# microsoft/Tokenizer

Measured on AMD Instinct MI355X. Metric: input MB/s encoded (cl100k_base), higher is better.
Workload: dtype u8

## Files before the change

### include/tkz.h

```cpp
#ifndef TKZ_H
#define TKZ_H

#include <stddef.h>
#include <stdint.h>

#ifdef __cplusplus
extern "C" {
#endif

typedef enum tkz_status {
    TKZ_OK = 0,
    TKZ_E_FORMAT = -1,
    TKZ_E_DUP_RANK = -2,
    TKZ_E_KEY_NOT_FOUND = -3,
    TKZ_E_CAPACITY = -4,
    TKZ_E_INVALID_UTF8 = -5,
    TKZ_E_ARG = -6,
    TKZ_E_UNSUPPORTED = -7,
    TKZ_E_DEVICE = -8,
    TKZ_E_NO_DEVICE = -9,
    TKZ_E_OUT_OF_MEMORY = -10
} tkz_status;

typedef enum tkz_pattern { TKZ_PATTERN_P1 = 1, TKZ_PATTERN_CL100K = 2, TKZ_PATTERN_O200K = 3, TKZ_PATTERN_O200K_DOTNET = 4 } tkz_pattern;
// ... 44 lines not shown
                                         int32_t n_allowed, int32_t* out_ids, int64_t out_cap, int64_t* out_offsets, int64_t* needed);
void tkz_encoder_special_stats(const tkz_encoder* e, int64_t* batches, int64_t* literals);

typedef struct tkz_pending tkz_pending;
tkz_status tkz_encode_batch_device_begin(tkz_encoder* e, const uint8_t* d_bytes, const int64_t* d_doc_offsets,
                                         int64_t n_docs, int64_t total_bytes, int32_t* d_out_ids,
                                         int64_t out_cap, int64_t* d_out_offsets, void* hip_stream,
                                         tkz_pending** pending);
tkz_status tkz_encode_batch_device_end(tkz_pending* pending, int64_t* total_tokens);
tkz_status tkz_encode_batch_device_begin_counts(tkz_encoder* e, const uint8_t* d_bytes, const int64_t* d_doc_offsets,
                                                int64_t n_docs, int64_t total_bytes, int32_t* d_out_ids,
                                                int64_t out_cap, int64_t* d_out_offsets, void* hip_stream,
                                                int64_t* d_counts3, tkz_pending** pending);
const int64_t* tkz_pending_counts_device(const tkz_pending* pending);

tkz_status tkz_encode_batch_utf16(tkz_encoder* e, const uint16_t* units, const int64_t* unit_offsets,
                                  int64_t n_docs, int32_t* out_ids, int64_t out_cap,
                                  int64_t* out_offsets, int64_t* needed);

tkz_status tkz_encode_utf8(tkz_encoder* e, const uint8_t* text, int64_t len, int32_t* out_ids,
                           int64_t out_cap, int64_t* n_out);
tkz_status tkz_encode_utf16(tkz_encoder* e, const uint16_t* text, int64_t len, int32_t* out_ids,
                            int64_t out_cap, int64_t* n_out);

tkz_status tkz_encode_batch_pieces_utf8(tkz_encoder* e, const uint8_t* bytes, const int64_t* doc_offsets,
                                        int64_t n_docs, int32_t* out_ids, int64_t out_cap,
                                        int64_t* doc_piece_offsets, int64_t* piece_byte_offsets,
                                        int64_t* piece_token_offsets, int64_t piece_cap,
                                        int64_t* n_pieces, int64_t* needed_ids);

tkz_status tkz_encoder_set_special_tokens(tkz_encoder* e, const int32_t* ids, const uint8_t* literals_utf8, const int64_t* literal_offsets, int32_t n);
tkz_status tkz_decode_batch_device(tkz_encoder* e, const int32_t* d_ids, const int64_t* d_id_offsets, int64_t n_docs, int64_t total_ids,
                                   uint8_t* d_out_bytes, int64_t out_cap, int64_t* d_out_offsets, void* hip_stream, int64_t* total_bytes);
tkz_status tkz_decode_batch(tkz_encoder* e, const int32_t* ids, const int64_t* id_offsets, int64_t n_docs, uint8_t* out_bytes, int64_t out_cap,
                            int64_t* out_offsets, int64_t* needed);

tkz_status tkz_shard_write(const char* path, const int32_t* ids, int64_t n_tokens, const int64_t* offsets, int64_t n_docs,
                           int64_t doc_base, int64_t token_base);
tkz_status tkz_shard_write_device(const char* path, int32_t device, const int32_t* d_ids, int64_t n_tokens, const int64_t* d_offsets,
                                  int64_t n_docs, int64_t doc_base, int64_t token_base);
tkz_status tkz_shard_read_header(const char* path, int64_t* n_docs, int64_t* n_tokens, int64_t* doc_base, int64_t* token_base);

typedef struct tkz_comm tkz_comm;
enum { TKZ_COMM_ID_BYTES = 128 };
tkz_status tkz_comm_unique_id(uint8_t* id128);
tkz_status tkz_comm_create(const uint8_t* id128, int32_t rank, int32_t world, int32_t device, tkz_comm** out);
void tkz_comm_destroy(tkz_comm* c);
int32_t tkz_comm_world(const tkz_comm* c);
int32_t tkz_comm_rank(const tkz_comm* c);
const char* tkz_comm_backend(const tkz_comm* c);
tkz_status tkz_comm_allgather_counts_device(tkz_comm* c, const int64_t* d_mine, int64_t* d_table, void* hip_stream);
tkz_status tkz_comm_allgather_counts(tkz_comm* c, int64_t n_docs, int64_t n_bytes, int64_t n_tokens, int64_t* table);
const int64_t* tkz_encoder_counts_device(const tkz_encoder* e);
void tkz_shard_range(int64_t n_docs_total, int32_t rank, int32_t world, int64_t* lo, int64_t* hi);
tkz_status tkz_shard_bases(const int64_t* table, int32_t world, int32_t rank, int64_t* bases3, int64_t* totals3);


tkz_status tkz_pretokenize_utf8(tkz_encoder* e, const uint8_t* bytes, const int64_t* doc_offsets,
                                int64_t n_docs, uint64_t* out_bitmap_words);
tkz_status tkz_encode_pieces(tkz_encoder* e, const uint8_t* bytes, const int64_t* piece_offsets,
                             int64_t n_pieces, int32_t* out_ids, int64_t out_cap,
                             int64_t* out_offsets, int64_t* needed);

enum { TKZ_OPT_PRETOK_SEQUENTIAL = 1,
       TKZ_OPT_PIECE_MEMO = 2,
       TKZ_OPT_PIECE_STATS = 3,
       TKZ_OPT_PROMOTE = 4,
       TKZ_OPT_PROMOTE_MIN_BYTES = 5, TKZ_OPT_PROMOTE_CAP = 6,
       TKZ_OPT_CASE_EQUIVALENCE = 7,
       TKZ_OPT_LATENCY_BYTES = 8,
       TKZ_OPT_ADAPT = 9 };
tkz_status tkz_encoder_set_option(tkz_encoder* e, int32_t option, int64_t value);


enum { TKZ_K_DOCMARK = 0, TKZ_K_PRETOK = 1, TKZ_K_PROBE = 2 , TKZ_K_SCAN = 3, TKZ_K_PLACE = 4,
       TKZ_K_DOCOFFS = 5, TKZ_K_MERGE_LONG = 6 , TKZ_K_MERGE_SHORT = 7 ,
       TKZ_K_COUNT = 8 };
tkz_status tkz_encoder_set_profiling(tkz_encoder* e, int32_t enabled);
tkz_status tkz_encoder_kernel_ms(tkz_encoder* e, double* ms, int64_t* launches, int32_t reset);
void tkz_encoder_pretok_leftovers(const tkz_encoder* e, int64_t* after_ascii_scanner, int64_t* after_multibyte_scanner);
void tkz_encoder_small_path_calls(const tkz_encoder* e, int64_t* calls, int64_t* handed_back);
int32_t tkz_encoder_small_path_phases(const tkz_encoder* e, int64_t* clocks16);
tkz_status tkz_encoder_piece_stats(tkz_encoder* e, int64_t* out8, int32_t reset);
tkz_status tkz_encoder_adapt_stats(tkz_encoder* e, int64_t* out8);
int64_t tkz_encoder_memo_slots(const tkz_encoder* e);
int32_t tkz_encoder_memo_ways(const tkz_encoder* e);
int64_t tkz_encoder_memo_bucket(const tkz_encoder* e, const uint8_t* piece, int32_t len);
tkz_status tkz_encoder_reserve(tkz_encoder* e, int64_t max_bytes, int64_t max_docs);
int64_t tkz_encoder_workspace_bytes(const tkz_encoder* e);
int64_t tkz_encoder_side_by_side_batches(const tkz_encoder* e);
int64_t tkz_encoder_engine_downloads(const tkz_encoder* e);
const char* tkz_kernel_name(int32_t k);

tkz_status tkz_corpus_generate_device(int32_t device, int32_t kind, uint64_t seed, int64_t first_doc,
                                      int64_t n_docs, int32_t min_len, int32_t max_len,
                                      int64_t* d_doc_offsets, uint8_t* d_bytes, int64_t cap_bytes,
                                      void* hip_stream, int64_t* total_bytes);
int64_t tkz_corpus_generate_doc_host(int32_t kind, uint64_t seed, int64_t doc_index, int32_t min_len,
                                     int32_t max_len, uint8_t* buf, int64_t cap);

#ifdef __cplusplus
}
#endif
#endif
```

### tokenizer_amd/_native.py

```python
import ctypes as C
import os

import numpy as np

_HERE = os.path.dirname(os.path.abspath(__file__))
DEFAULT_LIB = os.environ.get("TKZ_LIBTKZ") or os.path.join(_HERE, "lib", "libtkz.so")

OK = 0
E_FORMAT, E_DUP_RANK, E_KEY_NOT_FOUND, E_CAPACITY, E_INVALID_UTF8, E_ARG, E_UNSUPPORTED, E_DEVICE, E_NO_DEVICE, E_OUT_OF_MEMORY = range(-1, -11, -1)
ENGINE_DOTNET, ENGINE_ECMASCRIPT = 0, 1
P1, CL100K, O200K, O200K_DOTNET = 1, 2, 3, 4
OPT_PRETOK_SEQUENTIAL = 1
OPT_PIECE_MEMO = 2
OPT_PIECE_STATS = 3
OPT_PROMOTE_MIN_BYTES, OPT_PROMOTE_CAP = 5, 6
OPT_CASE_EQUIVALENCE = 7
OPT_LATENCY_BYTES = 8
OPT_ADAPT = 9
OPT_PROMOTE = 4
K_NAMES = ["k_docmark", "k_pretok", "k_probe", "k_scan", "k_place", "k_docoffs", "k_merge_long_group", "k_merge_short"]


class TkzError(Exception):

# ... 10 lines not shown
    pass


class KeyNotFoundError(TkzError, KeyError):
    pass


class UnsupportedError(TkzError, NotImplementedError):
    pass


_EXC = {E_FORMAT: FormatError, E_DUP_RANK: DuplicateRankError, E_KEY_NOT_FOUND: KeyNotFoundError, E_UNSUPPORTED: UnsupportedError}


class Library:
    def __init__(self, path=None):
        path = path or DEFAULT_LIB
        if not os.path.exists(path):
            raise RuntimeError("libtkz not built: %s is missing (run `python -c 'import __graft_entry__ as g; g.build()'` "
                               "or `make -C tokenizer_amd/csrc`); there is no CPU fallback" % path)
        self.path = path
        if os.path.basename(path) == "libtkz.so":
            try:
                import torch
                if torch.cuda.is_available():
                    torch.cuda.init()
            except ImportError:
                pass
        L = self.L = C.CDLL(path)
        vp, i64, i32, sz = C.c_void_p, C.c_int64, C.c_int32, C.c_size_t
        pv = C.POINTER(C.c_void_p)
        pi64 = C.POINTER(C.c_int64)
        L.tkz_last_error.restype = C.c_char_p
        L.tkz_vocab_from_tiktoken.argtypes = [vp, sz, pv]
        L.tkz_vocab_destroy.argtypes = [vp]
        L.tkz_vocab_destroy.restype = None
        L.tkz_vocab_size.argtypes = [vp]
        L.tkz_vocab_size.restype = i64
        L.tkz_vocab_max_key_len.argtypes = [vp]
        L.tkz_vocab_pair_table_entries.argtypes = [vp]
        L.tkz_vocab_pair_table_entries.restype = i64
        L.tkz_encoder_memo_slots.argtypes = [vp]
        L.tkz_encoder_memo_slots.restype = i64
        L.tkz_encoder_memo_ways.argtypes = [vp]
        L.tkz_encoder_small_path_calls.argtypes = [vp, pi64, pi64]
        L.tkz_encoder_small_path_calls.restype = None
        L.tkz_encoder_small_path_phases.argtypes = [vp, vp]
        L.tkz_encoder_memo_bucket.argtypes = [vp, vp, i32]
        L.tkz_encoder_memo_bucket.restype = i64
        L.tkz_unicode_classes.argtypes = [C.c_uint32, C.c_int32, vp]
        L.tkz_unicode_classes.restype = None
        L.tkz_encoder_unicode_classes.argtypes = [vp, C.c_uint32, C.c_int32, vp]
        L.tkz_encoder_set_unicode_classes.argtypes = [vp, vp, i64]
        L.tkz_encoder_pretok_leftovers.argtypes = [vp, pi64, pi64]
        L.tkz_encoder_pretok_leftovers.restype = None
        L.tkz_vocab_table_bytes.argtypes = [vp, C.c_int32]
        L.tkz_vocab_table_bytes.restype = i64
        L.tkz_vocab_rank.argtypes = [vp, vp, i32]
        L.tkz_pattern_from_regex.argtypes = [C.c_char_p, C.POINTER(i32)]
        L.tkz_pattern_from_regex_engine.argtypes = [C.c_char_p, i32, C.POINTER(i32)]
        L.tkz_encoder_create.argtypes = [vp, i32, i32, pv]
        L.tkz_encoder_destroy.argtypes = [vp]
        L.tkz_encoder_destroy.restype = None
        L.tkz_encoder_device.argtypes = [vp]
        L.tkz_encode_batch_utf8.argtypes = [vp, vp, vp, i64, vp, i64, vp, pi64]
        L.tkz_host_alloc.argtypes = [C.c_size_t, pv]
        L.tkz_host_free.argtypes = [vp]
        L.tkz_host_free.restype = None
        L.tkz_encode_batch_device.argtypes = [vp, vp, vp, i64, i64, vp, i64, vp, vp, pi64]
        L.tkz_encode_batch_device_begin.argtypes = [vp, vp, vp, i64, i64, vp, i64, vp, vp, C.POINTER(vp)]
        L.tkz_encode_batch_device_end.argtypes = [vp, pi64]
        L.tkz_encode_batch_device_begin_counts.argtypes = [vp, vp, vp, i64, i64, vp, i64, vp, vp, vp, C.POINTER(vp)]
        L.tkz_pending_counts_device.argtypes = [vp]
        L.tkz_pending_counts_device.restype = vp
        L.tkz_encode_batch_utf16.argtypes = [vp, vp, vp, i64, vp, i64, vp, pi64]
        L.tkz_encode_utf8.argtypes = [vp, vp, i64, vp, i64, pi64]
        L.tkz_encode_utf16.argtypes = [vp, vp, i64, vp, i64, pi64]
        L.tkz_pretokenize_utf8.argtypes = [vp, vp, vp, i64, vp]
        L.tkz_encode_pieces.argtypes = [vp, vp, vp, i64, vp, i64, vp, pi64]
        L.tkz_encode_batch_pieces_utf8.argtypes = [vp, vp, vp, i64, vp, i64, vp, vp, vp, i64, pi64, pi64]
        L.tkz_encoder_set_option.argtypes = [vp, i32, i64]
        L.tkz_encoder_piece_stats.argtypes = [vp, vp, i32]
        L.tkz_encoder_adapt_stats.argtypes = [vp, vp]
        L.tkz_encoder_reserve.argtypes = [vp, i64, i64]
        L.tkz_encoder_set_profiling.argtypes = [vp, i32]
        L.tkz_encoder_kernel_ms.argtypes = [vp, vp, vp, i32]
        L.tkz_encoder_workspace_bytes.argtypes = [vp]
        L.tkz_encoder_workspace_bytes.restype = i64
        L.tkz_encoder_side_by_side_batches.argtypes = [vp]
        L.tkz_encoder_side_by_side_batches.restype = i64
        L.tkz_encoder_engine_downloads.argtypes = [vp]
        L.tkz_encoder_engine_downloads.restype = i64
        L.tkz_kernel_name.argtypes = [i32]
        L.tkz_kernel_name.restype = C.c_char_p
        L.tkz_corpus_generate_device.argtypes = [i32, i32, C.c_uint64, i64, i64, i32, i32, vp, vp, i64, vp, pi64]
        L.tkz_corpus_generate_doc_host.argtypes = [i32, C.c_uint64, i64, i32, i32, vp, i64]
        L.tkz_corpus_generate_doc_host.restype = i64
        L.tkz_shard_range.argtypes = [i64, i32, i32, pi64, pi64]
        L.tkz_shard_range.restype = None
        L.tkz_shard_bases.argtypes = [vp, i32, i32, vp, vp]
        L.tkz_encoder_counts_device.argtypes = [vp]
        L.tkz_encoder_counts_device.restype = vp
        L.tkz_encoder_set_special_tokens.argtypes = [vp, vp, vp, vp, i32]
        L.tkz_encode_batch_special_device.argtypes = [vp, vp, vp, i64, i64, vp, i32, vp, i64, vp, vp, pi64]
        L.tkz_encode_batch_special_utf8.argtypes = [vp, vp, vp, i64, vp, i32, vp, i64, vp, pi64]
        L.tkz_encoder_special_stats.argtypes = [vp, pi64, pi64]
        L.tkz_encoder_special_stats.restype = None
        L.tkz_decode_batch_device.argtypes = [vp, vp, vp, i64, i64, vp, i64, vp, vp, pi64]
        L.tkz_decode_batch.argtypes = [vp, vp, vp, i64, vp, i64, vp, pi64]
        L.tkz_shard_write.argtypes = [C.c_char_p, vp, i64, vp, i64, i64, i64]
        L.tkz_shard_write_device.argtypes = [C.c_char_p, i32, vp, i64, vp, i64, i64, i64]
        L.tkz_shard_read_header.argtypes = [C.c_char_p, pi64, pi64, pi64, pi64]
        self.has_comm = hasattr(L, "tkz_comm_create")
        if self.has_comm:
            L.tkz_comm_unique_id.argtypes = [vp]
            L.tkz_comm_create.argtypes = [vp, i32, i32, i32, pv]
            L.tkz_comm_destroy.argtypes = [vp]
            L.tkz_comm_destroy.restype = None
            L.tkz_comm_world.argtypes = [vp]
            L.tkz_comm_rank.argtypes = [vp]
            L.tkz_comm_backend.argtypes = [vp]
            L.tkz_comm_backend.restype = C.c_char_p
            L.tkz_comm_allgather_counts_device.argtypes = [vp, vp, vp, vp]
            L.tkz_comm_allgather_counts.argtypes = [vp, i64, i64, i64, vp]

    def check(self, status):
        if status != OK:
            msg = (self.L.tkz_last_error() or b"").decode("utf-8", "replace")
            raise _EXC.get(status, TkzError)(status, msg)


_default = None


def default_library():
    global _default
    if _default is None:
        _default = Library()
    return _default


def _ptr(a):
    return a.ctypes.data if a is not None else None


class Vocab:

    def __init__(self, tiktoken_bytes: bytes, lib: Library = None):
        self.lib = lib or default_library()
        h = C.c_void_p()
        buf = (C.c_uint8 * max(1, len(tiktoken_bytes))).from_buffer_copy(tiktoken_bytes or b"\0")
        self.lib.check(self.lib.L.tkz_vocab_from_tiktoken(buf, len(tiktoken_bytes), C.byref(h)))
        self._h = h

    def __del__(self):
        if getattr(self, "_h", None):
            self.lib.L.tkz_vocab_destroy(self._h)
            self._h = None

    def __len__(self):
        return self.lib.L.tkz_vocab_size(self._h)

    @property
    def max_key_len(self):
        return self.lib.L.tkz_vocab_max_key_len(self._h)

    @property
    def pair_table_entries(self):
        return self.lib.L.tkz_vocab_pair_table_entries(self._h)

    def table_bytes(self):
        f = self.lib.L.tkz_vocab_table_bytes
        d = {k: int(f(self._h, i)) for i, k in enumerate(("short", "mid", "long", "pair", "direct"))}
        d["total"] = int(f(self._h, -1))
        return d

    def rank(self, key: bytes):
        buf = (C.c_uint8 * max(1, len(key))).from_buffer_copy(key or b"\0")
        return self.lib.L.tkz_vocab_rank(self._h, buf, len(key))


class Encoder:

    def __init__(self, vocab: Vocab, pattern: int, device: int = 0):
        self.lib = vocab.lib
        h = C.c_void_p()
        self.lib.check(self.lib.L.tkz_encoder_create(vocab._h, pattern, device, C.byref(h)))
        self._h = h
        self.pattern = pattern

    def close(self):
        if getattr(self, "_h", None):
            self.lib.L.tkz_encoder_destroy(self._h)
            self._h = None

    def __del__(self):
        self.close()

    def set_option(self, opt, value):
        self.lib.check(self.lib.L.tkz_encoder_set_option(self._h, opt, value))

    def set_unicode_classes(self, classes):
        if classes is None:
            self.lib.check(self.lib.L.tkz_encoder_set_unicode_classes(self._h, None, 0))
            return
        a = np.ascontiguousarray(classes, dtype=np.uint8)
        self.lib.check(self.lib.L.tkz_encoder_set_unicode_classes(self._h, a.ctypes.data, len(a)))

    def unicode_classes(self, first, n):
        out = np.zeros(n, np.uint8)
        self.lib.check(self.lib.L.tkz_encoder_unicode_classes(self._h, first, n, out.ctypes.data))
        return out

    def piece_stats(self, reset=False):
        out = np.zeros(8, np.int64)
        self.lib.check(self.lib.L.tkz_encoder_piece_stats(self._h, out.ctypes.data, 1 if reset else 0))
        pieces, sm, lm, gm, look, hit = (int(out[i]) for i in (1, 2, 3, 4, 5, 6))
        return {"batches": int(out[0]), "pieces": pieces, "short_misses": sm, "long_misses": lm, "giant_pieces": gm,
                "whole_piece_hit_rate": round(1.0 - (sm + lm + gm) / pieces, 5) if pieces else None,
                "memo_lookups": look, "memo_hits": hit, "memo_hit_rate": round(hit / look, 5) if look else None,
                "merged_short": look - hit if look else sm, "promoted_pieces_in_tables": int(out[7])}

    def reserve(self, max_bytes, max_docs):
        self.lib.check(self.lib.L.tkz_encoder_reserve(self._h, int(max_bytes), int(max_docs)))

    def adapt_stats(self):
        out = np.zeros(8, np.int64)
        self.lib.check(self.lib.L.tkz_encoder_adapt_stats(self._h, out.ctypes.data))
        return {"promotions": int(out[0]), "relearns": int(out[1]), "promoted_pieces": int(out[2]), "retired_images": int(out[3]),
                "settled_miss_share": None if out[4] < 0 else out[4] / 1e6, "recent_miss_share": None if out[5] < 0 else out[5] / 1e6,
                "bytes_since_tables_changed": int(out[6]), "learning_window_bytes": int(out[7])}

    def set_profiling(self, on):
        self.lib.check(self.lib.L.tkz_encoder_set_profiling(self._h, 1 if on else 0))

    def kernel_ms(self, reset=False):
        ms = np.zeros(len(K_NAMES), np.float64)
        n = np.zeros(len(K_NAMES), np.int64)
        self.lib.check(self.lib.L.tkz_encoder_kernel_ms(self._h, ms.ctypes.data, n.ctypes.data, 1 if reset else 0))
        return {K_NAMES[i]: (float(ms[i]), int(n[i])) for i in range(len(K_NAMES))}

    @property
    def memo_slots(self):
        return int(self.lib.L.tkz_encoder_memo_slots(self._h))

    @property
    def memo_ways(self):
        return int(self.lib.L.tkz_encoder_memo_ways(self._h))

    def memo_bucket(self, piece: bytes):
        return int(self.lib.L.tkz_encoder_memo_bucket(self._h, piece, len(piece)))

    def small_path_calls(self):
        a, b = C.c_int64(0), C.c_int64(0)
        self.lib.L.tkz_encoder_small_path_calls(self._h, C.byref(a), C.byref(b))
        return a.value, b.value

    def small_path_phases(self):
        a = np.zeros(16, np.int64)
        n = self.lib.L.tkz_encoder_small_path_phases(self._h, a.ctypes.data)
        return a[:n].tolist()

    def pretok_leftovers(self):
        a, b = C.c_int64(0), C.c_int64(0)
        self.lib.L.tkz_encoder_pretok_leftovers(self._h, C.byref(a), C.byref(b))
        return a.value, b.value

    @property
    def workspace_bytes(self):
        return self.lib.L.tkz_encoder_workspace_bytes(self._h)

    @property
    def engine_downloads(self):
        return self.lib.L.tkz_encoder_engine_downloads(self._h)

    @property
    def side_by_side_batches(self):
        return self.lib.L.tkz_encoder_side_by_side_batches(self._h)

    def encode_batch(self, data: np.ndarray, offsets: np.ndarray, out_cap=None, out=None):
        data = np.ascontiguousarray(data, dtype=np.uint8)
        offsets = np.ascontiguousarray(offsets, dtype=np.int64)
        n = len(offsets) - 1
        cap = len(data) if out_cap is None else out_cap
        if out is not None:
            ids, ooff = out
            assert ids.dtype == np.int32 and ooff.dtype == np.int64 and ids.flags.c_contiguous and ooff.flags.c_contiguous
            assert len(ooff) >= n + 1
            cap = len(ids)
        else:
            ids = np.empty(max(1, cap), np.int32)
            ooff = np.empty(n + 1, np.int64)
        needed = C.c_int64(0)
        self.lib.check(self.lib.L.tkz_encode_batch_utf8(self._h, _ptr(data), _ptr(offsets), n, _ptr(ids), cap, _ptr(ooff), C.byref(needed)))
        return ids[:needed.value], ooff[:n + 1]

    def encode_batch_special(self, data: np.ndarray, offsets: np.ndarray, allowed, out_cap=None, out=None):
        data = np.ascontiguousarray(data, dtype=np.uint8)
        offsets = np.ascontiguousarray(offsets, dtype=np.int64)
        allowed = np.ascontiguousarray(allowed, dtype=np.int32)
        n = len(offsets) - 1
        cap = len(data) if out_cap is None else out_cap
        if out is not None:
            ids, ooff = out
            assert ids.dtype == np.int32 and ooff.dtype == np.int64 and ids.flags.c_contiguous and ooff.flags.c_contiguous
# ... 240 lines not shown
```

### tokenizer_amd/csrc/tkz_api.cpp

```cpp
#include <algorithm>
#include <cstdio>
#include <cstdlib>
#include <cstring>
#include <atomic>
#include <chrono>
#include <memory>
#include <mutex>
#include <thread>
#include <string>
#include <unordered_map>
#include <unordered_set>
#include <vector>

#include "../../include/tkz.h"
#include "tkz_adapt.h"
#include "tkz_bpe.h"
#include "tkz_corpus.h"
#include "tkz_kernels.h"
#include "tkz_pretok.h"
#include "tkz_promo_select.h"
#include "tkz_sdma.h"
#include "tkz_vocab.h"

namespace {
// ... 5 lines not shown
struct DeviceScope {
    int prev = -1;
    hipError_t enter(int dev) {
        int cur = -1;
        if (hipGetDevice(&cur) == hipSuccess && cur == dev) return hipSuccess;
        const hipError_t r = hipSetDevice(dev);
        if (r == hipSuccess) prev = cur;
        return r;
    }
    ~DeviceScope() { if (prev >= 0) (void)hipSetDevice(prev); }
};

#define HIP_TRY(expr)                                                                                   \
    do {                                                                                                \
        hipError_t e_ = (expr);                                                                         \
        if (e_ != hipSuccess) return fail(TKZ_E_DEVICE, std::string(#expr) + ": " + hipGetErrorString(e_)); \
    } while (0)
#define TKZ_TRY(expr)                                                                                   \
    do {                                                                                                \
        const tkz_status s_ = (expr);                                                                   \
        if (s_ != TKZ_OK) return s_;                                                                    \
    } while (0)

thread_local int64_t g_alloc_ns = 0;
thread_local int g_alloc_calls = 0;
struct AllocClock {
    std::chrono::steady_clock::time_point t0 = std::chrono::steady_clock::now();
    ~AllocClock() { g_alloc_ns += std::chrono::duration_cast<std::chrono::nanoseconds>(std::chrono::steady_clock::now() - t0).count(); ++g_alloc_calls; }
};
struct DevBuf {
    void* p = nullptr; size_t cap = 0;
    hipError_t ensure(size_t n, int64_t* accounted) {
        if (n <= cap) return hipSuccess;
        AllocClock clock;
        size_t want = std::max(n, cap + cap / 2);
        want = (want + 255) & ~size_t(255);
        void* q = nullptr;
        hipError_t e = hipMalloc(&q, want);
        if (e != hipSuccess && want > n) { want = (n + 255) & ~size_t(255); e = hipMalloc(&q, want); }
        if (e != hipSuccess) return e;
        if (p) (void)hipFree(p);
        if (getenv("TKZ_LOG_ALLOC")) fprintf(stderr, "tkz alloc: %zu -> %zu bytes (asked %zu)\n", cap, want, n);
        *accounted += (int64_t)want - (int64_t)cap;
        p = q; cap = want;
        return hipSuccess;
    }
    void release() { if (p) { AllocClock clock; (void)hipFree(p); } p = nullptr; cap = 0; }
    template <class T> T* as() const { return reinterpret_cast<T*>(p); }
};

struct DevView {
    void* p = nullptr;
    template <class T> T* as() const { return reinterpret_cast<T*>(p); }
};

struct CounterBlock {
    int32_t err; int32_t mneed ; int32_t mhigh ;
    int32_t over64 ;
    int64_t grand;
    unsigned long long pool_head;
    int64_t ndocstarts;
    unsigned long long heavy_count;
    int64_t npieces;
    unsigned long long giant_ticket;
    unsigned long long xcount, xcount2;
    unsigned long long coop_count, coop_ticket;
    unsigned long long long_log_count;
    int64_t lq_total;
    unsigned long long miss_short, miss_long;
    unsigned long long n_literals;
};

}

namespace tkz { tkz_status set_error(tkz_status s, const std::string& msg) { return fail(s, msg); } }

struct tkz_vocab { tkz::Vocab v; };

struct Workspace {
    DevBuf w_gq, w_gcnt, w_xq, w_startbits, w_tmp, w_dense, w_tcount, w_prank, w_pcount, w_pbase, w_tbase, w_bsum, w_doctok, w_dcount, w_dbase, w_pool;
    DevBuf w_zero; size_t zero_bytes = 0;
    DevView w_counters, w_docbits, w_heavyq;
    DevBuf w_mlist, w_mquad, w_mcount, w_pextra, w_coopq, w_lqcnt, w_lqbase, w_lq;
    bool learn_window_start = false;
    DevBuf w_candbits, w_segbits, w_specbits, w_endbits, w_segoffs;
    int64_t n_seg = 0;
    int64_t spec_taken = 0;
    DevBuf w_counts3;
    bool sized = false;
    int32_t mcap = tkz::kMissCapMin;
    bool place128 = false;
    int low_lists = 0, low_place = 0;
    bool learning = false;
    DevBuf s_bytes[2], s_offs[2], s_out[3], s_outoffs[3];
    struct U16Stage {
        DevBuf units, offs, docbits, grp, tsum, tbase, bsum, counters, boffs; struct Host { int32_t err; int32_t pad; int64_t grand; }* h = nullptr;
        hipError_t ensure(int64_t max_units, int64_t max_docs, int64_t* acc) {
            const int64_t nw = max_units / 64 + 1, nt = tkz::u16_tiles(max_units), nblk = (nt + tkz::kScanBlock - 1) / tkz::kScanBlock;
            const std::pair<DevBuf*, size_t> want[] = {{&units, (size_t)(max_units + 64) * 2}, {&offs, (size_t)(max_docs + 1) * 8}, {&docbits, (size_t)(nw + 8) * 8},
                                                       {&grp, (size_t)nt * 64 * 4}, {&tsum, (size_t)nt * 4}, {&tbase, (size_t)nt * 8}, {&bsum, (size_t)(nblk + 1) * 8},
                                                       {&counters, 64}, {&boffs, (size_t)(max_docs + 1) * 8}};
            for (const auto& w : want) { const hipError_t r = w.first->ensure(w.second, acc); if (r != hipSuccess) return r; }
            return h ? hipSuccess : hipHostMalloc((void**)&h, 64, 0);
        }
        void release() {
            for (DevBuf* b : {&units, &offs, &docbits, &grp, &tsum, &tbase, &bsum, &counters, &boffs}) b->release();
            if (h) (void)hipHostFree(h);
            h = nullptr;
        }
    } u16[2];
    DevBuf u_bytes[2];
    DevBuf d_grp, d_tsum, d_tbase, d_bsum, d_counters, d_ids, d_idoffs, d_out, d_outoffs;
    DevBuf p_boffs, p_toffs, p_docp;
    CounterBlock* h_counters = nullptr;
    uint8_t* h_small = nullptr;
    bool fork_token = false;
    int64_t forked_batches = 0;
    int64_t last_coop = 0;
    int64_t last_lq_total = -1;
    hipStream_t st_side = nullptr, st_side2 = nullptr; hipEvent_t ev_fork = nullptr, ev_join = nullptr, ev_join2 = nullptr;
    hipStream_t st_small = nullptr;
    std::atomic<int64_t> small_calls{0}, small_fallbacks{0};
    int64_t small_clocks[16] = {};
    hipStream_t st_compute = nullptr, st_in = nullptr, st_out = nullptr;
    hipEvent_t ev_in[2] = {}, ev_out[3] = {};
    tkz::SdmaSignal sig_out[3], sig_outoffs[3];
    int sdma_state = 0;
    std::atomic<int64_t> engine_downloads{0};
    int64_t bytes_allocated = 0;
    bool busy = false;
    hipEvent_t ev[tkz::K_COUNT][2] = {};
    bool ev_used[tkz::K_COUNT] = {};
    double ms[tkz::K_COUNT] = {};
    int64_t launches[tkz::K_COUNT] = {};
    void release_all() {
        DevBuf* bufs[] = {&w_candbits, &w_segbits, &w_specbits, &w_endbits, &w_segoffs, &w_counts3, &w_mlist, &w_mquad, &w_mcount, &w_pextra, &w_coopq, &w_lqcnt, &w_lqbase, &w_lq, &w_gq, &w_gcnt, &w_xq, &w_zero, &w_startbits, &w_tmp, &w_dense, &w_tcount, &w_prank, &w_pcount, &w_pbase, &w_tbase, &w_bsum,
                          &w_doctok, &w_dcount, &w_dbase, &w_pool, &s_bytes[0], &s_bytes[1], &s_offs[0], &s_offs[1], &s_out[0], &s_out[1], &s_out[2],
                          &s_outoffs[0], &s_outoffs[1], &s_outoffs[2], &u_bytes[0], &u_bytes[1],
                          &d_grp, &d_tsum, &d_tbase, &d_bsum, &d_counters, &d_ids, &d_idoffs, &d_out, &d_outoffs, &p_boffs, &p_toffs, &p_docp};
        for (DevBuf* b : bufs) b->release();
        for (U16Stage& U : u16) U.release();
        if (h_counters) (void)hipHostFree(h_counters);
        if (h_small) (void)hipHostFree(h_small);
        if (st_small) (void)hipStreamDestroy(st_small);
        for (hipStream_t st : {st_side, st_side2}) if (st) (void)hipStreamDestroy(st);
        for (hipEvent_t ev : {ev_fork, ev_join, ev_join2}) if (ev) (void)hipEventDestroy(ev);
        for (int k = 0; k < tkz::K_COUNT; ++k) for (int q = 0; q < 2; ++q) if (ev[k][q]) (void)hipEventDestroy(ev[k][q]);
        for (int q = 0; q < 2; ++q) if (ev_in[q]) (void)hipEventDestroy(ev_in[q]);
        for (int q = 0; q < 3; ++q) if (ev_out[q]) (void)hipEventDestroy(ev_out[q]);
        if (st_compute) (void)hipStreamDestroy(st_compute);
        if (st_in) (void)hipStreamDestroy(st_in);
        if (st_out) (void)hipStreamDestroy(st_out);
        for (int q = 0; q < 3; ++q) { tkz::sdma_signal_destroy(&sig_out[q]); tkz::sdma_signal_destroy(&sig_outoffs[q]); }
    }
};

struct tkz_encoder {
    int device = 0;
    int pattern = 0;
    int max_key_len = 0;
    bool pretok_seq = false;
    bool profiling = false;
    std::mutex mu;
    std::vector<Workspace*> pool;
    DevBuf t_short, t_mid, t_long, t_blob, t_pair, t_byte, t_bpair, t_bmp, t_counts3, t_memo;
    uint32_t memo_slots = 0;
    TkzTables T{};
    DevBuf t_decoff, t_decblob, t_decids;
    TkzDecodeTable D{};
    std::vector<std::pair<int32_t, std::string>> dec_vocab, dec_special;
    DevBuf t_lit;
    tkz::TkzLitTable LIT{};
    int lit_state = 0;
    std::string lit_why;
    std::atomic<int64_t> spec_batches{0}, spec_literals{0};
    int64_t bytes_allocated = 0;
    std::atomic<int64_t> last_xcount{0}, last_xcount2{0};
    bool small_ok = false;
    bool piece_stats = false;
    int64_t latency_bytes = [] { const char* v = getenv("TKZ_LATENCY_BYTES"); return v ? (int64_t)atoll(v) : int64_t(16) << 20; }();
    bool case_equiv = false;
    size_t bmp_image_bytes = 0;
    DevBuf t_stats;
    int64_t stat_batches = 0, stat_giants = 0;
    int pending = 0;
    bool destroyed = false;
    tkz::AdaptPolicy policy;
    DevBuf t_memo_hits, t_promo;
    DevBuf t_long_log;
    int64_t long_log_n = 0;
    std::vector<DevBuf> retired;
    std::vector<tkz::KeyItem> promo_items;
    std::unordered_set<std::string> promo_keys;
    std::vector<uint32_t> promo_quads;
    uint32_t short_slots_n = 0, mid_slots_n = 0;
    std::thread promo_thread;
    std::mutex promo_join_mu;
};

namespace {

std::atomic<int> g_fork_in_flight{0};

struct SpecialCall { tkz::TkzLitAllowed allowed; };
thread_local const SpecialCall* g_special = nullptr;
struct SpecialScope {
    explicit SpecialScope(const SpecialCall* c) { g_special = c; }
    ~SpecialScope() { g_special = nullptr; }
};

struct Lease {
    tkz_encoder* e; Workspace* ws = nullptr;
    explicit Lease(tkz_encoder* enc) : e(enc) {
        std::lock_guard<std::mutex> lock(e->mu);
        for (Workspace* w : e->pool) if (!w->busy) { ws = w; break; }
        if (!ws) { ws = new Workspace(); e->pool.push_back(ws); }
        ws->busy = true;
    }
    ~Lease() {
// ... 154 lines not shown
    if (h == hipSuccess) h = img->nt.ensure(std::max<size_t>(64, short_bytes + mid_bytes), &acc);
    if (h == hipSuccess && short_bytes) h = hipMemcpyAsync(img->nt.p, ss.data(), short_bytes, hipMemcpyHostToDevice, cs);
    if (h == hipSuccess && mid_bytes) h = hipMemcpyAsync(static_cast<char*>(img->nt.p) + short_bytes, ms.data(), mid_bytes, hipMemcpyHostToDevice, cs);
    if (h == hipSuccess) h = img->np.ensure(std::max<size_t>(64, promo_quads.size() * 4), &acc);
    if (h == hipSuccess && !promo_quads.empty()) h = hipMemcpyAsync(img->np.p, promo_quads.data(), promo_quads.size() * 4, hipMemcpyHostToDevice, cs);
    if (h == hipSuccess) h = hipStreamSynchronize(cs);
    if (cs) (void)hipStreamDestroy(cs);
    if (h != hipSuccess) { img->nt.release(); img->np.release(); return fail(TKZ_E_DEVICE, std::string("promoted tables: ") + hipGetErrorString(h)); }
    img->short_bytes = short_bytes; img->n_short_slots = ss.size(); img->n_mid_slots = ms.size(); img->n_promo = promo_items.size();
    return TKZ_OK;
}
void install_key_tables(tkz_encoder* e, KeyTablesImage& img, bool retire) {
    int64_t* acc = &e->bytes_allocated;
    *acc += (int64_t)(img.nt.cap + img.np.cap);
    if (retire) { e->retired.push_back(e->t_short); e->retired.push_back(e->t_promo); }
    else { *acc -= (int64_t)(e->t_short.cap + e->t_promo.cap); e->t_short.release(); e->t_promo.release(); }
    e->t_short = img.nt; e->t_promo = img.np;
    e->T.short_slots = e->t_short.as<TkzShortSlot>(); e->T.short_nb = (uint32_t)(img.n_short_slots / 2); e->T.short_seed = img.sseed;
    e->T.mid_slots = reinterpret_cast<const TkzMidSlot*>(e->t_short.as<char>() + img.short_bytes); e->T.mid_ns = (uint32_t)img.n_mid_slots; e->T.mid_seed = img.mseed;
    e->T.promo = img.n_promo ? e->t_promo.as<uint4>() : nullptr; e->T.promo_n = (uint32_t)img.n_promo;
    e->short_slots_n = (uint32_t)img.n_short_slots; e->mid_slots_n = (uint32_t)img.n_mid_slots;
}

void join_promotion(tkz_encoder* e) {
    std::lock_guard<std::mutex> lock(e->promo_join_mu);
    if (e->promo_thread.joinable()) e->promo_thread.join();
}
tkz_status promote_from_memo(tkz_encoder* e, bool use_hits, bool retire, int64_t* added) {
    using tkz::kLongLogDwords; using tkz::kLongLogMaxLen;
    if (added) *added = 0;
    if (!e->memo_slots || e->T.max_rank >= (int32_t)kPromoFlag) return TKZ_OK;
    std::vector<TkzMemoSlot> memo(e->memo_slots);
    std::vector<uint32_t> hits;
    hipStream_t cs = nullptr;
    HIP_TRY(hipStreamCreateWithFlags(&cs, hipStreamNonBlocking));
    struct StreamGuard { hipStream_t s; ~StreamGuard() { (void)hipStreamDestroy(s); } } stream_guard{cs};
    HIP_TRY(hipMemcpyAsync(memo.data(), e->t_memo.p, memo.size() * sizeof(TkzMemoSlot), hipMemcpyDeviceToHost, cs));
    if (use_hits) { hits.resize(e->memo_slots); HIP_TRY(hipMemcpyAsync(hits.data(), e->t_memo_hits.p, hits.size() * 4, hipMemcpyDeviceToHost, cs)); }
    HIP_TRY(hipStreamSynchronize(cs));
    std::vector<uint32_t> llog;
    if (use_hits && e->t_long_log.p) {
        unsigned long long n = 0;
        HIP_TRY(hipMemcpyAsync(&n, e->t_long_log.as<char>() + (size_t)kLongLogCap * kLongLogDwords * 4, 8, hipMemcpyDeviceToHost, cs));
        HIP_TRY(hipStreamSynchronize(cs));
        e->long_log_n = (int64_t)std::min<unsigned long long>(n, (unsigned long long)kLongLogCap);
    }
    if (use_hits && e->long_log_n > 0) {
        llog.resize((size_t)e->long_log_n * kLongLogDwords);
        HIP_TRY(hipMemcpyAsync(llog.data(), e->t_long_log.p, llog.size() * 4, hipMemcpyDeviceToHost, cs));
        HIP_TRY(hipStreamSynchronize(cs));
    }
    std::vector<tkz::KeyItem> items_copy;
    std::vector<uint32_t> quads_copy;
    {
        std::lock_guard<std::mutex> lock(e->mu);
        const tkz::PromoSelection sel = tkz::select_promotions(memo, use_hits ? &hits : nullptr, llog, e->policy.cap(), &e->promo_items, &e->promo_keys, &e->promo_quads);
        if (use_hits) e->policy.memo_read_back(sel.valid_slots, e->memo_slots);
        if (added) *added = sel.added;
        if (!sel.added) return TKZ_OK;
        items_copy = e->promo_items; quads_copy = e->promo_quads;
    }
    KeyTablesImage img;
    const tkz_status bs = build_key_tables_image(e, items_copy, quads_copy, &img);
    if (bs != TKZ_OK) return bs;
    std::lock_guard<std::mutex> lock(e->mu);
    install_key_tables(e, img, retire);
    return TKZ_OK;
}

tkz_status drop_promotions(tkz_encoder* e, bool retire) {
    {
        std::lock_guard<std::mutex> lock(e->mu);
        if (e->promo_items.empty()) return TKZ_OK;
    }
    KeyTablesImage img;
    const tkz_status st = build_key_tables_image(e, {}, {}, &img);
    if (st != TKZ_OK) return st;
    std::lock_guard<std::mutex> lock(e->mu);
    e->promo_items.clear(); e->promo_keys.clear(); e->promo_quads.clear();
    install_key_tables(e, img, retire);
    return TKZ_OK;
}

tkz_status prepare_workspace(Workspace* ws, int64_t total, int64_t n_docs, bool bitmap_only, bool pieces) {
    using namespace tkz;
    const int64_t nwords = total / 64 + 1;
    const int64_t ntiles = (total + kSub - 1) / kSub;
    const int64_t nblk = (ntiles + kScanBlock - 1) / kScanBlock;
    int64_t* acc = &ws->bytes_allocated;
    {
        static_assert(sizeof(CounterBlock) <= 256, "the counter block's place in the zero region");
        const size_t off_bits = 256, off_flags = off_bits + (size_t)(nwords + 8) * 8, end = off_flags + (size_t)ntiles + 64;
        HIP_TRY(ws->w_zero.ensure(end, acc));
        ws->w_counters.p = ws->w_zero.p; ws->w_docbits.p = ws->w_zero.as<char>() + off_bits; ws->w_heavyq.p = ws->w_zero.as<char>() + off_flags;
        ws->zero_bytes = bitmap_only ? off_flags : end;
    }
    HIP_TRY(ws->w_startbits.ensure((size_t)(nwords + 8) * 8, acc));
    HIP_TRY(ws->w_counts3.ensure(32, acc));
    if (!bitmap_only) {
        HIP_TRY(ws->w_tmp.ensure((size_t)(total + 64) * 4, acc));
        HIP_TRY(ws->w_dense.ensure((size_t)(ntiles / kMergeGroup + 1) * kDenseCap * 4, acc));
        HIP_TRY(ws->w_tcount.ensure((size_t)ntiles * 4, acc));
        HIP_TRY(ws->w_pcount.ensure((size_t)ntiles * 4, acc));
        HIP_TRY(ws->w_pbase.ensure((size_t)ntiles * 8, acc));
        HIP_TRY(ws->w_prank.ensure((size_t)(total / 3 + 8 * ntiles + 4096) * 4, acc));
        HIP_TRY(ws->w_mlist.ensure((size_t)ntiles * (size_t)ws->mcap * 4, acc));
        HIP_TRY(ws->w_mquad.ensure((size_t)ntiles * (size_t)ws->mcap * 16, acc));
        HIP_TRY(ws->w_mcount.ensure((size_t)ntiles * 4, acc));
        HIP_TRY(ws->w_pextra.ensure((size_t)ntiles * 4, acc));
        HIP_TRY(ws->w_coopq.ensure((size_t)(total / kLanePiece + 64) * 8, acc));
        {
            const int64_t nchunks = (ntiles + 63) / 64;
            HIP_TRY(ws->w_lqcnt.ensure((size_t)nchunks * 16 * 4, acc));
            HIP_TRY(ws->w_lqbase.ensure((size_t)(nchunks * 16 + 1) * 8, acc));
            HIP_TRY(ws->w_lq.ensure((size_t)(total / (kShortMax + 1) + 64) * 8, acc));
        }
        HIP_TRY(ws->w_tbase.ensure((size_t)(ntiles + 1) * 8, acc));
        HIP_TRY(ws->w_bsum.ensure((size_t)(nblk + 1) * 8, acc));
        HIP_TRY(ws->w_doctok.ensure((size_t)((pieces ? total : n_docs) + 2) * 4, acc));
        HIP_TRY(ws->w_dcount.ensure((size_t)ntiles * 4, acc));
        HIP_TRY(ws->w_dbase.ensure((size_t)ntiles * 8, acc));
        HIP_TRY(ws->w_gq.ensure((size_t)(total / kArenaPiece + 2) * 24, acc));
        HIP_TRY(ws->w_gcnt.ensure((size_t)ntiles * 4, acc));
        if (!ws->w_pool.p) HIP_TRY(ws->w_pool.ensure((size_t)std::min<int64_t>(24 * total + 4096, int64_t(64) << 20), acc));
    }
    return TKZ_OK;
}

struct PiecesOut { int64_t* piece_boffs; int64_t* piece_toffs; int64_t* doc_piece; int64_t piece_cap; int64_t n_pieces; };

struct SlowCallLog {
    int64_t total; int attempts = 0; std::chrono::steady_clock::time_point t0 = std::chrono::steady_clock::now();
    SlowCallLog(int64_t n) : total(n) { g_alloc_ns = 0; g_alloc_calls = 0; }
    ~SlowCallLog() {
        const char* v = getenv("TKZ_LOG_SLOW_MS");
        const long limit_ms = v ? atol(v) : -1L;
        if (limit_ms < 0) return;
        const double ms = std::chrono::duration<double, std::milli>(std::chrono::steady_clock::now() - t0).count();
        if (ms > (double)limit_ms)
            { fprintf(stderr, "tkz: batch call of %lld bytes: %.1f ms on the host, %.1f ms of it in %d hipMalloc/hipFree calls, %d attempt(s)\n", (long long)total, ms, (double)g_alloc_ns * 1e-6, g_alloc_calls, attempts); fflush(stderr); }
    }
};
struct HostTrace {
    static bool on() { static const bool v = getenv("TKZ_TRACE_HOST") != nullptr; return v; }
    std::chrono::steady_clock::time_point t_call = std::chrono::steady_clock::now();
    std::vector<std::pair<std::string, double>> stamps;
    void stamp(const char* what, int64_t k) {
        if (on()) stamps.emplace_back(std::string(what) + " " + std::to_string(k), std::chrono::duration<double, std::micro>(std::chrono::steady_clock::now() - t_call).count());
    }
    void print(int64_t nchunks) const {
        if (!on()) return;
        std::string line = "[tkz host trace] " + std::to_string(nchunks) + " chunks:";
        for (const auto& sp : stamps) { char b[96]; snprintf(b, sizeof b, " %s @%.0f", sp.first.c_str(), sp.second); line += b; }
        fprintf(stderr, "%s\n", line.c_str());
    }
};
enum { kCallWhole = 0, kCallBegin = 1, kCallEnd = 2 };
struct IngestSrc { const uint8_t* h_bytes; const int64_t* h_offs; };

constexpr int64_t kForkMaxLong = int64_t(1) << 20;
constexpr int64_t kForkMaxLongTail = int64_t(1) << 21, kForkTailShare = 2048;
void side_streams(tkz_encoder* e, Workspace* ws, int64_t total, tkz::Launch* L) {
    const bool short_queue = ws->last_lq_total >= 0 && (ws->last_lq_total <= kForkMaxLong || (ws->last_lq_total <= kForkMaxLongTail && ws->last_coop * kForkTailShare >= ws->last_lq_total));
    if (total <= e->latency_bytes || !short_queue) return;
    if (!ws->fork_token) { int none = 0; ws->fork_token = g_fork_in_flight.compare_exchange_strong(none, 1); }
    bool ok = ws->fork_token;
    for (hipStream_t* st : {&ws->st_side, &ws->st_side2}) if (!*st && hipStreamCreateWithFlags(st, hipStreamNonBlocking) != hipSuccess) { *st = nullptr; ok = false; }
    for (hipEvent_t* ev : {&ws->ev_fork, &ws->ev_join, &ws->ev_join2}) if (!*ev && hipEventCreateWithFlags(ev, hipEventDisableTiming) != hipSuccess) { *ev = nullptr; ok = false; }
    if (ok) { L->side = ws->st_side; L->side2 = ws->st_side2; L->ev_fork = ws->ev_fork; L->ev_join = ws->ev_join; L->ev_join2 = ws->ev_join2; }
    else (void)hipGetLastError();
}

int64_t sizing_sample(int64_t ntiles) {
    int64_t min_sub = (int64_t(64) << 20) / tkz::kSub;
    { const char* v = getenv("TKZ_SIZING_MIN_SUB"); if (v && atoll(v) > 0) min_sub = atoll(v); }
    return ntiles >= min_sub ? std::min<int64_t>(ntiles, std::max<int64_t>(ntiles / 16, min_sub / 16)) : -1;
}

tkz_status arm_learning(tkz_encoder* e, Workspace* ws, int64_t total, bool first, bool may_learn, hipStream_t stream, TkzTables* T) {
    using namespace tkz;
    {
        std::lock_guard<std::mutex> lock(e->mu);
        bool others = false;
        for (Workspace* w : e->pool) if (w != ws && w->busy) others = true;
        const AdaptPolicy::Arm arm = e->policy.may_learn(total, first && !ws->learning, may_learn, e->T.memo_n != 0, e->T.max_rank < (int32_t)kPromoFlag, e->promo_items.size(), others);
        if (arm != AdaptPolicy::Arm::No && e->t_memo_hits.ensure((size_t)e->memo_slots * 4, &e->bytes_allocated) == hipSuccess &&
            e->t_long_log.ensure((size_t)kLongLogCap * kLongLogDwords * 4 + 64, &e->bytes_allocated) == hipSuccess) {
            const bool clear = arm == AdaptPolicy::Arm::YesClearMemo;
            if (!clear || (hipMemsetAsync(e->t_memo.p, 0, size_t(e->memo_slots) * sizeof(TkzMemoSlot), stream) == hipSuccess && hipStreamSynchronize(stream) == hipSuccess)) {
                ws->learn_window_start = e->policy.window_armed(clear);
                ws->learning = true;
            }
        }
        *T = e->T;
    }
    if (ws->learning) {
        T->memo_hits = e->t_memo_hits.as<uint32_t>();
        T->memo_hits_sparse = total >= (int64_t(64) << 20) ? 1u : 0u;
        if (ws->learn_window_start && first) {
            HIP_TRY(hipMemsetAsync(T->memo_hits, 0, (size_t)e->memo_slots * 4, stream));
            HIP_TRY(hipMemsetAsync(e->t_long_log.as<char>() + (size_t)kLongLogCap * kLongLogDwords * 4, 0, 64, stream));
        }
    }
    return TKZ_OK;
}

tkz::EncodeParams bind_params(Workspace* ws, const uint8_t* d_bytes, const int64_t* d_offs, int64_t n_docs, int64_t total) {
    using namespace tkz;
    char* cb = ws->w_counters.as<char>();
    EncodeParams P{};
    P.bytes = d_bytes; P.total = total; P.startbits = ws->w_startbits.as<uint64_t>(); P.docbits = ws->w_docbits.as<uint64_t>(); P.nwords = total / 64 + 1;
    P.offs = d_offs; P.n_docs = n_docs;
    P.tmp = ws->w_tmp.as<int32_t>(); P.dense = ws->w_dense.as<int32_t>(); P.tile_count = ws->w_tcount.as<int32_t>();
    P.prank = ws->w_prank.as<int32_t>(); P.prank_cap = (int64_t)(ws->w_prank.cap / 4); P.pcount = ws->w_pcount.as<int32_t>(); P.pbase = ws->w_pbase.as<int64_t>();
    P.mlist = ws->w_mlist.as<uint32_t>(); P.mquad = ws->w_mquad.as<uint4>(); P.mcap = ws->mcap; P.mcount = ws->w_mcount.as<uint32_t>();
    P.docord_base = ws->w_dbase.as<int64_t>(); P.doc_tok = ws->w_doctok.as<int32_t>(); P.counters = ws->w_counters.as<int32_t>();
    P.giant_q = ws->w_gq.as<int64_t>(); P.giant_cap = total / kArenaPiece + 1; P.giant_cnt = ws->w_gcnt.as<int32_t>();
    P.giant_count = reinterpret_cast<unsigned long long*>(cb + offsetof(CounterBlock, heavy_count));
    P.giant_ticket = reinterpret_cast<unsigned long long*>(cb + offsetof(CounterBlock, giant_ticket));
    P.heavy_flag = ws->w_heavyq.as<uint8_t>(); P.nsub = (total + kSub - 1) / kSub;
    P.pool = ws->w_pool.as<int32_t>(); P.pool_head = reinterpret_cast<unsigned long long*>(cb + offsetof(CounterBlock, pool_head)); P.pool_cap = (int64_t)(ws->w_pool.cap / 4);
    return P;
}

#ifdef TKZ_DEVPROF
unsigned long long* g_devprof = nullptr;
tkz_status devprof_arm(tkz::EncodeParams* P, hipStream_t stream) {
    { const char* ab = getenv("TKZ_DEV_ABLATE"); P->ablate = ab ? atoi(ab) : 0; }
    if (P->ablate & 16) {
        if (!g_devprof) { HIP_TRY(hipMalloc((void**)&g_devprof, 64 * 8)); }
        HIP_TRY(hipMemsetAsync(g_devprof, 0, 64 * 8, stream));
    }
    P->devprof = g_devprof;
    return TKZ_OK;
}
tkz_status devprof_report() {
    if (!g_devprof || !getenv("TKZ_DEV_ABLATE") || !(atoi(getenv("TKZ_DEV_ABLATE")) & 16)) return TKZ_OK;
    unsigned long long h[64];
    HIP_TRY(hipMemcpy(h, g_devprof, sizeof h, hipMemcpyDeviceToHost));
    const double w = h[0] ? (double)h[0] : 1.0;
    fprintf(stderr, "[tkz devprof] k_probe waves %llu  clock ticks/wave: total %.0f  load+compact %.0f  short batches %.0f  mid batches %.0f | mid pieces/wave %.1f pieces/wave %.1f\n",
            h[0], h[1] / w, h[2] / w, h[3] / w, h[4] / w, h[5] / w, h[6] / w);
    if (h[51]) fprintf(stderr, "[tkz devprof] k_probe lane-cycle table, per sub-tile: load+compact %.0f ticks (64 lanes) | 13+-byte pre-pass %.0f ticks, %.1f pieces in %.2f passes of 64 (lane use %.3f) | main loop: first bucket %.0f ticks at lane use %.3f (%.2f batches of 64, %.1f pieces), second bucket %.0f ticks for %.1f lanes (%.3f of the lanes of the iterations that run it: %.2f of %.2f iterations), records and lists %.0f ticks at lane use %.3f\n",
                       h[2] / w, h[4] / w, h[5] / w, (double)((h[5] + 63 * h[0]) / 64) / w, h[5] ? (double)h[5] / (64.0 * (double)((h[5] + 63 * h[0]) / 64)) : 0.0,
                       h[48] / w, (double)h[52] / (64.0 * (double)h[51]), h[51] / w, h[52] / w, h[49] / w, h[53] / w, h[54] ? (double)h[53] / (128.0 * (double)h[54]) : 0.0, h[54] / w, (double)((h[51] + 1) / 2) / w,
                       h[50] / w, (double)h[52] / (64.0 * (double)h[51]));
    if (h[8]) fprintf(stderr, "[tkz devprof] k_giant_merge pieces %llu  clock ticks/piece: rounds in global memory %.0f  the tail %.0f | bytes/piece %.0f tokens/piece %.0f | slowest piece %llu ticks | global rounds/piece %.2f | parts/piece when the tail took over %.0f\n",
                      h[8], (double)h[9] / h[8], (double)h[10] / h[8], (double)h[11] / h[8], (double)h[12] / h[8], h[13], (double)h[14] / h[8], (double)h[7] / h[8]);
    if (h[8]) fprintf(stderr, "[tkz devprof] slowest giant piece: %llu bytes -> %llu tokens, global rounds %llu (%llu ticks), bytes first/middle/last %02llx %02llx %02llx\n",
                      h[24], h[27], h[25], h[28], h[29] & 255, (h[29] >> 8) & 255, (h[29] >> 16) & 255);
    if (h[32]) fprintf(stderr, "[tkz devprof] k_merge_long waves %llu units %llu  ticks/wave %.0f | of all ticks: sort %.3f batch formation %.3f bytes %.3f first level %.3f merges %.3f emission %.3f | fast batches %llu lanes/batch %.1f steps/batch %.1f merges/lane %.2f lane use in the merge loop %.3f ticks/step %.0f\n",
                       h[32], h[44], (double)h[33] / h[32], (double)h[34] / h[33], (double)h[35] / h[33], (double)h[36] / h[33], (double)h[37] / h[33], (double)h[38] / h[33], (double)h[39] / h[33],
                       h[40], (double)h[41] / (h[40] ? h[40] : 1), (double)h[42] / (h[40] ? h[40] : 1), (double)h[43] / (h[41] ? h[41] : 1), (double)h[43] / (64.0 * (h[42] ? h[42] : 1)), (double)h[38] / (h[42] ? h[42] : 1));
    if (h[16]) fprintf(stderr, "[tkz devprof] tail: batches %llu merges %llu (%.2f a batch) proposals/batch %.1f | rounds for chains of equal pairs %llu | ticks/batch %.0f | longest tail: %llu batches, %llu ticks\n",
                       h[16], h[17], (double)h[17] / h[16], (double)h[18] / h[16], h[19], (double)h[22] / h[16], h[20], h[23]);
    return TKZ_OK;
}
#else
tkz_status devprof_arm(tkz::EncodeParams*, hipStream_t) { return TKZ_OK; }
tkz_status devprof_report() { return TKZ_OK; }
#endif

tkz_status enqueue_attempt(tkz_encoder* e, Workspace* ws, const tkz::Launch& L, const TkzTables& T, const uint8_t* d_bytes, const int64_t* d_offs, int64_t n_docs,
                           int64_t total, int32_t* d_out, int64_t out_cap, int64_t* d_out_offs, bool pretok, uint64_t* d_bitmap_only, PiecesOut* po,
                           int64_t* d_counts3, const IngestSrc* ingest, bool marks_reused, int64_t nsample, bool* pieces_over) {
    using namespace tkz;
    const hipStream_t stream = L.stream;
    const int64_t nwords = total / 64 + 1, ntiles = (total + kSub - 1) / kSub;
    int32_t* counters = ws->w_counters.as<int32_t>();
    char* cb = ws->w_counters.as<char>();
    uint64_t* docbits = ws->w_docbits.as<uint64_t>();
    uint64_t* startbits = ws->w_startbits.as<uint64_t>();
    const SpecialCall* const special = d_bitmap_only || po || !pretok ? nullptr : g_special;
    if (marks_reused) {
        HIP_TRY(hipMemsetAsync(ws->w_zero.p, 0, 256, stream));
        if (!d_bitmap_only) HIP_TRY(hipMemsetAsync(ws->w_heavyq.p, 0, (size_t)(ws->w_zero.as<char>() + ws->zero_bytes - ws->w_heavyq.as<char>()), stream));
    } else {
        if (ingest) launch_ingest(L, ingest->h_bytes, total, const_cast<uint8_t*>(d_bytes), ingest->h_offs, n_docs + 1, const_cast<int64_t*>(d_offs), ws->w_zero.p, (int64_t)ws->zero_bytes);
        else if (ws->zero_bytes <= (size_t(8) << 20)) launch_ingest(L, nullptr, 0, nullptr, nullptr, 0, nullptr, ws->w_zero.p, (int64_t)ws->zero_bytes);
        else HIP_TRY(hipMemsetAsync(ws->w_zero.p, 0, ws->zero_bytes, stream));
        launch_docmark(L, d_offs, n_docs, total, docbits, counters);
        const uint64_t* isobits = docbits;
        const int64_t* iso_offs = d_offs;
        int64_t n_iso = n_docs;
        if (special) {
            for (DevBuf* b : {&ws->w_candbits, &ws->w_segbits, &ws->w_specbits, &ws->w_endbits}) HIP_TRY(b->ensure((size_t)(nwords + 8) * 8, &ws->bytes_allocated));
            launch_lit_scan(L, d_bytes, total, docbits, nwords, e->LIT, special->allowed, ws->w_candbits.as<uint64_t>(), ws->w_segbits.as<uint64_t>(),
                            ws->w_specbits.as<uint64_t>(), ws->w_endbits.as<uint64_t>(), reinterpret_cast<unsigned long long*>(cb + offsetof(CounterBlock, n_literals)));
            isobits = ws->w_segbits.as<uint64_t>();
            if (e->pretok_seq || e->pattern == TKZ_PATTERN_O200K || e->pattern == TKZ_PATTERN_O200K_DOTNET) {
                int64_t* nseg = reinterpret_cast<int64_t*>(cb + offsetof(CounterBlock, ndocstarts));
                launch_doccount2(L, isobits, isobits, nwords, total, ntiles, ws->w_dcount.as<int32_t>(), ws->w_pcount.as<int32_t>());
                launch_scan2(L, ntiles, ws->w_bsum.as<int64_t>(), ws->w_dcount.as<int32_t>(), ws->w_dbase.as<int64_t>(), nseg, 1, nullptr, nullptr, nullptr, 1, -1);
                HIP_TRY(hipMemcpyAsync(&ws->h_counters->ndocstarts, nseg, 8, hipMemcpyDeviceToHost, stream));
                HIP_TRY(hipStreamSynchronize(stream));
                ws->n_seg = ws->h_counters->ndocstarts;
                HIP_TRY(ws->w_segoffs.ensure((size_t)(ws->n_seg + 2) * 8, &ws->bytes_allocated));
                launch_seg_offsets(L, isobits, nwords, total, ntiles, ws->w_dbase.as<int64_t>(), ws->n_seg, ws->w_segoffs.as<int64_t>());
                iso_offs = ws->w_segoffs.as<int64_t>();
                n_iso = ws->n_seg;
            }
        }
        if (!pretok) {
            HIP_TRY(hipMemcpyAsync(startbits, docbits, (size_t)nwords * 8, hipMemcpyDeviceToDevice, stream));
        } else if (e->pretok_seq) {
            HIP_TRY(hipMemcpyAsync(startbits, isobits, (size_t)nwords * 8, hipMemcpyDeviceToDevice, stream));
            launch_pretok_seq(L, e->pattern, d_bytes, iso_offs, n_iso, total, startbits, T.bmp_class, counters);
        } else {
            HIP_TRY(ws->w_xq.ensure((size_t)(nwords / kRowsPerWave + 4) * 16, &ws->bytes_allocated));
            launch_pretok_rows(L, e->pattern, d_bytes, iso_offs, n_iso, total, isobits, startbits, nwords, T.bmp_class, counters,
                               ws->w_xq.as<int64_t>(), reinterpret_cast<unsigned long long*>(cb + offsetof(CounterBlock, xcount)));
        }
        if (pretok && e->case_equiv && e->pattern == TKZ_PATTERN_CL100K) launch_case_equiv_fix(L, d_bytes, total, isobits, startbits);
        if (special) launch_lit_fix(L, startbits, isobits, ws->w_specbits.as<uint64_t>(), ws->w_endbits.as<uint64_t>(), nwords);
    }
    if (d_bitmap_only) {
        HIP_TRY(hipMemcpyAsync(d_bitmap_only, startbits, (size_t)nwords * 8, hipMemcpyDeviceToDevice, stream));
    } else {
        EncodeParams P = bind_params(ws, d_bytes, d_offs, n_docs, total);
        P.lane_piece = kLanePiece;
        P.latency = total <= e->latency_bytes ? 1 : 0;
        P.tc_atomic = (L.side || P.latency) ? 1 : 0;
        if (L.side && nsample < 0) ++ws->forked_batches;
        P.coop_cap = total / P.lane_piece + 64;
        P.coop_q = ws->w_coopq.as<uint64_t>();
        P.coop_count = reinterpret_cast<unsigned long long*>(cb + offsetof(CounterBlock, coop_count));
        P.coop_ticket = reinterpret_cast<unsigned long long*>(cb + offsetof(CounterBlock, coop_ticket));
        P.lq_cnt = ws->w_lqcnt.as<int32_t>(); P.lq_base = ws->w_lqbase.as<int64_t>(); P.lq = ws->w_lq.as<uint64_t>(); P.lq_cap = total / (kShortMax + 1) + 64;
        P.lq_total = reinterpret_cast<int64_t*>(cb + offsetof(CounterBlock, lq_total)); P.lq_bsum = ws->w_bsum.as<int64_t>();
        P.miss_sums = reinterpret_cast<unsigned long long*>(cb + offsetof(CounterBlock, miss_short));
        P.stats = e->piece_stats ? e->t_stats.as<unsigned long long>() : nullptr;
        if (P.stats) HIP_TRY(hipMemcpyAsync(e->t_stats.as<char>() + 64, P.stats, 64, hipMemcpyDeviceToDevice, stream));
        P.place128 = ws->place128 ? 1 : 0;
        P.promo = T.promo; P.pextra = T.promo ? ws->w_pextra.as<int32_t>() : nullptr;
        if (ws->learning) {
            P.long_log = e->t_long_log.as<uint32_t>(); P.long_log_cap = (int32_t)kLongLogCap; P.long_log_sparse = T.memo_hits_sparse ? 1 : 0;
            P.long_log_count = reinterpret_cast<unsigned long long*>(e->t_long_log.as<char>() + (size_t)kLongLogCap * kLongLogDwords * 4);
        }
        if (special) { P.specbits = ws->w_specbits.as<uint64_t>(); P.lit_meta = e->LIT.meta; P.lit_blob = e->LIT.blob; P.n_lit = e->LIT.n; }
        TKZ_TRY(devprof_arm(&P, stream));
        int64_t* ndocstarts = reinterpret_cast<int64_t*>(cb + offsetof(CounterBlock, ndocstarts));
        int64_t* npieces = reinterpret_cast<int64_t*>(cb + offsetof(CounterBlock, npieces));
        int64_t* grand = reinterpret_cast<int64_t*>(cb + offsetof(CounterBlock, grand));
        const uint64_t* markbits = po ? startbits : docbits;
        P.docbits = markbits;
        launch_doccount2(L, markbits, startbits, nwords, total, ntiles, ws->w_dcount.as<int32_t>(), ws->w_pcount.as<int32_t>());
        launch_scan2(L, ntiles, ws->w_bsum.as<int64_t>(), ws->w_dcount.as<int32_t>(), ws->w_dbase.as<int64_t>(), ndocstarts, 1,
                     ws->w_pcount.as<int32_t>(), ws->w_pbase.as<int64_t>(), npieces, kRecordLine, -1);
        if (po) {
            HIP_TRY(hipMemcpyAsync(&ws->h_counters->ndocstarts, ndocstarts, 8, hipMemcpyDeviceToHost, stream));
            HIP_TRY(hipStreamSynchronize(stream));
            po->n_pieces = ws->h_counters->ndocstarts;
            *pieces_over = po->n_pieces > po->piece_cap;
            if (!*pieces_over) launch_piece_index(L, startbits, nwords, total, ntiles, ws->w_dbase.as<int64_t>(), po->n_pieces, po->piece_boffs, d_offs, n_docs, po->doc_piece);
        }
        if (nsample >= 0) {
            launch_probe_sample(L, T, P, nsample);
        } else {
            launch_encode(L, T, P, ntiles);
            if (P.stats) launch_miss_stats(L, P, ntiles);
            launch_scan2(L, ntiles, ws->w_bsum.as<int64_t>(), P.tile_count, ws->w_tbase.as<int64_t>(), grand, 1, nullptr, nullptr, nullptr, 1, K_SCAN);
            launch_place(L, P, ws->w_tbase.as<int64_t>(), ntiles, d_out, out_cap);
            if (po) {
                if (!*pieces_over) launch_docoffs(L, po->piece_boffs, po->n_pieces, total, ws->w_tbase.as<int64_t>(), markbits, P.docord_base, P.doc_tok, grand, po->piece_toffs);
                launch_counts3(L, n_docs, total, grand, e->t_counts3.as<int64_t>(), ws->w_counts3.as<int64_t>(), d_counts3);
            } else
                launch_docoffs(L, d_offs, n_docs, total, ws->w_tbase.as<int64_t>(), docbits, P.docord_base, P.doc_tok, grand, d_out_offs,
                               n_docs, e->t_counts3.as<int64_t>(), ws->w_counts3.as<int64_t>(), d_counts3);
        }
    }
    HIP_TRY(hipMemcpyAsync(ws->h_counters, counters, sizeof(CounterBlock), hipMemcpyDeviceToHost, stream));
    return TKZ_OK;
}

tkz_status check_counters(tkz_encoder* e, Workspace* ws, hipStream_t stream, int64_t total, int attempt, int64_t nsample, bool bitmap_only, bool* retry) {
    using namespace tkz;
    const CounterBlock& c = *ws->h_counters;
    const int64_t ntiles = (total + kSub - 1) / kSub;
    int64_t* acc = &ws->bytes_allocated;
    const int32_t err = c.err;
    *retry = false;
    if (err & kErrOffsets) return fail(TKZ_E_ARG, "document offsets must start at 0, be non-decreasing and end at the byte count");
    if (err & kErrUtf8) return fail(TKZ_E_INVALID_UTF8, "input is not well-formed UTF-8 (or a document boundary falls inside a character)");
    if (err & kErrTooLong) return fail(TKZ_E_UNSUPPORTED, "a single piece longer than 2^30 bytes");
    if (!bitmap_only) ws->sized = true;
    if (!bitmap_only && nsample < 0 && total > e->latency_bytes) {
        ws->last_coop = (int64_t)c.coop_count;
        ws->last_lq_total = c.lq_total;
    }
    if (nsample >= 0 && (int64_t)c.over64 * 5 > nsample) { ws->place128 = true; ws->low_place = 0; }
    const bool last = attempt >= 4;
    if (err & kErrPool) {
        if (last) return fail(TKZ_E_OUT_OF_MEMORY, "long-piece scratch exhausted");
        const size_t need = (size_t)c.pool_head * 4 + 4096;
        if (ws->w_pool.ensure(need, acc) != hipSuccess)
            return fail(TKZ_E_OUT_OF_MEMORY, "scratch for the pieces longer than 1024 bytes: " + std::to_string(need) + " bytes could not be allocated");
    } else if (err & kErrMissCap) {
        if (last) return fail(TKZ_E_DEVICE, "miss list overflow");
        int32_t want = kMissCapMin;
        while (want < c.mneed && want < kMissCapMax) want *= 2;
        if (want <= ws->mcap) return fail(TKZ_E_DEVICE, "miss list overflow");
        if (ws->w_mlist.ensure((size_t)ntiles * (size_t)want * 4, acc) != hipSuccess || ws->w_mquad.ensure((size_t)ntiles * (size_t)want * 16, acc) != hipSuccess)
            return fail(TKZ_E_OUT_OF_MEMORY, "miss lists: " + std::to_string((size_t)ntiles * (size_t)want * 20) + " bytes could not be allocated");
        ws->mcap = want;
    } else if (err & kErrCapacity) {
        if (last) return fail(TKZ_E_DEVICE, "piece record buffer overflow");
        const size_t need = ((size_t)c.npieces + 4096) * 4;
        if (ws->w_prank.ensure(need, acc) != hipSuccess)
            return fail(TKZ_E_OUT_OF_MEMORY, "piece records: " + std::to_string(need) + " bytes could not be allocated");
    } else if (nsample >= 0) {
        const size_t need = ((size_t)c.npieces + 4096) * 4;
        if (need > ws->w_prank.cap && ws->w_prank.ensure(need, acc) != hipSuccess)
            return fail(TKZ_E_OUT_OF_MEMORY, "piece records: " + std::to_string(need) + " bytes could not be allocated");
    } else {
        if (err & kErrKeyNotFound) return fail(TKZ_E_KEY_NOT_FOUND, "a byte of the input is not in the vocabulary (KeyNotFoundException in the reference)");
        if (!bitmap_only && e->piece_stats) {
            std::lock_guard<std::mutex> lock(e->mu);
            ++e->stat_batches; e->stat_giants += (int64_t)c.heavy_count;
        }
        return TKZ_OK;
    }
    if (e->piece_stats && e->t_stats.p && !bitmap_only) HIP_TRY(hipMemcpyAsync(e->t_stats.p, e->t_stats.as<char>() + 64, 64, hipMemcpyDeviceToDevice, stream));
    *retry = true;
    return TKZ_OK;
}

void settle_workspace(Workspace* ws, int64_t ntiles) {
    using namespace tkz;
    constexpr int kLowBatches = 3;
    const bool heavy = (int64_t)ws->h_counters->over64 * 5 > ntiles;
    if (heavy) { ws->place128 = true; ws->low_place = 0; }
    else if (ws->place128 && ++ws->low_place >= kLowBatches) { ws->place128 = false; ws->low_place = 0; }
    if (ws->mcap <= kMissCapMin) return;
    int32_t want = kMissCapMin;
    while (want < ws->h_counters->mhigh) want *= 2;
    if (want >= ws->mcap) ws->low_lists = 0;
    else if (++ws->low_lists >= kLowBatches) {
        ws->low_lists = 0;
        ws->mcap = std::max(want, ws->mcap / 2);
        if (ws->w_mquad.cap > (size_t)ntiles * (size_t)ws->mcap * 16 * 4) {
            ws->bytes_allocated -= (int64_t)(ws->w_mquad.cap + ws->w_mlist.cap);
            ws->w_mquad.release(); ws->w_mlist.release();
        }
    }
}

void promote_or_drop(tkz_encoder* e, bool promote) {
    DeviceScope scope;
    const bool dev = scope.enter(e->device) == hipSuccess;
    if (promote) {
        int64_t added = 0;
        size_t held;
        { std::lock_guard<std::mutex> lock(e->mu); held = e->promo_items.size(); }
        if (dev) (void)promote_from_memo(e, true, true, &added);
        std::lock_guard<std::mutex> lock(e->mu);
        e->policy.promotion_installed(added, held);
    } else {
        if (dev) (void)drop_promotions(e, true);
        std::lock_guard<std::mutex> lock(e->mu);
        e->policy.promotions_dropped();
    }
}

void after_batch(tkz_encoder* e, Workspace* ws, int64_t total) {
    const CounterBlock& c = *ws->h_counters;
    tkz::AdaptPolicy::After what;
    {
        std::lock_guard<std::mutex> lock(e->mu);
        what = e->policy.batch_ended(total, (double)(c.miss_short + c.miss_long), (double)c.npieces, ws->learning, e->promo_items.size());
        ws->learning = false;
    }
    const bool promote = what == tkz::AdaptPolicy::After::Promote;
    if (!promote && what != tkz::AdaptPolicy::After::Relearn) return;
    join_promotion(e);
    bool started = false;
    {
        std::lock_guard<std::mutex> jl(e->promo_join_mu);
        try { e->promo_thread = std::thread(promote_or_drop, e, promote); started = true; } catch (...) {}
    }
    if (!started) { const std::string keep_msg = g_err; promote_or_drop(e, promote); g_err = keep_msg; }
}

tkz_status encode_device(tkz_encoder* e, Workspace* ws, const uint8_t* d_bytes, const int64_t* d_offs, int64_t n_docs, int64_t total,
                         int32_t* d_out, int64_t out_cap, int64_t* d_out_offs, hipStream_t stream, bool pretok,
                         uint64_t* d_bitmap_only, int64_t* total_tokens, PiecesOut* po = nullptr, int phase = kCallWhole, int64_t* d_counts3 = nullptr,
                         const IngestSrc* ingest = nullptr) {
    using namespace tkz;
    if (n_docs < 0 || total < 0 || out_cap < 0) return fail(TKZ_E_ARG, "negative size");
    if (total_tokens) *total_tokens = 0;
    if (n_docs == 0 && total != 0) return fail(TKZ_E_ARG, "bytes without documents");
    if (total == 0) {
        if (phase != kCallEnd) {
            HIP_TRY(ws->w_counts3.ensure(32, &ws->bytes_allocated));
            { Launch L0{stream, nullptr, ws}; launch_counts3(L0, n_docs, 0, nullptr, e->t_counts3.as<int64_t>(), ws->w_counts3.as<int64_t>(), d_counts3); }
            if (d_out_offs) HIP_TRY(hipMemsetAsync(d_out_offs, 0, (size_t)(n_docs + 1) * sizeof(int64_t), stream));
            if (d_bitmap_only) { const uint64_t one = 1; HIP_TRY(hipMemcpyAsync(d_bitmap_only, &one, 8, hipMemcpyHostToDevice, stream)); }
            if (phase == kCallBegin) return TKZ_OK;
        }
        HIP_TRY(hipStreamSynchronize(stream));
        return TKZ_OK;
    }
    const int64_t ntiles = (total + kSub - 1) / kSub;
    SlowCallLog slow_log(total);
    TKZ_TRY(prepare_workspace(ws, total, n_docs, d_bitmap_only != nullptr, po != nullptr));
    if (!ws->h_counters) HIP_TRY(hipHostMalloc((void**)&ws->h_counters, sizeof(CounterBlock), 0));

    struct LearnGuard {
        tkz_encoder* e; Workspace* ws; bool keep = false;
        ~LearnGuard() { if (!keep && ws->learning) { ws->learning = false; std::lock_guard<std::mutex> lock(e->mu); e->policy.learning_abandoned(); } }
    } learn_guard{e, ws};
    bool marks_ready = false;
    for (int attempt = 0; attempt < 5; ++attempt) {
        slow_log.attempts = attempt + 1;
        bool pieces_over = false;
        const int64_t nsample = attempt == 0 && phase == kCallWhole && !ws->sized && pretok && !d_bitmap_only && !po ? sizing_sample(ntiles) : -1;
        const bool marks_reused = marks_ready;
        Launch L{stream, e->profiling ? prof_hook : nullptr, ws};
        side_streams(e, ws, total, &L);
        if (!(phase == kCallEnd && attempt == 0)) {
            TkzTables T;
            TKZ_TRY(arm_learning(e, ws, total, attempt == 0, pretok && !d_bitmap_only, stream, &T));
            TKZ_TRY(enqueue_attempt(e, ws, L, T, d_bytes, d_offs, n_docs, total, d_out, out_cap, d_out_offs, pretok, d_bitmap_only, po, d_counts3, ingest,
                                    marks_reused, nsample, &pieces_over));
        }
        if (phase == kCallBegin) { learn_guard.keep = true; return TKZ_OK; }
        HIP_TRY(hipStreamSynchronize(stream));
        HIP_TRY(hipGetLastError());
        if (e->profiling) prof_collect(ws);
        if (!d_bitmap_only) TKZ_TRY(devprof_report());
        if (!marks_reused) { e->last_xcount = (int64_t)ws->h_counters->xcount; e->last_xcount2 = (int64_t)ws->h_counters->xcount2; ws->spec_taken = (int64_t)ws->h_counters->n_literals; }
        bool retry = false;
        TKZ_TRY(check_counters(e, ws, stream, total, attempt, nsample, d_bitmap_only != nullptr, &retry));
        marks_ready = true;
        if (retry) continue;
        if (d_bitmap_only) return TKZ_OK;
        settle_workspace(ws, ntiles);
        if (pretok) after_batch(e, ws, total);
        if (g_special && !po) e->spec_literals += ws->spec_taken;
        if (total_tokens) *total_tokens = ws->h_counters->grand;
        if (pieces_over) return fail(TKZ_E_CAPACITY, "piece arrays too small");
        if (ws->h_counters->grand > out_cap) return fail(TKZ_E_CAPACITY, "output capacity too small");
        return TKZ_OK;
    }
    return fail(TKZ_E_DEVICE, "unreachable");
}

constexpr size_t kSmallOffBytes = 0, kSmallOffOffs = tkz::kSmallMaxBytes + 64, kSmallOffIds = kSmallOffOffs + (tkz::kSmallMaxDocs + 1) * 8,
                 kSmallOffOut = kSmallOffIds + tkz::kSmallMaxBytes * 4, kSmallOffRes = kSmallOffOut + (tkz::kSmallMaxDocs + 1) * 8, kSmallBlock = kSmallOffRes + 256;
bool small_eligible(const tkz_encoder* e, const int64_t* offs, int64_t n_docs, int64_t total) {
    if (!e->small_ok || e->profiling || e->pretok_seq || (e->case_equiv && e->pattern == TKZ_PATTERN_CL100K) || total <= 0 || total > tkz::kSmallMaxBytes || n_docs < 1 || n_docs > tkz::kSmallMaxDocs) return false;
    const bool o200k = e->pattern == TKZ_PATTERN_O200K || e->pattern == TKZ_PATTERN_O200K_DOTNET;
    if (o200k && total > tkz::kSmallMaxBytesO200k) return false;
    if (o200k)
        for (int64_t d = 0; d < n_docs; ++d) { const int64_t len = offs[d + 1] - offs[d]; if (len < 0 || len > tkz::kSmallMaxDoc) return false; }
    return true;
}
tkz_status encode_small(tkz_encoder* e, Workspace* ws, const uint8_t* bytes, const int64_t* offs, int64_t n_docs, int64_t total,
                        int32_t* out_ids, int64_t out_cap, int64_t* out_offsets, int64_t* needed, bool* handled) {
    using namespace tkz;
    *handled = false;
    { const tkz_status ps = prepare_workspace(ws, total, n_docs, false, false); if (ps != TKZ_OK) return ps; }
    int64_t* acc = &ws->bytes_allocated;
    HIP_TRY(ws->s_bytes[0].ensure((size_t)kSmallMaxBytes + 64, acc));
    HIP_TRY(ws->s_offs[0].ensure((size_t)(kSmallMaxDocs + 1) * 8, acc));
    if (!ws->h_small) HIP_TRY(hipHostMalloc((void**)&ws->h_small, kSmallBlock, 0));
    if (!ws->st_small) HIP_TRY(hipStreamCreateWithFlags(&ws->st_small, hipStreamNonBlocking));
    uint8_t* H = ws->h_small;
    memcpy(H + kSmallOffBytes, bytes, (size_t)total);
    memcpy(H + kSmallOffOffs, offs, (size_t)(n_docs + 1) * 8);
    int64_t* h_res = reinterpret_cast<int64_t*>(H + kSmallOffRes);
    h_res[0] = -1; h_res[1] = 0; h_res[2] = 0;
    EncodeParams P = bind_params(ws, ws->s_bytes[0].as<uint8_t>(), ws->s_offs[0].as<int64_t>(), n_docs, total);
    P.lane_piece = kSmallLanePiece;
    SmallArgs A{};
    A.h_bytes = H + kSmallOffBytes; A.h_offs = reinterpret_cast<const int64_t*>(H + kSmallOffOffs);
    A.out = reinterpret_cast<int32_t*>(H + kSmallOffIds); A.out_cap = std::min<int64_t>(out_cap, kSmallMaxBytes); A.out_offs = reinterpret_cast<int64_t*>(H + kSmallOffOut);
    A.h_result = h_res;
    A.docbits = ws->w_docbits.as<uint64_t>(); A.startbits = ws->w_startbits.as<uint64_t>();
    A.pcount = ws->w_pcount.as<int32_t>(); A.pbase = ws->w_pbase.as<int64_t>(); A.docord_base = ws->w_dbase.as<int64_t>(); A.tile_base = ws->w_tbase.as<int64_t>();
    A.counter_words = (int32_t)(sizeof(CounterBlock) / 4);
    A.counts3[0] = e->t_counts3.as<int64_t>(); A.counts3[1] = ws->w_counts3.as<int64_t>();
    TkzTables T;
    { std::lock_guard<std::mutex> lock(e->mu); T = e->T; }
    P.promo = T.promo; P.pextra = T.promo ? ws->w_pextra.as<int32_t>() : nullptr;
    Launch L{ws->st_small, nullptr, ws};
    launch_small(L, T, P, A);
    HIP_TRY(hipStreamSynchronize(ws->st_small));
    HIP_TRY(hipGetLastError());
    ws->small_calls.fetch_add(1, std::memory_order_relaxed);
    { std::lock_guard<std::mutex> lock(e->mu); memcpy(ws->small_clocks, h_res + 4, sizeof ws->small_clocks); }
    if (h_res[0] != 0) { ws->small_fallbacks.fetch_add(1, std::memory_order_relaxed); return TKZ_OK; }
    const int64_t tokens = h_res[2];
    if (needed) *needed = tokens;
    *handled = true;
    if (tokens > out_cap) return fail(TKZ_E_CAPACITY, "output capacity too small");
    if (tokens) memcpy(out_ids, H + kSmallOffIds, (size_t)tokens * 4);
    memcpy(out_offsets, H + kSmallOffOut, (size_t)(n_docs + 1) * 8);
    return TKZ_OK;
}

tkz_status check_encoder(tkz_encoder* e, DeviceScope& scope) {
    if (!e) return fail(TKZ_E_ARG, "null encoder");
    hipError_t r = scope.enter(e->device);
    if (r != hipSuccess) return fail(TKZ_E_NO_DEVICE, std::string("hipSetDevice: ") + hipGetErrorString(r));
    return TKZ_OK;
}

hipError_t ensure_streams(Workspace* ws) {
    hipError_t r = hipSuccess;
    if (!ws->st_compute) r = hipStreamCreate(&ws->st_compute);
    if (r == hipSuccess && !ws->st_in) r = hipStreamCreate(&ws->st_in);
    if (r == hipSuccess && !ws->st_out) r = hipStreamCreate(&ws->st_out);
    for (int q = 0; q < 2 && r == hipSuccess; ++q) if (!ws->ev_in[q]) r = hipEventCreate(&ws->ev_in[q]);
    for (int q = 0; q < 3 && r == hipSuccess; ++q) if (!ws->ev_out[q]) r = hipEventCreate(&ws->ev_out[q]);
    return r;
}

bool pinned_host(const void* p, void** dev) {
    if (!p) return false;
    hipPointerAttribute_t a;
    if (hipPointerGetAttributes(&a, p) != hipSuccess) { (void)hipGetLastError(); return false; }
    if (a.type != hipMemoryTypeHost) return false;
    void* d = nullptr;
    if (hipHostGetDevicePointer(&d, const_cast<void*>(p), 0) != hipSuccess || !d) { (void)hipGetLastError(); return false; }
    *dev = d;
    return true;
}

const char* const kMsgUnitOffsets = "document offsets must start at 0, be non-decreasing and end at the unit count";
const char* const kMsgEngineDownload = "a copy engine reported an error for a download";
constexpr int64_t kHostChunkMin = int64_t(8) << 20;

struct HostPlan {
    bool pin_in = false, pin_out = false;
    void *dv_in = nullptr, *dv_offs = nullptr, *dv_ids = nullptr, *dv_ooffs = nullptr;
    int64_t unit = 1, up_bytes = 0, chunk_bytes = 0, nchunks = 1;
    std::vector<int64_t> cut;
    bool blocking = false;
    bool direct_out = false, ingest_in = false;
    int nout = 1;
    int64_t max_units = 0, max_docs = 0;
};
HostPlan plan_host_batch(const void* in, bool u16, const int64_t* offs, int64_t n_docs, const int32_t* out_ids, int64_t out_cap, const int64_t* out_offsets,
                         bool pretok, const uint64_t* bitmap) {
// ... 862 lines not shown
            if (value == 0) join_promotion(e);
            return TKZ_OK;
        }
        if (value != 2 && value != 3) return fail(TKZ_E_ARG, "TKZ_OPT_PROMOTE takes 0, 1, 2 or 3");
        join_promotion(e);
        {
            std::lock_guard<std::mutex> lock(e->mu);
            for (Workspace* w : e->pool) if (w->busy) return fail(TKZ_E_ARG, "promotions can only be made or dropped by hand while no call of this encoder is in flight");
        }
        if (hipDeviceSynchronize() != hipSuccess) return fail(TKZ_E_DEVICE, "hipDeviceSynchronize");
        if (value == 2) return promote_from_memo(e, false, true, nullptr);
        { std::lock_guard<std::mutex> lock(e->mu); e->policy.reset_by_hand(); }
        return drop_promotions(e, true);
    }
    if (option == TKZ_OPT_PIECE_MEMO) {
        DeviceScope scope;
        if (value == 2) join_promotion(e);
        std::lock_guard<std::mutex> lock(e->mu);
        if (value == 2) {
            tkz_status st = check_encoder(e, scope);
            if (st != TKZ_OK) return st;
            for (Workspace* w : e->pool) if (w->busy) return fail(TKZ_E_ARG, "the piece memo can only be emptied while no call of this encoder is in flight");
            if (hipDeviceSynchronize() != hipSuccess) return fail(TKZ_E_DEVICE, "hipDeviceSynchronize");
            if (hipMemset(e->t_memo.p, 0, size_t(e->memo_slots) * sizeof(TkzMemoSlot)) != hipSuccess) return fail(TKZ_E_DEVICE, "hipMemset");
        }
        e->T.memo_n = value ? e->memo_slots : 0u;
        return TKZ_OK;
    }
    if (option == TKZ_OPT_ADAPT) {
        if (value != 0 && value != 1) return fail(TKZ_E_ARG, "TKZ_OPT_ADAPT takes 0 or 1");
        std::lock_guard<std::mutex> lock(e->mu);
        e->policy.set_adapt((int)value);
        return TKZ_OK;
    }
    return fail(TKZ_E_ARG, "unknown option");
}

tkz_status tkz_encoder_adapt_stats(tkz_encoder* e, int64_t* out8) {
    if (!e || !out8) return fail(TKZ_E_ARG, "null argument");
    join_promotion(e);
    std::lock_guard<std::mutex> lock(e->mu);
    e->policy.stats(out8);
    out8[2] = (int64_t)e->promo_items.size(); out8[3] = (int64_t)e->retired.size();
    return TKZ_OK;
}

tkz_status tkz_encoder_set_profiling(tkz_encoder* e, int32_t enabled) {
    if (!e) return fail(TKZ_E_ARG, "null encoder");
    e->profiling = enabled != 0;
    return TKZ_OK;
}
tkz_status tkz_encoder_kernel_ms(tkz_encoder* e, double* ms, int64_t* launches, int32_t reset) {
    if (!e) return fail(TKZ_E_ARG, "null encoder");
    std::lock_guard<std::mutex> lock(e->mu);
    for (int k = 0; k < tkz::K_COUNT; ++k) {
        double m = 0; int64_t n = 0;
        for (Workspace* w : e->pool) { m += w->ms[k]; n += w->launches[k]; if (reset) { w->ms[k] = 0; w->launches[k] = 0; } }
        if (ms) ms[k] = m;
        if (launches) launches[k] = n;
    }
    return TKZ_OK;
}
void tkz_encoder_pretok_leftovers(const tkz_encoder* e, int64_t* after_ascii_scanner, int64_t* after_multibyte_scanner) {
    if (after_ascii_scanner) *after_ascii_scanner = e ? e->last_xcount.load() : 0;
    if (after_multibyte_scanner) *after_multibyte_scanner = e ? e->last_xcount2.load() : 0;
}
tkz_status tkz_encoder_piece_stats(tkz_encoder* e, int64_t* out8, int32_t reset) {
    if (!e || !out8) return fail(TKZ_E_ARG, "null argument");
    for (int i = 0; i < 8; ++i) out8[i] = 0;
    join_promotion(e);
    if (!e->t_stats.p) { std::lock_guard<std::mutex> lock(e->mu); out8[7] = (int64_t)e->promo_items.size(); return TKZ_OK; }
    DeviceScope scope;
    tkz_status st = check_encoder(e, scope);
    if (st != TKZ_OK) return st;
    unsigned long long h[8] = {};
    HIP_TRY(hipDeviceSynchronize());
    HIP_TRY(hipMemcpy(h, e->t_stats.p, sizeof h, hipMemcpyDeviceToHost));
    std::lock_guard<std::mutex> lock(e->mu);
    out8[0] = e->stat_batches; out8[1] = (int64_t)h[4]; out8[2] = (int64_t)h[2]; out8[3] = (int64_t)h[3]; out8[4] = e->stat_giants;
    out8[5] = (int64_t)h[0]; out8[6] = (int64_t)h[1]; out8[7] = (int64_t)e->promo_items.size();
    if (reset) { HIP_TRY(hipMemset(e->t_stats.p, 0, 64)); e->stat_batches = e->stat_giants = 0; }
    return TKZ_OK;
}
int64_t tkz_encoder_memo_slots(const tkz_encoder* e) { return e ? (int64_t)e->memo_slots : 0; }
void tkz_encoder_small_path_calls(const tkz_encoder* e, int64_t* calls, int64_t* handed_back) {
    int64_t c = 0, f = 0;
    if (e) { tkz_encoder* m = const_cast<tkz_encoder*>(e); std::lock_guard<std::mutex> lock(m->mu); for (Workspace* w : e->pool) { c += w->small_calls; f += w->small_fallbacks; } }
    if (calls) *calls = c;
    if (handed_back) *handed_back = f;
}
int32_t tkz_encoder_small_path_phases(const tkz_encoder* e, int64_t* clocks16) {
    if (!e || !clocks16) return 0;
    tkz_encoder* m = const_cast<tkz_encoder*>(e);
    std::lock_guard<std::mutex> lock(m->mu);
    for (Workspace* w : e->pool) if (w->h_small) { memcpy(clocks16, w->small_clocks, 16 * 8); return 16; }
    return 0;
}
int32_t tkz_encoder_memo_ways(const tkz_encoder* e) { return e ? (int32_t)kMemoWays : 0; }
int64_t tkz_encoder_memo_bucket(const tkz_encoder* e, const uint8_t* piece, int32_t len) {
    if (!e || !piece || len < 1 || len > 16 || !e->memo_slots) return -1;
    uint32_t kw[4] = {0, 0, 0, 0};
    for (int32_t i = 0; i < len; ++i) { if (!piece[i]) return -1; kw[i >> 2] |= (uint32_t)piece[i] << (8 * (i & 3)); }
    return (int64_t)tkz_mulhi(tkz_hash_memo(kw, (uint32_t)len), e->memo_slots / kMemoWays);
}
tkz_status tkz_encoder_reserve(tkz_encoder* e, int64_t max_bytes, int64_t max_docs) {
    using namespace tkz;
    if (!e) return fail(TKZ_E_ARG, "null encoder");
    if (max_bytes < 0 || max_docs < 0) return fail(TKZ_E_ARG, "negative size");
    DeviceScope scope;
    tkz_status st = check_encoder(e, scope);
    if (st != TKZ_OK) return st;
    Lease lease(e);
    Workspace* ws = lease.ws;
    int64_t* acc = &ws->bytes_allocated;
    st = prepare_workspace(ws, max_bytes, max_docs, false, false);
    if (st != TKZ_OK) return st;
    const int64_t nwords = max_bytes / 64 + 1;
    HIP_TRY(ws->w_xq.ensure((size_t)(nwords / kRowsPerWave + 4) * 16, acc));
    {
        bool lits; { std::lock_guard<std::mutex> lock(e->mu); lits = e->lit_state == 1; }
        if (lits) for (DevBuf* b : {&ws->w_candbits, &ws->w_segbits, &ws->w_specbits, &ws->w_endbits}) HIP_TRY(b->ensure((size_t)(nwords + 8) * 8, acc));
    }
    if (!ws->h_counters) HIP_TRY(hipHostMalloc((void**)&ws->h_counters, sizeof(CounterBlock), 0));
    HIP_TRY(ensure_streams(ws));
    {
        const int64_t chunk = std::min<int64_t>(max_bytes, int64_t(32) << 20), cdocs = std::min<int64_t>(max_docs, std::max<int64_t>(1, chunk / 16));
        for (int q = 0; q < 3; ++q) {
            if (q < 2) {
                HIP_TRY(ws->s_bytes[q].ensure((size_t)chunk + 64, acc));
                HIP_TRY(ws->s_offs[q].ensure((size_t)(cdocs + 1) * 8, acc));
            }
            HIP_TRY(ws->s_out[q].ensure((size_t)std::max<int64_t>(chunk, 1) * 4, acc));
            HIP_TRY(ws->s_outoffs[q].ensure((size_t)(cdocs + 1) * 8, acc));
        }
    }
    {
        std::lock_guard<std::mutex> lock(e->mu);
        if (e->memo_slots && e->policy.mode() == 1) {
            if (e->t_memo_hits.ensure((size_t)e->memo_slots * 4, &e->bytes_allocated) != hipSuccess ||
                e->t_long_log.ensure((size_t)kLongLogCap * kLongLogDwords * 4 + 64, &e->bytes_allocated) != hipSuccess)
                return fail(TKZ_E_OUT_OF_MEMORY, "learning buffers could not be allocated");
        }
    }
    HIP_TRY(hipDeviceSynchronize());
    return TKZ_OK;
}
int64_t tkz_encoder_workspace_bytes(const tkz_encoder* e) {
    if (!e) return 0;
    tkz_encoder* m = const_cast<tkz_encoder*>(e);
    std::lock_guard<std::mutex> lock(m->mu);
    int64_t n = e->bytes_allocated;
    for (Workspace* w : e->pool) n += w->bytes_allocated;
    return n;
}
int64_t tkz_encoder_side_by_side_batches(const tkz_encoder* e) {
    if (!e) return 0;
    tkz_encoder* m = const_cast<tkz_encoder*>(e);
    std::lock_guard<std::mutex> lock(m->mu);
    int64_t n = 0;
    for (Workspace* w : e->pool) n += w->forked_batches;
    return n;
}
int64_t tkz_encoder_engine_downloads(const tkz_encoder* e) {
    if (!e) return 0;
    tkz_encoder* m = const_cast<tkz_encoder*>(e);
    std::lock_guard<std::mutex> lock(m->mu);
    int64_t n = 0;
    for (Workspace* w : e->pool) n += w->engine_downloads.load(std::memory_order_relaxed);
    return n;
}
const char* tkz_kernel_name(int32_t k) {
    static const char* const names[] = {"k_docmark", "k_pretok", "k_probe", "k_scan", "k_place", "k_docoffs", "k_merge_long_group", "k_merge_short"};
    return (k >= 0 && k < tkz::K_COUNT) ? names[k] : "?";
}

tkz_status tkz_corpus_generate_device(int32_t device, int32_t kind, uint64_t seed, int64_t first_doc, int64_t n_docs,
                                      int32_t min_len, int32_t max_len, int64_t* d_doc_offsets, uint8_t* d_bytes,
                                      int64_t cap_bytes, void* hip_stream, int64_t* total_bytes) {
    if (kind < 1 || kind > 5 || kind == 4 || n_docs < 0 || min_len < 0 || max_len < min_len || !d_doc_offsets || !total_bytes)
        return fail(TKZ_E_ARG, "bad corpus arguments");
    DeviceScope scope;
    hipError_t r = scope.enter(device);
    if (r != hipSuccess) return fail(TKZ_E_NO_DEVICE, std::string("hipSetDevice: ") + hipGetErrorString(r));
    hipStream_t s = static_cast<hipStream_t>(hip_stream);
    int64_t* d_total = nullptr;
    HIP_TRY(hipMalloc((void**)&d_total, 8));
    tkz::launch_corpus(s, kind, seed, first_doc, n_docs, min_len, max_len, d_doc_offsets, d_bytes, d_bytes ? cap_bytes : 0, d_total);
    hipError_t c = hipMemcpyAsync(total_bytes, d_total, 8, hipMemcpyDeviceToHost, s);
    if (c == hipSuccess) c = hipStreamSynchronize(s);
    if (c == hipSuccess) c = hipGetLastError();
    (void)hipFree(d_total);
    if (c != hipSuccess) return fail(TKZ_E_DEVICE, std::string("corpus generation: ") + hipGetErrorString(c));
    if (d_bytes && *total_bytes > cap_bytes) return fail(TKZ_E_CAPACITY, "corpus buffer too small");
    return TKZ_OK;
}

void tkz_shard_range(int64_t n_docs_total, int32_t rank, int32_t world, int64_t* lo, int64_t* hi) {
    if (world < 1) world = 1;
// ... 27 lines not shown
```

### tokenizer_amd/csrc/tkz_kernels.h

```cpp
#pragma once
#include <stdint.h>

#include "tkz_simt.h"
#include "tkz_tables.h"

namespace tkz {

constexpr int kThreads = 256;
constexpr int kSub = 1024;
constexpr int kHalo = 64;
constexpr int kShortMax = 16;
#ifndef TKZ_MERGE_GROUP
#define TKZ_MERGE_GROUP 16
#endif
constexpr int kMergeGroup = TKZ_MERGE_GROUP;
constexpr int kDenseCap = 256 * kMergeGroup;
#ifndef TKZ_ARENA_DWORDS
#define TKZ_ARENA_DWORDS 2560
#endif
constexpr int kArenaDwords = TKZ_ARENA_DWORDS;
constexpr int kArenaPiece = 1024;
#ifndef TKZ_LANE_PIECE
#define TKZ_LANE_PIECE 128
#endif
constexpr int kLanePiece = TKZ_LANE_PIECE;
constexpr int kLongLogDwords = 12, kLongLogMaxLen = 28;
constexpr int kSmallLanePiece = 256;
constexpr int kMaxPiece = 1 << 30;
constexpr int kRowsPerWave = 62;
constexpr int kScanBlock = 1024;
constexpr int kRecordLine = 16;
constexpr int kMissCapMin = 64, kMissCapMax = 1024;

enum { K_DOCMARK = 0, K_PRETOK = 1, K_ENCODE = 2, K_SCAN = 3, K_GATHER = 4, K_DOCOFFS = 5, K_HEAVY = 6, K_MERGE_SHORT = 7, K_COUNT = 8 };

#ifdef TKZ_DEVPROF
#define TKZ_DEV_FLAG(P, bit) (((P).ablate & (bit)) != 0)
#else
#define TKZ_DEV_FLAG(P, bit) false
#endif

struct EncodeParams {
    const uint8_t* bytes; int64_t total;
    const uint64_t* startbits; const uint64_t* docbits; int64_t nwords;
    const int64_t* offs; int64_t n_docs;
    int32_t* tmp;
    int32_t* dense;
    int32_t* tile_count;
    int32_t* prank; int64_t prank_cap;
    const int32_t* pcount;
    const int64_t* pbase;
    uint32_t* mlist; int32_t mcap;
    uint4* mquad;
    uint32_t* mcount;
    const int64_t* docord_base;
    int32_t* doc_tok;
    int32_t* counters;
    int32_t latency;
    int32_t lane_piece;
    uint8_t* heavy_flag; int64_t nsub;
    int32_t* pool; unsigned long long* pool_head; int64_t pool_cap;
    int64_t* giant_q; unsigned long long* giant_count; int64_t giant_cap; int32_t* giant_cnt;
    unsigned long long* giant_ticket;
    uint64_t* coop_q; unsigned long long* coop_count; unsigned long long* coop_ticket; int64_t coop_cap;
    int32_t* lq_cnt; int64_t* lq_base; int64_t* lq_total; int64_t* lq_bsum; uint64_t* lq; int64_t lq_cap;
    unsigned long long* miss_sums;
    unsigned long long* devprof;
    int32_t ablate;
    unsigned long long* stats;
    uint32_t* long_log; unsigned long long* long_log_count; int32_t long_log_cap; int32_t long_log_sparse;
    int32_t* pextra;
    const uint4* promo;
    int32_t tc_atomic;
    int32_t place128;
    const uint64_t* specbits; const uint32_t* lit_meta; const uint8_t* lit_blob; int32_t n_lit;
};

constexpr int kLitMax = 256, kLitMaxLen = 128, kLitMetaHead = 8;
struct TkzLitTable { const uint32_t* meta; const uint8_t* blob; int32_t n; int32_t blob_bytes; };
struct TkzLitAllowed { uint64_t m[kLitMax / 64]; };

constexpr int kSmallLdsBytesNeeded = 86 * 1024;
constexpr int kSmallMaxBytes = 131072, kSmallMaxBytesO200k = 65536, kSmallMaxDocs = 8192, kSmallMaxDoc = 1024;
struct SmallArgs {
    const uint8_t* h_bytes; const int64_t* h_offs;
    int32_t* out; int64_t out_cap; int64_t* out_offs;
    int64_t* h_result;
    uint64_t* docbits; uint64_t* startbits;
    int32_t* pcount; int64_t* pbase; int64_t* docord_base; int64_t* tile_base;
    int32_t counter_words;
    int64_t* counts3[2];
};

typedef void (*KernelHook)(void* ctx, int kernel_id, int phase , hipStream_t s);
struct Launch { hipStream_t stream; KernelHook hook; void* hook_ctx; hipStream_t side = nullptr, side2 = nullptr; hipEvent_t ev_fork = nullptr, ev_join = nullptr, ev_join2 = nullptr; };

void launch_docmark(const Launch& L, const int64_t* d_offs, int64_t n_items, int64_t total, uint64_t* bits, int32_t* counters);
void launch_pretok_rows(const Launch& L, int pattern, const uint8_t* d_bytes, const int64_t* d_offs, int64_t n_docs, int64_t total,
                        const uint64_t* docbits, uint64_t* startbits, int64_t nrows, const uint8_t* bmp, int32_t* counters,
                        int64_t* xq, unsigned long long* xcount);
void launch_pretok_seq(const Launch& L, int pattern, const uint8_t* d_bytes, const int64_t* d_offs, int64_t n_docs, int64_t total,
                       uint64_t* startbits, const uint8_t* bmp, int32_t* counters);
void launch_ingest(const Launch& L, const uint8_t* h_bytes, int64_t total, uint8_t* d_bytes, const int64_t* h_offs, int64_t n_offs, int64_t* d_offs, void* zero, int64_t zero_bytes);
void launch_probe_sample(const Launch& L, const TkzTables& T, const EncodeParams& P, int64_t nsample);
void launch_encode(const Launch& L, const TkzTables& T, const EncodeParams& P, int64_t nsub);
void launch_small(const Launch& L, const TkzTables& T, const EncodeParams& P, const SmallArgs& A);
void launch_scan(const Launch& L, const int32_t* tile_count, int64_t ntiles, int64_t* bsum, int64_t* tile_base, int64_t* grand, int kid, int round_to = 1);
void launch_place(const Launch& L, const EncodeParams& P, const int64_t* tile_base, int64_t nsub, int32_t* out, int64_t out_cap);
void launch_docoffs(const Launch& L, const int64_t* d_offs, int64_t n_docs, int64_t total, const int64_t* tile_base,
                    const uint64_t* docbits, const int64_t* docord_base, const int32_t* doc_tok, const int64_t* grand, int64_t* out_offs,
                    int64_t c3_docs = 0, int64_t* c3a = nullptr, int64_t* c3b = nullptr, int64_t* c3c = nullptr);
void launch_doccount2(const Launch& L, const uint64_t* bits_a, const uint64_t* bits_b, int64_t nwords, int64_t total, int64_t nsub, int32_t* cnt_a, int32_t* cnt_b);
void launch_scan2(const Launch& L, int64_t ntiles, int64_t* bsum, const int32_t* cnt_a, int64_t* base_a, int64_t* grand_a, int round_to_a,
                  const int32_t* cnt_b, int64_t* base_b, int64_t* grand_b, int round_to_b, int kid);
void launch_rebase(const Launch& L, int64_t* offs, int64_t n, int64_t base);
void launch_case_equiv_fix(const Launch& L, const uint8_t* d_bytes, int64_t total, const uint64_t* docbits, uint64_t* startbits);
void launch_miss_stats(const Launch& L, const EncodeParams& P, int64_t nsub);
void launch_lit_scan(const Launch& L, const uint8_t* d_bytes, int64_t total, const uint64_t* docbits, int64_t nwords, const TkzLitTable& LT, const TkzLitAllowed& A,
                     uint64_t* candbits, uint64_t* segbits, uint64_t* specbits, uint64_t* endbits, unsigned long long* n_taken);
void launch_lit_fix(const Launch& L, uint64_t* startbits, const uint64_t* segbits, const uint64_t* specbits, const uint64_t* endbits, int64_t nwords);
void launch_seg_offsets(const Launch& L, const uint64_t* segbits, int64_t nwords, int64_t total, int64_t nsub, const int64_t* ord_base, int64_t n_seg, int64_t* seg_offs);
void launch_counts3(const Launch& L, int64_t n_docs, int64_t total, const int64_t* grand, int64_t* out3, int64_t* out3b = nullptr, int64_t* out3c = nullptr);
int64_t u16_tiles(int64_t total_units);
void launch_u16_len(const Launch& L, const uint16_t* units, int64_t total, const uint64_t* docbits, int64_t ntiles, int32_t* grp_prefix, int32_t* tile_sum);
void launch_u16_write(const Launch& L, const uint16_t* units, int64_t total, const uint64_t* docbits, int64_t ntiles, const int64_t* tile_base,
                      uint8_t* out, const int64_t* unit_offs, int64_t n_docs, const int32_t* grp_prefix, const int64_t* grand, int64_t* byte_offs);
void launch_piece_index(const Launch& L, const uint64_t* startbits, int64_t nwords, int64_t total, int64_t nsub, const int64_t* ord_base,
                        int64_t n_pieces, int64_t* piece_offs, const int64_t* d_offs, int64_t n_docs, int64_t* doc_piece);
int64_t dec_tiles(int64_t total_ids);
void launch_dec_len(const Launch& L, const TkzDecodeTable& D, const int32_t* ids, int64_t total, int64_t ntiles, int32_t* grp_prefix, int32_t* tile_sum);
void launch_dec_write(const Launch& L, const TkzDecodeTable& D, const int32_t* ids, int64_t total, int64_t ntiles, const int64_t* tile_base, uint8_t* out,
                      int64_t out_cap, const int64_t* id_offs, int64_t n_docs, const int32_t* grp_prefix, const int64_t* grand, int64_t* byte_offs, int32_t* counters);
void launch_corpus(hipStream_t s, int kind, uint64_t seed, int64_t first_doc, int64_t n_docs, int min_len, int max_len,
                   int64_t* d_offs, uint8_t* d_bytes, int64_t cap_bytes, int64_t* d_total);

}
```

### tokenizer_amd/csrc/tkz_kernels.hip

```cpp
#include "tkz_kernels.h"

#include <type_traits>

#include "tkz_bpe.h"
#include "tkz_classes.h"
#include "tkz_corpus.h"
#include "tkz_pretok.h"
#include "tkz_simt.h"

namespace tkz {

TKZ_KERNEL(256) void k_docmark(const int64_t* offs, int64_t n_items, int64_t total, uint64_t* bits, int32_t* counters) {
    const int64_t stride = simt::nblocks() * simt::nthreads();
    for (int64_t d = simt::bid() * simt::nthreads() + simt::tid(); d <= n_items; d += stride) {
        const int64_t pos = offs[d];
        bool ok = pos >= 0 && pos <= total;
        if (d == 0) ok = ok && pos == 0;
        if (d == n_items) ok = ok && pos == total;
        else ok = ok && pos <= offs[d + 1];
        if (!ok) { simt::atomic_or((unsigned*)&counters[0], (unsigned)kErrOffsets); continue; }
        const int64_t w = pos >> 6;
        if (d > 0) { const int64_t prev = offs[d - 1]; if (prev >= 0 && prev <= pos && (prev >> 6) == w) continue; }
        uint64_t m = 1ull << (pos & 63);
        int64_t cur = pos;
        for (int64_t e = d + 1; e <= n_items;) {
            const int64_t q = offs[e];
            if (q < cur || (q >> 6) != w) break;
            if (q == cur) {
                int64_t lo = e + 1, hi = n_items + 1;
                while (lo < hi) { const int64_t mid = (lo + hi) >> 1; if (offs[mid] <= cur) lo = mid + 1; else hi = mid; }
                e = lo;
                continue;
            }
            m |= 1ull << (q & 63);
            cur = q; ++e;
        }
        bits[w] = m;
    }
}

struct RowInfo { TkzRowLane L; TkzRowMasks m; bool simple; };
template <int PATTERN>
TKZ_DEV RowInfo tkz_load_row(const TkzSrc& S, int64_t row, const uint8_t* bmp, const uint16_t* aflags) {
    RowInfo r;
    const int64_t pos = (row << 6) + simt::lane();
    const uint32_t b = tkz_gbyte(S, pos);
    const bool full = row >= 0 && ((row + 1) << 6) <= S.total;
    r.simple = full && simt::ballot(b >= 0x80u) == 0;
    if (r.simple) {
        const uint32_t f = aflags[b];
        r.L.pc = tkz_pc_of_flags(f); r.L.len = 1; r.L.off = 0; r.L.b = b; r.L.bad = 0;
        r.m = tkz_row_masks_ascii(f);
    } else {
        r.L = tkz_classify_byte(S, pos, bmp);
        r.m = tkz_row_masks(r.L, PATTERN == TKZ_PAT_CL100K);
    }
    return r;
}

template <int PATTERN>
TKZ_DEV void tkz_rows_sequential(const TkzSrc& S, const uint64_t* docbits, uint64_t* startbits, int64_t nrows, const uint8_t* bmp,
                                 const uint16_t* aflags, int64_t r0, int64_t r1, int32_t* counters) {
    const int lane = simt::lane();
    auto ds_at = [&](int64_t r) -> uint64_t { return (r >= 0 && r < nrows) ? docbits[r] : 0; };
    int64_t rw = r0;
    while (rw > 0) {
        if (ds_at(rw) & 1ull) break;
        const int pc = simt::first_lane(tkz_classify_byte(S, (rw << 6) - 1, bmp).pc);
        if (pc != PC_N && pc != PC_CRLF) break;
        --rw;
    }
    TkzScanCarry cy;
    cy.nb63 = 0; cy.carryN = 0; cy.abs63 = 0; cy.sa_from = -1; cy.sa_end = -1; cy.sa_lastcr = -1;
    int64_t row = rw > 0 ? rw - 1 : 0;
    RowInfo P = tkz_load_row<PATTERN>(S, row - 1, bmp, aflags);
    RowInfo C = tkz_load_row<PATTERN>(S, row, bmp, aflags);
    uint64_t dsP = ds_at(row - 1), dsC = ds_at(row);
    int clenP = 0, o1msP = 0, bad = 0;
    uint64_t c2P = 0, c3P = 0, o1P = 0;
    for (; row < r1; ++row) {
        const RowInfo N = tkz_load_row<PATTERN>(S, row + 1, bmp, aflags);
        const uint64_t dsN = ds_at(row + 1);
        int clenC, o1msC;
        uint64_t c2C, c3C, o1C, out;
        if (C.simple && N.simple) {
            out = tkz_row_eval_ascii<PATTERN>(P.m, C.m, N.m, dsC, dsN, c2P, c3P, o1P, &c2C, &c3C, &o1C, cy, S, docbits, nrows, bmp, row);
            clenC = (int)((c2C >> lane) & 1ull) * 2 + (int)((c3C >> lane) & 1ull) * 3;
            o1msC = (int)((o1C >> lane) & 1ull);
        } else {
            out = tkz_row_eval<PATTERN>(P.L, C.L, N.L, dsP, dsC, dsN, C.m, N.m, clenP, o1msP, &clenC, &o1msC, &c2C, &c3C, &o1C, cy,
                                        S, docbits, nrows, bmp, row);
        }
        if (row >= r0) {
            if (lane == 0) startbits[row] = out;
            bad |= C.L.bad | ((C.L.off != 0 && ((dsC >> lane) & 1ull)) ? 1 : 0);
        }
        P = C; C = N; dsP = dsC; dsC = dsN; clenP = clenC; o1msP = o1msC; c2P = c2C; c3P = c3C; o1P = o1C;
    }
    if (simt::ballot(bad != 0) && lane == 0) simt::atomic_or((unsigned*)&counters[0], (unsigned)kErrUtf8);
}

template <int PATTERN>
TKZ_KERNEL(64) void k_pretok_rows(const uint8_t* bytes, int64_t total, const uint64_t* docbits, uint64_t* startbits,
                                  int64_t nrows, const uint8_t* bmp, int32_t* counters, int64_t* xq, unsigned long long* xcount) {
    TKZ_SHARED uint16_t s_aflags[128];
    TKZ_SHARED uint4 s_blk[(65 * kBlockRowStride) / 16];
    for (int i = simt::tid(); i < 128; i += simt::nthreads()) s_aflags[i] = (uint16_t)tkz_ascii_flags((uint32_t)i, PATTERN == TKZ_PAT_CL100K);
    const int lane = simt::lane();
    const int64_t r0 = simt::bid() * kRowsPerWave;
    const int64_t first = r0 - 1;
    const bool inside = ((first + 64) << 6) <= total;
    if (inside) {
        for (int c = lane; c < 256; c += 64) {
            const int64_t pos = (first << 6) + 16 * (int64_t)c;
            uint4 v; v.x = v.y = v.z = v.w = 0;
            if (pos >= 0) v = tkz_load16(bytes + pos);
            s_blk[((c >> 2) * kBlockRowStride + (c & 3) * 16) / 16] = v;
        }
        if (lane < kBlockRowStride / 16) {
            uint4 z; z.x = z.y = z.z = z.w = 0;
            const int64_t pos = (first + 64) << 6;
            if (lane == 0 && pos + 16 <= total) z = tkz_load16(bytes + pos);
            s_blk[(64 * kBlockRowStride) / 16 + lane] = z;
        }
    }
    simt::sync();
    if (r0 >= nrows) return;
    if (inside) {
        const int64_t row = first + lane;
        const uint64_t ds = (row >= 0 && row < nrows) ? docbits[row] : 0;
        uint64_t out;
        bool done;
        if constexpr (PATTERN == TKZ_PAT_O200K) {
            TkzBlockCtx X; X.bytes = bytes; X.docbits = docbits; X.total = total; X.nrows = nrows; X.row0 = first;
            done = tkz_block_eval_o200k(reinterpret_cast<const uint8_t*>(s_blk), ds, X, &out);
        } else done = tkz_block_eval<PATTERN>(reinterpret_cast<const uint8_t*>(s_blk), ds, bmp, &out);
        if (done) {
            if (lane >= 1 && lane <= kRowsPerWave && row < nrows) startbits[row] = out;
            if (PATTERN == TKZ_PAT_O200K && lane == 0) reinterpret_cast<uint8_t*>(xq)[simt::bid()] = 0;
            return;
        }
    }
    const int64_t r1 = r0 + kRowsPerWave < nrows ? r0 + kRowsPerWave : nrows;
    if constexpr (PATTERN == TKZ_PAT_O200K) {
        for (int64_t r = r0 + lane; r < r1; r += 64) startbits[r] = docbits[r];
        if (lane == 0) reinterpret_cast<uint8_t*>(xq)[simt::bid()] = 1;
    } else {
        TkzSrc S;
        S.bytes = bytes; S.total = total; S.stage = nullptr; S.lo = 0; S.hi = 0;
        tkz_rows_sequential<PATTERN>(S, docbits, startbits, nrows, bmp, s_aflags, r0, r1, counters);
    }
}

constexpr int kPretokBlkQuads = (65 * kBlockRowStride) / 16;
template <int PATTERN>
TKZ_DEV void tkz_pretok_block(int64_t blk, uint4* s_blk, const uint16_t* s_aflags, const uint8_t* bytes, int64_t total, const uint64_t* docbits,
                              uint64_t* startbits, int64_t nrows, const uint8_t* bmp, int32_t* counters) {
    static_assert(PATTERN != TKZ_PAT_O200K, "o200k blocks need the two follow-up kernels");
    const int lane = simt::lane();
    const int64_t r0 = blk * kRowsPerWave;
    if (r0 >= nrows) return;
    const int64_t first = r0 - 1;
    const bool inside = ((first + 64) << 6) <= total;
    if (inside) {
        (void)simt::ballot(true);
        for (int c = lane; c < 256; c += 64) {
            const int64_t pos = (first << 6) + 16 * (int64_t)c;
            uint4 v; v.x = v.y = v.z = v.w = 0;
            if (pos >= 0) v = tkz_load16(bytes + pos);
            s_blk[((c >> 2) * kBlockRowStride + (c & 3) * 16) / 16] = v;
        }
        if (lane < kBlockRowStride / 16) {
            uint4 z; z.x = z.y = z.z = z.w = 0;
            const int64_t pos = (first + 64) << 6;
            if (lane == 0 && pos + 16 <= total) z = tkz_load16(bytes + pos);
            s_blk[(64 * kBlockRowStride) / 16 + lane] = z;
        }
        (void)simt::ballot(true);
        const int64_t row = first + lane;
        const uint64_t ds = (row >= 0 && row < nrows) ? docbits[row] : 0;
        uint64_t out;
        if (tkz_block_eval<PATTERN>(reinterpret_cast<const uint8_t*>(s_blk), ds, bmp, &out)) {
            if (lane >= 1 && lane <= kRowsPerWave && row < nrows) startbits[row] = out;
            return;
        }
    }
    const int64_t r1 = r0 + kRowsPerWave < nrows ? r0 + kRowsPerWave : nrows;
    TkzSrc S;
    S.bytes = bytes; S.total = total; S.stage = nullptr; S.lo = 0; S.hi = 0;
    tkz_rows_sequential<PATTERN>(S, docbits, startbits, nrows, bmp, s_aflags, r0, r1, counters);
}

TKZ_KERNEL_OCC(64, 3) void k_pretok_mb_blocks(const uint8_t* bytes, int64_t total, const uint64_t* docbits, uint64_t* startbits, int64_t nrows,
                                       const uint8_t* bmp, const uint8_t* xflag, int64_t nblk, unsigned long long* xcount, int64_t* xq2, unsigned long long* xcount2,
                                       int by_code_point) {
    TKZ_SHARED uint4 s_blk[(65 * kBlockRowStride) / 16];
    const int lane = simt::lane();
    unsigned long long mine = 0;
    for (int64_t blk = simt::bid(); blk < nblk; blk += simt::nblocks()) {
        if (xflag[blk] != 1) continue;
        ++mine;
        const int64_t r0 = blk * kRowsPerWave, first = r0 - 1;
        bool done = false;
        uint64_t out = 0;
        simt::sync();
        for (int c = lane; c < 260; c += 64) {
            const int64_t pos = (first << 6) + 16 * (int64_t)c;
            uint4 v; v.x = v.y = v.z = v.w = 0;
            if (pos >= 0 && pos + 16 <= total) v = tkz_load16(bytes + pos);
            else if (pos >= 0 && pos < total) {
                uint32_t w[4] = {0, 0, 0, 0};
                for (int j = 0; j < 16; ++j) if (pos + j < total) w[j >> 2] |= (uint32_t)bytes[pos + j] << (8 * (j & 3));
                v.x = w[0]; v.y = w[1]; v.z = w[2]; v.w = w[3];
            }
            if (c < 256) s_blk[((c >> 2) * kBlockRowStride + (c & 3) * 16) / 16] = v;
            else {
                uint4 z; z.x = z.y = z.z = z.w = 0;
                s_blk[(64 * kBlockRowStride) / 16 + (c - 256)] = c == 256 ? v : z;
            }
        }
        if (lane == 0) { uint4 z; z.x = z.y = z.z = z.w = 0; s_blk[(64 * kBlockRowStride) / 16 + 4] = z; }
        simt::sync();
        {
            const int64_t row = first + lane;
            const uint64_t ds = (row >= 0 && row < nrows) ? docbits[row] : 0;
            TkzBlockCtx X; X.bytes = bytes; X.docbits = docbits; X.total = total; X.nrows = nrows; X.row0 = first;
            done = tkz_block_eval_o200k_mb(reinterpret_cast<const uint8_t*>(s_blk), ds, X, bmp, by_code_point != 0, &out);
            if (done && lane >= 1 && lane <= kRowsPerWave && row < nrows) startbits[row] = out;
        }
        if (!done && lane == 0) xq2[simt::atomic_add64(xcount2, 1ull)] = blk;
// ... 178 lines not shown
            if (acc) simt::atomic_or64((unsigned long long*)&startbits[curw], acc);
        }
    }
}

TKZ_KERNEL(256) void k_pretok_seq(const uint8_t* bytes, const int64_t* offs, int64_t n_docs, int64_t total, uint64_t* startbits,
                                  int pattern, const uint8_t* bmp, int32_t* counters) {
    const int64_t stride = simt::nblocks() * simt::nthreads();
    for (int64_t d = simt::bid() * simt::nthreads() + simt::tid(); d < n_docs; d += stride) {
        const int64_t a = offs[d], b = offs[d + 1];
        if (b <= a || a < 0 || b > total) continue;
        TkzDoc doc; doc.b = bytes + a; doc.n = b - a; doc.bmp = bmp; doc.by_code_point = pattern == TKZ_PAT_O200K;
        int bad = 0;
        for (int64_t p = 0; p < doc.n;) { const TkzChar c = tkz_doc_char(doc, p); bad |= c.bad; p += c.len; }
        if (bad) { simt::atomic_or((unsigned*)&counters[0], (unsigned)kErrUtf8); continue; }
        int64_t curw = -1; uint64_t acc = 0;
        for (int64_t p = 0; p < doc.n;) {
            const int64_t g = a + p;
            if ((g >> 6) != curw) {
                if (acc) simt::atomic_or64((unsigned long long*)&startbits[curw], acc);
                curw = g >> 6; acc = 0;
            }
            acc |= 1ull << (g & 63);
            p = tkz_match_at(pattern, doc, p);
        }
        if (acc) simt::atomic_or64((unsigned long long*)&startbits[curw], acc);
    }
}

constexpr uint32_t kPrMiss = 1u << 31, kPrMark = 1u << 30, kPrLong = 1u << 29, kPrGiant = 1u << 28;
constexpr uint32_t kPrRankMask = (1u << 28) - 1u;
constexpr uint32_t kMrDone = 1u << 31, kMrDense = 1u << 30, kMrInline = 1u << 29;
constexpr int kMrLenShift = 10, kMrCntShift = 12;
constexpr uint32_t kMrOffMask = (1u << kMrCntShift) - 1u;
static_assert(kDenseCap <= (1 << kMrCntShift) && kSub <= (1 << kMrLenShift), "the offset field of a result entry");
#ifndef TKZ_PROBE_U
#define TKZ_PROBE_U 2
#endif
#ifndef TKZ_MS_THREADS
#define TKZ_MS_THREADS 256
#endif
#ifndef TKZ_PROBE_OCC
#define TKZ_PROBE_OCC 8
#endif
constexpr int kGroup = kMergeGroup;
constexpr int kMsThreads = TKZ_MS_THREADS;
#ifndef TKZ_PROBE_PER
#define TKZ_PROBE_PER 1
#endif
constexpr int kProbePer = TKZ_PROBE_PER;
constexpr int kMidMax = kSub / (TKZ_SHORT_KEY_MAX + 1) + 2;

TKZ_DEV int64_t tkz_xcd_block(int64_t b, int64_t nblocks) { return (b & 7) * (nblocks >> 3) + (b >> 3); }

template <int BITS>
TKZ_DEV int tkz_wave_scan(int v, int* total) {
    const uint64_t below = tkz_lowmask(simt::lane());
    int pre = 0, tot = 0;
#pragma unroll
    for (int j = 0; j < BITS; ++j) {
        const uint64_t m = simt::ballot((v >> j) & 1);
        pre += tkz_popc64(m & below) << j;
        tot += tkz_popc64(m) << j;
    }
    *total = tot;
    return pre;
}

TKZ_DEV int tkz_wave_scan_sum(int v, int* total) {
    const int x = simt::scan_inclusive(v);
    *total = simt::last_lane(x);
    return x - v;
}

TKZ_DEV uint32_t tkz_key_dword(const uint32_t* s_bytes, int s, int len, int i) {
    const int w = (s >> 2) + i;
    const uint32_t x = simt::alignbit(s_bytes[w + 1], s_bytes[w], (uint32_t)(s & 3) * 8u);
    const int nb = len - 4 * i;
    return nb >= 4 ? x : (nb <= 0 ? 0u : (x & ((1u << (8 * nb)) - 1u)));
}

constexpr int kProbeLdsBytes = (kSub + kHalo) + 2 * (kSub + 2) + 2 * kMidMax + 4 * kMidMax + 4 * (kSub / 32);
constexpr int kProbeLdsQuads = (kProbeLdsBytes + 15) / 16;
struct ProbeLds { uint32_t* bytes; uint16_t* pstart; uint16_t* mid; uint32_t* midres; uint32_t* mark; const uint4* kmask; uint32_t* spec ; };
TKZ_DEV ProbeLds tkz_probe_lds(uint4* wave_quads, const uint4* kmask) {
    ProbeLds L;
    uint8_t* b = reinterpret_cast<uint8_t*>(wave_quads);
    L.bytes = reinterpret_cast<uint32_t*>(b); b += kSub + kHalo;
    L.midres = reinterpret_cast<uint32_t*>(b); b += 4 * kMidMax;
    L.mark = reinterpret_cast<uint32_t*>(b); b += 4 * (kSub / 32);
    L.pstart = reinterpret_cast<uint16_t*>(b); b += 2 * (kSub + 2);
    L.mid = reinterpret_cast<uint16_t*>(b);
    L.kmask = kmask;
    L.spec = nullptr;
    return L;
}
TKZ_DEV void tkz_probe_kmask_init(uint4* s_kmask) {
    if (simt::tid() <= TKZ_SHORT_KEY_MAX) {
        const int len = simt::tid();
        uint32_t m[3];
        for (int i = 0; i < 3; ++i) { const int nb = len - 4 * i; m[i] = nb >= 4 ? 0xFFFFFFFFu : (nb <= 0 ? 0u : ((1u << (8 * nb)) - 1u)); }
        uint4 v; v.x = m[0]; v.y = m[1]; v.z = m[2]; v.w = 0;
        s_kmask[len] = v;
    }
}
struct ProbeText { uint4 v0, v1; };
static_assert((kSub + kHalo) / 16 <= 128, "two 16-byte loads per lane cover the sub-tile and its halo");
TKZ_DEV void tkz_probe_request_text(const EncodeParams& P, int64_t sub, ProbeText* tx) {
    const int lane = simt::lane();
    const int64_t base = sub * kSub;
    uint4 v0, v1;
    v0.x = v0.y = v0.z = v0.w = 0; v1 = v0;
    const int64_t p0 = base + 16 * (int64_t)lane, p1 = base + 16 * (int64_t)(lane + 64);
    if (p0 + 16 <= P.total) v0 = tkz_load16_nt(P.bytes + p0);
    else {
        uint32_t w[4] = {0, 0, 0, 0};
        for (int j = 0; j < 16; ++j) if (p0 + j < P.total) w[j >> 2] |= (uint32_t)P.bytes[p0 + j] << (8 * (j & 3));
        v0.x = w[0]; v0.y = w[1]; v0.z = w[2]; v0.w = w[3];
    }
    if (lane + 64 < (kSub + kHalo) / 16) {
        if (p1 + 16 <= P.total) v1 = tkz_load16_nt(P.bytes + p1);
        else {
            uint32_t w[4] = {0, 0, 0, 0};
            for (int j = 0; j < 16; ++j) if (p1 + j < P.total) w[j >> 2] |= (uint32_t)P.bytes[p1 + j] << (8 * (j & 3));
            v1.x = w[0]; v1.y = w[1]; v1.z = w[2]; v1.w = w[3];
        }
    }
    tx->v0 = v0; tx->v1 = v1;
}
TKZ_DEV int32_t tkz_lit_id(const EncodeParams& P, const uint8_t* sb, const uint8_t* gb, int s, int len) {
    const uint8_t* tx = s + len <= kSub + kHalo ? sb + s : gb + s;
    for (int i = 0; i < P.n_lit; ++i) {
        const uint32_t m = P.lit_meta[kLitMetaHead + 2 * i];
        if ((int)(m >> 16) != len) continue;
        const uint8_t* lit = P.lit_blob + (m & 0xFFFFu);
        int k = 0;
        while (k < len && lit[k] == tx[k]) ++k;
        if (k == len) return (int32_t)P.lit_meta[kLitMetaHead + 2 * i + 1];
    }
    return TKZ_RANK_NONE;
}
template <bool REPORT, bool SPECIAL = false>
TKZ_DEV void tkz_probe_subtile(const TkzTables& T, const EncodeParams& P, int64_t sub, const ProbeLds& LD, ProbeText& tx, int64_t next) {
    const int lane = simt::lane();
    uint32_t* s_bytes = LD.bytes;
    uint16_t* s_pstart = LD.pstart;
    uint16_t* s_mid = LD.mid;
    uint32_t* s_midres = LD.midres;
    uint32_t* s_mark = LD.mark;
    const uint4* s_kmask = LD.kmask;
    const uint8_t* sb = reinterpret_cast<const uint8_t*>(s_bytes);
    const int64_t base = sub * kSub;
    const int nb = (int)(P.total - base < kSub ? P.total - base : kSub);
    const uint8_t* gbase = P.bytes + base;
    const bool prof = TKZ_DEV_FLAG(P, 16);
    long long t_0 = prof ? simt::clock() : 0, t_1 = 0, t_2 = 0, t_3 = 0;
    uint4 v0 = tx.v0, v1 = tx.v1;
    uint64_t myword = 0, mymark = 0;
    uint64_t myspec = 0;
    if (lane < kSub / 64) {
        const int64_t w = sub * (kSub / 64) + lane;
        if (w < P.nwords) { myword = P.startbits[w]; mymark = P.docbits[w]; if (SPECIAL) myspec = P.specbits[w]; }
    }
    const int64_t from = base + nb, w0 = from >> 6;
    uint64_t ahead = (w0 + lane < P.nwords) ? P.startbits[w0 + lane] : 0ull;
    const int64_t pb = P.pbase[sub];
    { uint4* s4 = reinterpret_cast<uint4*>(s_bytes); s4[lane] = v0; if (lane + 64 < (kSub + kHalo) / 16) s4[lane + 64] = v1; }
    if (next >= 0) tkz_probe_request_text(P, next, &tx);
    if (lane < kSub / 64) {
        const int lim = nb - lane * 64;
        if (lim <= 0) myword = 0; else if (lim < 64) myword &= tkz_lowmask(lim);
        s_mark[2 * lane] = (uint32_t)mymark; s_mark[2 * lane + 1] = (uint32_t)(mymark >> 32);
        if (SPECIAL) { LD.spec[2 * lane] = (uint32_t)myspec; LD.spec[2 * lane + 1] = (uint32_t)(myspec >> 32); }
    }
    int64_t last_end;
    {
        int64_t found = -1;
        for (int64_t c = 0; found < 0; ++c) {
            const int64_t w = w0 + c * 64 + lane;
            uint64_t v = c == 0 ? ahead : (w < P.nwords ? P.startbits[w] : 0);
            if (w == w0) v &= ~tkz_lowmask((int)(from & 63));
            const uint64_t any = simt::ballot(v != 0);
            if (any) {
                const int src = tkz_ctz64(any);
                const uint32_t lo = simt::shflu((uint32_t)v, src), hi = simt::shflu((uint32_t)(v >> 32), src);
                found = ((w0 + c * 64 + src) << 6) + tkz_ctz64(((uint64_t)hi << 32) | lo);
            } else if (w0 + (c + 1) * 64 >= P.nwords) found = P.total;
        }
        last_end = found;
    }
    const int last_end_rel = (int)(last_end - base < 2 * kSub + 2 ? last_end - base : 2 * kSub + 2);
    const uint32_t wlo = simt::shflu((uint32_t)myword, lane >> 2), whi = simt::shflu((uint32_t)(myword >> 32), lane >> 2);
    const uint32_t bits16 = (uint32_t)(((((uint64_t)whi << 32) | wlo) >> (16 * (lane & 3))) & 0xFFFFull);
    int np;
    {
        int off = tkz_wave_scan<5>(tkz_popc32(bits16), &np);
        for (uint32_t b = bits16; b; b &= b - 1) s_pstart[off++] = (uint16_t)(16 * lane + tkz_ctz32(b));
        if (lane == 0) s_pstart[np] = (uint16_t)last_end_rel;
    }
    (void)simt::ballot(true);
    if (prof) t_1 = simt::clock();
    const char* tb0 = reinterpret_cast<const char*>(T.short_slots);
    const uint32_t mid_off = (uint32_t)(reinterpret_cast<const char*>(T.mid_slots) - tb0);
    int nmid = 0;
#pragma unroll 1
    for (int k0 = 0; k0 < np; k0 += 64) {
        const int k = k0 + lane;
        int len = 0;
        if (k < np) len = (int)s_pstart[k + 1] - (int)s_pstart[k];
        const uint64_t midm = simt::ballot(len > TKZ_SHORT_KEY_MAX && len <= kArenaPiece);
        if ((midm >> lane) & 1ull) s_mid[nmid + tkz_popc64(midm & tkz_lowmask(lane))] = (uint16_t)k;
        nmid += tkz_popc64(midm);
    }
    (void)simt::ballot(true);
#pragma unroll 1
    for (int m0 = 0; m0 < nmid; m0 += 64) {
        const bool valid = m0 + lane < nmid;
        int s = 0, len = 13;
        uint32_t kk[7] = {0, 0, 0, 0, 0, 0, 0}, oa = 0, ob = 0;
        if (valid) {
            const int k = s_mid[m0 + lane];
            s = s_pstart[k];
            len = (int)s_pstart[k + 1] - s;
        }
        const bool is_lit = SPECIAL && valid && ((LD.spec[s >> 5] >> (s & 31)) & 1u);
        const bool is_mid = valid && len <= TKZ_MID_KEY_MAX && !is_lit;
        if (is_mid) {
#pragma unroll
            for (int i = 0; i < 7; ++i) kk[i] = tkz_key_dword(s_bytes, s, len, i);
            uint32_t s1, s2;
            tkz_mid_slots(T, kk, (uint32_t)len, &s1, &s2);
            oa = mid_off + 32u * s1; ob = mid_off + 32u * s2;
        }
        const uint4 a0 = tkz_load16(tb0 + oa), a1 = tkz_load16(tb0 + oa + 16u), b0 = tkz_load16(tb0 + ob), b1 = tkz_load16(tb0 + ob + 16u);
        int32_t rank = TKZ_RANK_NONE;
        if (is_mid) rank = tkz_match_mid(kk, (uint32_t)len, a0, a1, b0, b1);
        else if (is_lit) rank = tkz_lit_id(P, sb, gbase, s, len);
        else if (valid) {
            if (s + len <= kSub + kHalo) rank = tkz_lookup_long(T, [&](int i) -> uint32_t { return sb[s + i]; }, (uint32_t)len);
            else rank = tkz_lookup_long(T, [&](int i) -> uint32_t { return gbase[s + i]; }, (uint32_t)len);
        }
        if (valid) s_midres[m0 + lane] = (uint32_t)rank;
    }
    (void)simt::ballot(true);
    if (prof) t_2 = simt::clock();
    uint32_t* const ml = P.mlist + sub * (int64_t)P.mcap;
    uint4* const mq = P.mquad + sub * (int64_t)P.mcap;
    int ns = 0, nl = 0, midseen = 0;
    int promo_extra = 0;
    bool giant = false, coopl = false;
    constexpr int U = TKZ_PROBE_U;
#ifdef TKZ_DEVPROF
    long long pf_first = 0, pf_second = 0, pf_emit = 0, pf_t = 0;
    int pf_batches = 0, pf_valid = 0, pf_want2 = 0, pf_iters2 = 0;
#define TKZ_PROBE_MARK(acc) do { if (prof) { const long long pf_now = simt::clock(); acc += pf_now - pf_t; pf_t = pf_now; } } while (0)
    if (prof) pf_t = simt::clock();
#else
#define TKZ_PROBE_MARK(acc) do { } while (0)
#endif
#pragma unroll 1
    for (int k0 = 0; k0 < np; k0 += 64 * U) {
        int ps[U], plen[U];
        uint32_t hs[U], kw0[U], kw1[U], kw2[U];
        uint4 a0[U], a1[U];
#pragma unroll
        for (int u = 0; u < U; ++u) {
            const int k = k0 + 64 * u + lane;
            ps[u] = 0; plen[u] = 0;
            if (k < np) { ps[u] = s_pstart[k]; plen[u] = (int)s_pstart[k + 1] - ps[u]; }
            const int s = ps[u], w = s >> 2;
            const uint32_t sh = (uint32_t)(s & 3) * 8u;
            const uint32_t d0 = s_bytes[w], d1 = s_bytes[w + 1], d2 = s_bytes[w + 2], d3 = s_bytes[w + 3];
            const bool is_short = plen[u] >= 1 && plen[u] <= TKZ_SHORT_KEY_MAX;
            const uint4 km = s_kmask[is_short ? plen[u] : 0];
            kw0[u] = simt::alignbit(d1, d0, sh) & km.x; kw1[u] = simt::alignbit(d2, d1, sh) & km.y; kw2[u] = simt::alignbit(d3, d2, sh) & km.z;
            const uint32_t slot = tkz_short_slot_first(T, kw0[u], kw1[u], kw2[u], (uint32_t)plen[u], &hs[u]);
            const uint32_t oa = is_short ? 16u * slot : 0u;
            a0[u] = tkz_load16(tb0 + oa); a1[u] = tkz_load16(tb0 + oa + 16u);
        }
        int32_t rk[U];
        bool more = false;
#pragma unroll
        for (int u = 0; u < U; ++u) {
            const bool is_short = plen[u] >= 1 && plen[u] <= TKZ_SHORT_KEY_MAX;
            rk[u] = tkz_match_short2x(kw0[u], kw1[u], kw2[u], (uint32_t)plen[u], a0[u], a1[u]);
            if (SPECIAL && is_short && ((LD.spec[ps[u] >> 5] >> (ps[u] & 31)) & 1u)) rk[u] = tkz_lit_id(P, sb, gbase, ps[u], plen[u]);
            more = more || (is_short && rk[u] == TKZ_RANK_NONE);
        }
        bool two_pass = simt::ballot(more) != 0;
        TKZ_PROBE_MARK(pf_first);
#ifdef TKZ_DEVPROF
        if (prof) {
            for (int u = 0; u < U; ++u) { const int nv = np - (k0 + 64 * u); if (nv > 0) { ++pf_batches; pf_valid += nv < 64 ? nv : 64; } }
            for (int u = 0; u < U; ++u) pf_want2 += tkz_popc64(simt::ballot(plen[u] >= 1 && plen[u] <= TKZ_SHORT_KEY_MAX && rk[u] == TKZ_RANK_NONE));
            pf_iters2 += two_pass ? 1 : 0;
            pf_t = simt::clock();
        }
#endif
        if (two_pass) {
#pragma unroll
            for (int u = 0; u < U; ++u) {
                const bool want = plen[u] >= 1 && plen[u] <= TKZ_SHORT_KEY_MAX && rk[u] == TKZ_RANK_NONE;
                if (want) {
                    const uint32_t ob = 16u * tkz_short_slot_second(T, hs[u]);
                    a0[u] = tkz_load16(tb0 + ob); a1[u] = tkz_load16(tb0 + ob + 16u);
                }
            }
#pragma unroll
            for (int u = 0; u < U; ++u) {
                const bool want = plen[u] >= 1 && plen[u] <= TKZ_SHORT_KEY_MAX && rk[u] == TKZ_RANK_NONE;
                if (want) rk[u] = tkz_match_short2x(kw0[u], kw1[u], kw2[u], (uint32_t)plen[u], a0[u], a1[u]);
            }
        }
        TKZ_PROBE_MARK(pf_second);
#pragma unroll
        for (int u = 0; u < U; ++u) {
            const int k = k0 + 64 * u + lane;
            const bool valid = k < np;
            const int s = ps[u], len = plen[u];
            const bool is_mid = len > TKZ_SHORT_KEY_MAX && len <= kArenaPiece;
            const uint64_t midm = simt::ballot(is_mid);
            int32_t rank = rk[u];
            if (is_mid) rank = (int32_t)s_midres[midseen + tkz_popc64(midm & tkz_lowmask(lane))];
            midseen += tkz_popc64(midm);
            const bool is_giant = len > kArenaPiece;
            const bool miss = valid && !is_giant && rank == TKZ_RANK_NONE;
            if (P.pextra) {
                const uint32_t ex = (valid && !is_giant && !miss && ((uint32_t)rank & kPromoFlag)) ? (((uint32_t)rank >> kPromoCntShift) & 3u) : 0u;
                promo_extra += (int)ex;
            }
            const bool miss_s = miss && len <= kShortMax, miss_l = miss && len > kShortMax;
            const uint64_t sm = simt::ballot(miss_s), lm = simt::ballot(miss_l);
            const int is_ = ns + tkz_popc64(sm & tkz_lowmask(lane)), il = nl + tkz_popc64(lm & tkz_lowmask(lane));
            ns += tkz_popc64(sm); nl += tkz_popc64(lm);
            const uint32_t ent = (uint32_t)s | ((uint32_t)(len - 1) << kMrLenShift);
            if (miss_s && is_ + nl < P.mcap) {
                ml[is_] = ent;
                uint4 kq; kq.x = kw0[u]; kq.y = kw1[u]; kq.z = kw2[u]; kq.w = 0;
                if (len > TKZ_SHORT_KEY_MAX) { kq.x = tkz_key_dword(s_bytes, s, len, 0); kq.y = tkz_key_dword(s_bytes, s, len, 1); kq.z = tkz_key_dword(s_bytes, s, len, 2); kq.w = tkz_key_dword(s_bytes, s, len, 3); }
                mq[is_] = kq;
            }
            if (miss_l && il + ns < P.mcap) ml[P.mcap - 1 - il] = ent;
            uint32_t rec = ((s_mark[s >> 5] >> (s & 31)) & 1u) ? kPrMark : 0u;
            if (REPORT) giant = giant || (miss_l && len > kSmallLanePiece);
            else coopl = coopl || (miss_l && len > P.lane_piece);
            if (is_giant) { rec |= kPrMiss | kPrGiant | (uint32_t)s; giant = giant || valid; }
            else if (miss) rec |= kPrMiss | (miss_l ? (kPrLong | (uint32_t)il) : (uint32_t)is_);
            else rec |= (uint32_t)rank;
            if (valid && pb + k < P.prank_cap) tkz_store_nt(&P.prank[pb + k], (int32_t)rec);
        }
        TKZ_PROBE_MARK(pf_emit);
    }
#undef TKZ_PROBE_MARK
#ifdef TKZ_DEVPROF
    if (prof && lane == 0) {
        simt::atomic_add64(&P.devprof[48], (unsigned long long)pf_first); simt::atomic_add64(&P.devprof[49], (unsigned long long)pf_second);
        simt::atomic_add64(&P.devprof[50], (unsigned long long)pf_emit); simt::atomic_add64(&P.devprof[51], (unsigned long long)pf_batches);
        simt::atomic_add64(&P.devprof[52], (unsigned long long)pf_valid); simt::atomic_add64(&P.devprof[53], (unsigned long long)pf_want2);
        simt::atomic_add64(&P.devprof[54], (unsigned long long)pf_iters2);
    }
#endif
    if (prof && lane == 0) {
        t_3 = simt::clock();
        simt::atomic_add64(&P.devprof[0], 1); simt::atomic_add64(&P.devprof[1], (unsigned long long)(t_3 - t_0));
        simt::atomic_add64(&P.devprof[2], (unsigned long long)(t_1 - t_0)); simt::atomic_add64(&P.devprof[3], (unsigned long long)(t_3 - t_2));
        simt::atomic_add64(&P.devprof[4], (unsigned long long)(t_2 - t_1)); simt::atomic_add64(&P.devprof[5], (unsigned long long)nmid);
        simt::atomic_add64(&P.devprof[6], (unsigned long long)np);
    }
    const uint32_t f = (nl ? 1u : 0u) | (simt::ballot(giant) ? 2u : 0u) | (simt::ballot(coopl) ? 4u : 0u);
    if (P.pextra) { int tot; (void)tkz_wave_scan_sum(promo_extra, &tot); promo_extra = tot; }
    if (lane == 0) {
        P.heavy_flag[sub] = (uint8_t)f;
        P.mcount[sub] = (uint32_t)ns | ((uint32_t)nl << 16);
        if (P.pextra) P.pextra[sub] = promo_extra;
        if (!REPORT && P.tc_atomic) P.tile_count[sub] = 0;
        if (REPORT && ns + nl > P.mcap) { simt::atomic_or((unsigned*)&P.counters[0], (unsigned)kErrMissCap); simt::atomic_max((unsigned*)&P.counters[1], (unsigned)(ns + nl)); }
        if (pb + np > P.prank_cap) simt::atomic_or((unsigned*)&P.counters[0], (unsigned)kErrCapacity);
    }
}
TKZ_KERNEL_OCC(256, TKZ_PROBE_OCC) void k_probe(TkzTables T, EncodeParams P) {
    TKZ_SHARED uint4 s_wave[kThreads / 64][kProbeLdsQuads];
    TKZ_SHARED uint4 s_kmask[TKZ_SHORT_KEY_MAX + 1];
    tkz_probe_kmask_init(s_kmask);
    simt::sync();
    const int64_t sub0 = (tkz_xcd_block(simt::bid(), simt::nblocks()) * (kThreads / 64) + simt::wave()) * kProbePer;
    if (sub0 >= P.nsub) return;
    const ProbeLds LD = tkz_probe_lds(s_wave[simt::wave()], s_kmask);
    ProbeText tx;
    tkz_probe_request_text(P, sub0, &tx);
#pragma unroll 1
    for (int it = 0; it < kProbePer && sub0 + it < P.nsub; ++it) {
        const int64_t nxt = (it + 1 < kProbePer && sub0 + it + 1 < P.nsub) ? sub0 + it + 1 : -1;
        tkz_probe_subtile<false>(T, P, sub0 + it, LD, tx, nxt);
        (void)simt::ballot(true);
    }
}

TKZ_KERNEL_OCC(256, TKZ_PROBE_OCC) void k_probe_special(TkzTables T, EncodeParams P) {
    TKZ_SHARED uint4 s_wave[kThreads / 64][kProbeLdsQuads];
    TKZ_SHARED uint4 s_kmask[TKZ_SHORT_KEY_MAX + 1];
    TKZ_SHARED uint32_t s_spec[kThreads / 64][kSub / 32];
    tkz_probe_kmask_init(s_kmask);
    simt::sync();
    const int64_t sub0 = (tkz_xcd_block(simt::bid(), simt::nblocks()) * (kThreads / 64) + simt::wave()) * kProbePer;
    if (sub0 >= P.nsub) return;
    ProbeLds LD = tkz_probe_lds(s_wave[simt::wave()], s_kmask);
    LD.spec = s_spec[simt::wave()];
    ProbeText tx;
    tkz_probe_request_text(P, sub0, &tx);
#pragma unroll 1
    for (int it = 0; it < kProbePer && sub0 + it < P.nsub; ++it) {
        const int64_t nxt = (it + 1 < kProbePer && sub0 + it + 1 < P.nsub) ? sub0 + it + 1 : -1;
        tkz_probe_subtile<false, true>(T, P, sub0 + it, LD, tx, nxt);
        (void)simt::ballot(true);
    }
}

struct alignas(4) TkzDwords4 { uint32_t x, y, z, w; };
TKZ_DEV void tkz_load_piece16(const uint8_t* bytes, int64_t total, int64_t abs, uint32_t* pw) {
    const int64_t a0 = abs & ~(int64_t)3;
    const uint32_t sh = (uint32_t)(abs & 3) * 8u;
    uint32_t w[5];
    if (a0 + 20 <= total) {
        const TkzDwords4 v = *reinterpret_cast<const TkzDwords4*>(bytes + a0);
        w[0] = v.x; w[1] = v.y; w[2] = v.z; w[3] = v.w;
        w[4] = *reinterpret_cast<const uint32_t*>(bytes + a0 + 16);
    } else {
#pragma unroll
        for (int i = 0; i < 5; ++i) {
            const int64_t p = a0 + 4 * i;
            if (p + 4 <= total) w[i] = *reinterpret_cast<const uint32_t*>(bytes + p);
            else { w[i] = 0; for (int j = 0; j < 4; ++j) if (p + j < total) w[i] |= (uint32_t)bytes[p + j] << (8 * j); }
        }
    }
#pragma unroll
    for (int i = 0; i < 4; ++i) pw[i] = simt::alignbit(w[i + 1], w[i], sh);
}

TKZ_HD uint32_t tkz_result_entry(bool dense, int cnt, int off) { return kMrDone | (dense ? kMrDense : 0u) | ((uint32_t)(cnt - 1) << kMrCntShift) | (uint32_t)off; }
TKZ_HD uint32_t tkz_result_inline(int cnt) { return kMrDone | kMrInline | ((uint32_t)(cnt - 1) << kMrCntShift); }
TKZ_HD int tkz_result_cnt(uint32_t r) { return (int)((r >> kMrCntShift) & 1023u) + 1; }
TKZ_HD int tkz_result_off(uint32_t r) { return (int)(r & kMrOffMask); }

template <int N, class Pre>
TKZ_DEV int tkz_find_list(const Pre* pre, int g) {
    int q = 0;
#pragma unroll
    for (int step = N / 2; step >= 1; step >>= 1) if (pre[q + step] <= g) q += step;
    return q;
}

constexpr int kMsStride = TkzBpeGeom<16>::kStride, kMsIdStride = TkzBpeGeom<16>::kIdStride;
#ifndef TKZ_MS_SHORT_LEN
#define TKZ_MS_SHORT_LEN 8
#endif
#ifndef TKZ_MS_TWO_MIN
#define TKZ_MS_TWO_MIN 320
#endif
constexpr int kMsTwoListsMin = TKZ_MS_TWO_MIN;
constexpr int kMsShortLen = TKZ_MS_SHORT_LEN;
struct MsLds { uint4* pr; uint32_t* ids; uint16_t* rec; uint16_t* idx; int* extra; uint16_t* pre; const uint16_t* brank16; };
constexpr int kMsLdsBytes = kMsStride * 64 * 4 + kMsIdStride * 64 * 4 + 2 * (2 * 64 + 2 * 64) + 4 * kGroup + 2 * (kGroup + 1);
constexpr int kMsLdsQuads = (kMsLdsBytes + 15) / 16;
static_assert((kMsThreads / 64) * kMsLdsQuads * 16 + 512 <= 40960, "k_merge_short: four workgroups a CU (160 KB of LDS, allocated in units of 1,280 bytes)");
TKZ_DEV MsLds tkz_ms_lds(uint4* wave_quads, const uint16_t* brank16) {
    MsLds L;
    uint8_t* b = reinterpret_cast<uint8_t*>(wave_quads);
    L.pr = reinterpret_cast<uint4*>(b); b += kMsStride * 64 * 4;
    L.ids = reinterpret_cast<uint32_t*>(b); b += kMsIdStride * 64 * 4;
    L.extra = reinterpret_cast<int*>(b); b += 4 * kGroup;
    L.rec = reinterpret_cast<uint16_t*>(b); b += 2 * 2 * 64;
    L.idx = reinterpret_cast<uint16_t*>(b); b += 2 * 2 * 64;
    L.pre = reinterpret_cast<uint16_t*>(b);
    L.brank16 = brank16;
    return L;
}
TKZ_DEV void tkz_ms_brank_init(const TkzTables& T, uint16_t* s_brank16) {
    for (int i = simt::tid(); i < 256; i += simt::nthreads()) {
        const uint32_t v = (uint32_t)T.byte_rank[i];
        s_brank16[i] = (uint16_t)(v >= (uint32_t)TKZ_PSEUDO_BASE ? 0xFFFFu : (v < 0xFFFEu ? v : 0xFFFEu));
    }
}
TKZ_DEV void tkz_merge_short_group(const TkzTables& T, const EncodeParams& P, int64_t grp, const MsLds& LD) {
    constexpr int NMAX = 16, STRIDE = kMsStride, IDSTRIDE = kMsIdStride;
    static_assert(kGroup == 16 && kShortMax == 16, "list entries: 4 bits of sub-tile, 10 of index; 10 of relpos, 4 of length, 1 flag");
    const int lane = simt::lane();
    const uint16_t* s_brank16 = LD.brank16;
    auto byte_id = [&](uint32_t b) -> uint32_t {
        const uint32_t v = s_brank16[b];
        return v < 0xFFFEu ? v : (v == 0xFFFFu ? (uint32_t)TKZ_PSEUDO_BASE + b : (uint32_t)T.byte_rank[b]);
    };
    auto pair_rank = [&](uint32_t b0, uint32_t b1) -> int32_t { return T.bytepair_rank[(b0 << 8) | b1]; };
    const int64_t sub0 = grp * kGroup;
    if (sub0 >= P.nsub) return;
    uint16_t* s_rec = LD.rec;
    uint16_t* s_idx = LD.idx;
    int* s_extra = LD.extra;
    uint16_t* s_pre = LD.pre;
    uint32_t* ids = LD.ids + lane * IDSTRIDE;
    uint32_t* pr = reinterpret_cast<uint32_t*>(LD.pr) + lane * STRIDE;
    int my_np = 0, my_ns = 0;
// ... 1779 lines not shown
            ProbeText tx;
            tkz_probe_request_text(P, sub, &tx);
            tkz_probe_subtile<true>(T, P, sub, tkz_probe_lds(s_raw + wave * kProbeLdsQuads, s_kmask), tx, -1);
            (void)simt::ballot(true);
        }
    }
    simt::sync();
    if (tid == 0) { int f = P.counters[0] != 0; for (int t = 0; t < nsub; ++t) f |= (P.heavy_flag[t] & 2u) != 0; s_flag = f; }
    simt::sync();
    if (s_flag) {
        if (tid == 0) { A.h_result[0] = 1; A.h_result[1] = P.counters[0]; }
        return;
    }
    stamp();
    {
        uint16_t* s_brank16 = reinterpret_cast<uint16_t*>(s_raw + 8 * kMsLdsQuads);
        tkz_ms_brank_init(T, s_brank16);
        simt::sync();
        for (int g = wave; g < 8 && g * kGroup < nsub; g += nwaves) tkz_merge_short_group(T, P, g, tkz_ms_lds(s_raw + wave * kMsLdsQuads, s_brank16));
    }
    simt::sync();
    stamp();
    if (wave == 0) {
        const LongLds LD = tkz_long_lds(s_raw);
        tkz_long_brank_init(T, LD.brank);
        if (T.max_rank <= kVarCompactMaxRank) tkz_merge_long_chunks<true>(T, P, 0, 1, LD, kSmallLanePiece);
        else tkz_merge_long_chunks<false>(T, P, 0, 1, LD, kSmallLanePiece);
    }
    simt::sync();
    stamp();
    if (wave == 0) {
        int carry = 0;
        for (int q0 = 0; q0 < nsub; q0 += 64) {
            const int q = q0 + lane;
            int tot;
            const int pre = carry + tkz_wave_scan_sum(q < nsub ? P.tile_count[q] : 0, &tot);
            if (q < nsub) A.tile_base[q] = pre;
            carry += tot;
        }
        if (lane == 0) { A.h_result[2] = carry; A.tile_base[nsub] = carry; }
    }
    simt::sync();
    stamp();
    for (int s0 = wave * kPlacePer; s0 < nsub; s0 += nwaves * kPlacePer)
    {
        if (P.promo) tkz_place_subtiles<64, true, kStageMin>(P, A.tile_base, A.out, A.out_cap, s0, tkz_place_lds<64, kStageMin>(s_raw + wave * kPlaceLdsQuads));
        else tkz_place_subtiles<64, false, kStageMin>(P, A.tile_base, A.out, A.out_cap, s0, tkz_place_lds<64, kStageMin>(s_raw + wave * kPlaceLdsQuads));
    }
    simt::sync();
    stamp();
    {
        const int64_t grand = A.tile_base[nsub];
        for (int64_t d = tid; d <= n_docs; d += kThreads) {
            const int64_t pos = d_offs[d];
            if (pos >= total) { A.out_offs[d] = grand; continue; }
            const int64_t sub = pos / kSub, wpos = pos >> 6;
            int64_t ord = A.docord_base[sub];
            for (int64_t w = sub * (kSub / 64); w < wpos; ++w) ord += tkz_popc64(A.docbits[w]);
            ord += tkz_popc64(A.docbits[wpos] & tkz_lowmask((int)(pos & 63)));
            A.out_offs[d] = A.tile_base[sub] + P.doc_tok[ord];
        }
    }
    simt::sync();
    stamp();
    if (tid == 0) {
        const int32_t err = P.counters[0]; A.h_result[1] = err; A.h_result[0] = err ? 1 : 0;
        if (!err) for (int k = 0; k < 2; ++k) if (A.counts3[k]) { A.counts3[k][0] = n_docs; A.counts3[k][1] = total; A.counts3[k][2] = A.tile_base[nsub]; }
    }
}

static inline void hook(const Launch& L, int id, int phase) { if (L.hook) L.hook(L.hook_ctx, id, phase, L.stream); }
static inline int64_t cdiv(int64_t a, int64_t b) { return (a + b - 1) / b; }
static inline int64_t grid1(int64_t g) { return g < 1 ? 1 : g; }
static inline int64_t xcd_grid(int64_t blocks) { return (blocks + 7) & ~(int64_t)7; }
static inline int64_t grid_for(int64_t items) { const int64_t g = cdiv(items, kThreads); return g < 1 ? 1 : (g > 16384 ? 16384 : g); }

void launch_docmark(const Launch& L, const int64_t* d_offs, int64_t n_items, int64_t total, uint64_t* bits, int32_t* counters) {
    hook(L, K_DOCMARK, 0);
    TKZ_LAUNCH(k_docmark, grid_for(n_items + 1), kThreads, L.stream, d_offs, n_items, total, bits, counters);
    hook(L, K_DOCMARK, 1);
}
void launch_pretok_rows(const Launch& L, int pattern, const uint8_t* d_bytes, const int64_t* d_offs, int64_t n_docs, int64_t total,
                        const uint64_t* docbits, uint64_t* startbits, int64_t nrows, const uint8_t* bmp, int32_t* counters,
                        int64_t* xq, unsigned long long* xcount) {
    const int64_t grid = cdiv(nrows, kRowsPerWave);
    hook(L, K_PRETOK, 0);
    if (pattern == TKZ_PAT_P1)
        TKZ_LAUNCH(k_pretok_rows<TKZ_PAT_P1>, grid, 64, L.stream, d_bytes, total, docbits, startbits, nrows, bmp, counters, xq, xcount);
    else if (pattern == TKZ_PAT_CL100K)
        TKZ_LAUNCH(k_pretok_rows<TKZ_PAT_CL100K>, grid, 64, L.stream, d_bytes, total, docbits, startbits, nrows, bmp, counters, xq, xcount);
    else {
        TKZ_LAUNCH(k_pretok_rows<TKZ_PAT_O200K>, grid, 64, L.stream, d_bytes, total, docbits, startbits, nrows, bmp, counters, xq, xcount);
        int64_t* xq2 = xq + grid + 1;
        unsigned long long* xcount2 = xcount + 1;
        TKZ_LAUNCH(k_pretok_mb_blocks, grid < 8192 ? grid : 8192, 64, L.stream, d_bytes, total, docbits, startbits, nrows, bmp, (const uint8_t*)xq, grid,
                   xcount, xq2, xcount2, (int)(pattern == TKZ_PAT_O200K));
        TKZ_LAUNCH(k_pretok_seq_blocks, grid_for(n_docs > grid ? n_docs : grid), kThreads, L.stream, d_bytes, d_offs, n_docs, total, startbits, nrows,
                   pattern, bmp, (const int64_t*)xq2, (const unsigned long long*)xcount2, counters);
    }
    hook(L, K_PRETOK, 1);
}
void launch_pretok_seq(const Launch& L, int pattern, const uint8_t* d_bytes, const int64_t* d_offs, int64_t n_docs, int64_t total,
                       uint64_t* startbits, const uint8_t* bmp, int32_t* counters) {
    hook(L, K_PRETOK, 0);
    TKZ_LAUNCH(k_pretok_seq, grid_for(n_docs), kThreads, L.stream, d_bytes, d_offs, n_docs, total, startbits, pattern, bmp, counters);
    hook(L, K_PRETOK, 1);
}
static void launch_giants(const Launch& L, const TkzTables& T, const EncodeParams& P) {
#ifdef TKZ_HOSTEMU
    constexpr int kGiantGrid = 2;
#else
    constexpr int kGiantGrid = 256;
#endif
    TKZ_LAUNCH(k_giant_order, 1, 1024, L.stream, P);
    TKZ_LAUNCH(k_giant_merge, kGiantGrid, 1024, L.stream, T, P);
}
static void launch_long_queue(const Launch& L, const EncodeParams& P, int64_t nsub) {
    const int64_t nchunks = cdiv(nsub, 64), g4 = cdiv(nchunks, 4);
    TKZ_LAUNCH(k_long_count, g4 < 4096 ? g4 : 4096, kThreads, L.stream, P);
    launch_scan2(L, nchunks * kLenClasses, P.lq_bsum, P.lq_cnt, P.lq_base, P.lq_total, 1, nullptr, nullptr, nullptr, 1, -1);
    TKZ_LAUNCH(k_long_scatter, g4 < 4096 ? g4 : 4096, kThreads, L.stream, P);
}
static void launch_long_q(hipStream_t st, const TkzTables& T, const EncodeParams& P, int64_t cap) {
    const int64_t ranges = cdiv(P.lq_cap, kLqRangeLong), grid = ranges < cap ? (ranges < 1 ? 1 : ranges) : cap;
    if (T.max_rank <= kVarCompactMaxRank) TKZ_LAUNCH((k_merge_long_q<true>), grid, 64, st, T, P);
    else TKZ_LAUNCH((k_merge_long_q<false>), grid, 64, st, T, P);
}
static void launch_coop(hipStream_t st, const TkzTables& T, const EncodeParams& P, int64_t grid, int64_t cap) {
    TKZ_LAUNCH(k_merge_coop, grid < cap ? grid : cap, 64, st, T, P);
}
constexpr int64_t kSideLongGrid = 2048, kSideCoopGrid = 1024;
void launch_encode(const Launch& L, const TkzTables& T, const EncodeParams& P, int64_t nsub) {
    hook(L, K_ENCODE, 0);
    if (P.specbits) TKZ_LAUNCH(k_probe_special, xcd_grid(cdiv(nsub, (kThreads / 64) * kProbePer)), kThreads, L.stream, T, P);
    else TKZ_LAUNCH(k_probe, xcd_grid(cdiv(nsub, (kThreads / 64) * kProbePer)), kThreads, L.stream, T, P);
    hook(L, K_ENCODE, 1);
    { const int64_t g = grid_for(nsub); TKZ_LAUNCH(k_list_stats, g < 1024 ? g : 1024, kThreads, L.stream, (const uint32_t*)P.mcount, nsub, P.mcap, P.counters,
                                                     (const uint8_t*)P.heavy_flag, P.startbits, P.nwords, P.total, P.giant_q, P.giant_count, P.giant_cap,
                                                     (const uint32_t*)P.mlist, P.coop_q, P.coop_count, P.coop_cap, (int)P.lane_piece, P.miss_sums); }
    const int64_t nb_short = xcd_grid(cdiv(nsub, (kMsThreads / 64) * kGroup));
    if (P.latency) {
        hook(L, K_HEAVY, 0);
        launch_giants(L, T, P);
        hook(L, K_HEAVY, 1);
        const int64_t chunks = cdiv(nsub, 64) * kLongPartsLatency, nb_long = cdiv(chunks < 65536 ? chunks : 65536, kMsThreads / 64);
        hook(L, K_MERGE_SHORT, 0);
        if (T.max_rank <= kVarCompactMaxRank) TKZ_LAUNCH((k_merge_latency<true>), nb_short + nb_long, kMsThreads, L.stream, T, P, (int)nb_short, (int)nb_long);
        else TKZ_LAUNCH((k_merge_latency<false>), nb_short + nb_long, kMsThreads, L.stream, T, P, (int)nb_short, (int)nb_long);
        launch_coop(L.stream, T, P, 512, kCoopGrid);
        hook(L, K_MERGE_SHORT, 1);
    } else if (!L.side) {
        hook(L, K_MERGE_SHORT, 0);
        TKZ_LAUNCH(k_merge_short, nb_short, kMsThreads, L.stream, T, P);
        hook(L, K_MERGE_SHORT, 1);
        hook(L, K_HEAVY, 0);
        launch_giants(L, T, P);
        launch_long_queue(L, P, nsub);
        launch_long_q(L.stream, T, P, kLongQGrid);
        launch_coop(L.stream, T, P, cdiv(nsub, 64), kCoopGrid);
        hook(L, K_HEAVY, 1);
    } else {
        hook(L, K_HEAVY, 0);
        launch_giants(L, T, P);
        launch_long_queue(L, P, nsub);
        hook(L, K_HEAVY, 1);
        hook(L, K_MERGE_SHORT, 0);
        (void)hipEventRecord(L.ev_fork, L.stream); (void)hipStreamWaitEvent(L.side, L.ev_fork, 0); (void)hipStreamWaitEvent(L.side2, L.ev_fork, 0);
        launch_long_q(L.side, T, P, kSideLongGrid);
        launch_coop(L.side2, T, P, cdiv(nsub, 64), kSideCoopGrid);
        (void)hipEventRecord(L.ev_join, L.side); (void)hipEventRecord(L.ev_join2, L.side2);
        TKZ_LAUNCH(k_merge_short, nb_short, kMsThreads, L.stream, T, P);
        (void)hipStreamWaitEvent(L.stream, L.ev_join, 0); (void)hipStreamWaitEvent(L.stream, L.ev_join2, 0);
        hook(L, K_MERGE_SHORT, 1);
    }
}
void launch_probe_sample(const Launch& L, const TkzTables& T, const EncodeParams& P, int64_t nsample) {
    if (nsample > P.nsub) nsample = P.nsub;
    hook(L, K_ENCODE, 0);
    if (P.specbits) TKZ_LAUNCH(k_probe_special, xcd_grid(cdiv(nsample, (kThreads / 64) * kProbePer)), kThreads, L.stream, T, P);
    else TKZ_LAUNCH(k_probe, xcd_grid(cdiv(nsample, (kThreads / 64) * kProbePer)), kThreads, L.stream, T, P);
    hook(L, K_ENCODE, 1);
    { const int64_t g = grid_for(nsample); TKZ_LAUNCH(k_list_stats, g < 1024 ? g : 1024, kThreads, L.stream, (const uint32_t*)P.mcount, nsample, P.mcap, P.counters,
                                                     (const uint8_t*)P.heavy_flag, P.startbits, P.nwords, P.total, P.giant_q, P.giant_count, P.giant_cap,
                                                     (const uint32_t*)P.mlist, P.coop_q, P.coop_count, P.coop_cap, (int)P.lane_piece, P.miss_sums); }
}
void launch_ingest(const Launch& L, const uint8_t* h_bytes, int64_t total, uint8_t* d_bytes, const int64_t* h_offs, int64_t n_offs, int64_t* d_offs, void* zero, int64_t zero_bytes) {
    const int64_t quads = std::max<int64_t>(total / 16 + 1, (zero_bytes + 15) / 16);
    const int64_t g = cdiv(quads, kThreads * 4);
    TKZ_LAUNCH(k_ingest, g < 1 ? 1 : (g > 2048 ? 2048 : g), kThreads, L.stream, h_bytes, total, d_bytes, h_offs, n_offs, d_offs, reinterpret_cast<uint4*>(zero), (zero_bytes + 15) / 16);
}
void launch_small(const Launch& L, const TkzTables& T, const EncodeParams& P, const SmallArgs& A) {
    TKZ_LAUNCH(k_small, 1, P.nsub <= 4 ? 256 : 1024, L.stream, T, P, A);
}
void launch_place(const Launch& L, const EncodeParams& P, const int64_t* tile_base, int64_t nsub, int32_t* out, int64_t out_cap) {
    hook(L, K_GATHER, 0);
    const int64_t grid = xcd_grid(cdiv(nsub, (kThreads / 64) * kPlacePer));
    if (P.promo) {
        if (P.place128) TKZ_LAUNCH((k_place<128, true>), grid, kThreads, L.stream, P, tile_base, out, out_cap);
        else TKZ_LAUNCH((k_place<64, true>), grid, kThreads, L.stream, P, tile_base, out, out_cap);
    } else {
        if (P.place128) TKZ_LAUNCH((k_place<128, false>), grid, kThreads, L.stream, P, tile_base, out, out_cap);
        else TKZ_LAUNCH((k_place<64, false>), grid, kThreads, L.stream, P, tile_base, out, out_cap);
    }
    hook(L, K_GATHER, 1);
}
void launch_doccount2(const Launch& L, const uint64_t* bits_a, const uint64_t* bits_b, int64_t nwords, int64_t total, int64_t nsub, int32_t* cnt_a, int32_t* cnt_b) {
    TKZ_LAUNCH(k_doccount2, grid_for(nsub * (kSub / 64)), kThreads, L.stream, bits_a, bits_b, nwords, total, nsub, cnt_a, cnt_b);
}
void launch_scan2(const Launch& L, int64_t ntiles, int64_t* bsum, const int32_t* cnt_a, int64_t* base_a, int64_t* grand_a, int round_to_a,
                  const int32_t* cnt_b, int64_t* base_b, int64_t* grand_b, int round_to_b, int kid) {
    if (ntiles <= kScanSmallMax) {
        if (kid >= 0) hook(L, kid, 0);
        TKZ_LAUNCH(k_scan_small, 1, 1024, L.stream, cnt_a, base_a, grand_a, round_to_a > 1 ? round_to_a - 1 : 0, cnt_b, base_b, grand_b, round_to_b > 1 ? round_to_b - 1 : 0, (int)ntiles);
        if (kid >= 0) hook(L, kid, 1);
        return;
    }
    launch_scan(L, cnt_a, ntiles, bsum, base_a, grand_a, kid, round_to_a);
    if (cnt_b) launch_scan(L, cnt_b, ntiles, bsum, base_b, grand_b, kid, round_to_b);
}
void launch_scan(const Launch& L, const int32_t* tile_count, int64_t ntiles, int64_t* bsum, int64_t* tile_base, int64_t* grand, int kid, int round_to) {
    const int64_t nblk = grid1(cdiv(ntiles, kScanBlock));
    const int round = round_to > 1 ? round_to - 1 : 0;
    if (kid >= 0) hook(L, kid, 0);
    TKZ_LAUNCH(k_scan_partials, nblk, kThreads, L.stream, tile_count, ntiles, bsum, round);
    TKZ_LAUNCH(k_scan_top, 1, kThreads, L.stream, bsum, nblk, grand);
    TKZ_LAUNCH(k_scan_final, nblk, kThreads, L.stream, tile_count, ntiles, (const int64_t*)bsum, tile_base, round);
    if (kid >= 0) hook(L, kid, 1);
}
void launch_docoffs(const Launch& L, const int64_t* d_offs, int64_t n_docs, int64_t total, const int64_t* tile_base,
                    const uint64_t* docbits, const int64_t* docord_base, const int32_t* doc_tok, const int64_t* grand, int64_t* out_offs,
                    int64_t c3_docs, int64_t* c3a, int64_t* c3b, int64_t* c3c) {
    hook(L, K_DOCOFFS, 0);
    TKZ_LAUNCH(k_docoffs, grid_for(n_docs + 1), kThreads, L.stream, d_offs, n_docs, total, tile_base, docbits, docord_base, doc_tok, grand, out_offs, c3_docs, c3a, c3b, c3c);
    hook(L, K_DOCOFFS, 1);
}
void launch_case_equiv_fix(const Launch& L, const uint8_t* d_bytes, int64_t total, const uint64_t* docbits, uint64_t* startbits) {
    TKZ_LAUNCH(k_case_equiv_fix, grid_for((total + 7) / 8), kThreads, L.stream, d_bytes, total, docbits, startbits);
}
void launch_lit_scan(const Launch& L, const uint8_t* d_bytes, int64_t total, const uint64_t* docbits, int64_t nwords, const TkzLitTable& LT, const TkzLitAllowed& A,
                     uint64_t* candbits, uint64_t* segbits, uint64_t* specbits, uint64_t* endbits, unsigned long long* n_taken) {
    TKZ_LAUNCH(k_lit_scan, grid1(cdiv(nwords, (kThreads / 64) * (kLitBlock / 64))), kThreads, L.stream, d_bytes, total, docbits, nwords, LT, A, candbits, segbits, specbits, endbits);
    TKZ_LAUNCH(k_lit_resolve, grid_for(nwords), kThreads, L.stream, d_bytes, total, docbits, (const uint64_t*)candbits, nwords, LT, segbits, specbits, endbits, n_taken);
    hook(L, K_DOCMARK, 1);
}
void launch_lit_fix(const Launch& L, uint64_t* startbits, const uint64_t* segbits, const uint64_t* specbits, const uint64_t* endbits, int64_t nwords) {
    TKZ_LAUNCH(k_lit_fix, grid_for(nwords), kThreads, L.stream, startbits, segbits, specbits, endbits, nwords);
    hook(L, K_PRETOK, 1);
}
void launch_seg_offsets(const Launch& L, const uint64_t* segbits, int64_t nwords, int64_t total, int64_t nsub, const int64_t* ord_base, int64_t n_seg, int64_t* seg_offs) {
    TKZ_LAUNCH(k_piece_index, grid1(cdiv(nsub, kThreads / 64)), kThreads, L.stream, segbits, nwords, total, nsub, ord_base, n_seg, seg_offs);
}
void launch_rebase(const Launch& L, int64_t* offs, int64_t n, int64_t base) {
    TKZ_LAUNCH(k_rebase, grid_for(n), kThreads, L.stream, offs, n, base);
}
void launch_miss_stats(const Launch& L, const EncodeParams& P, int64_t nsub) {
    const int64_t g = grid_for(nsub);
    TKZ_LAUNCH(k_miss_stats, g < 1024 ? g : 1024, kThreads, L.stream, (const uint32_t*)P.mcount, P.pcount, nsub, P.stats);
}
void launch_counts3(const Launch& L, int64_t n_docs, int64_t total, const int64_t* grand, int64_t* out3, int64_t* out3b, int64_t* out3c) {
    TKZ_LAUNCH(k_counts3, 1, 64, L.stream, n_docs, total, grand, out3, out3b, out3c);
}
void launch_u16_len(const Launch& L, const uint16_t* units, int64_t total, const uint64_t* docbits, int64_t ntiles, int32_t* grp_prefix, int32_t* tile_sum) {
    TKZ_LAUNCH(k_u16_len, grid1(cdiv(ntiles, kThreads / 64)), kThreads, L.stream, units, total, docbits, ntiles, grp_prefix, tile_sum);
// ... 31 lines not shown
```

Measured before the change: 254,800.

## Resolve mid-length piece lookups ahead of time inside the pretokenizer kernel

```diff
diff --git a/include/tkz.h b/include/tkz.h
--- a/include/tkz.h
+++ b/include/tkz.h
@@ -150,6 +150,7 @@
 void tkz_encoder_small_path_calls(const tkz_encoder* e, int64_t* calls, int64_t* handed_back);
 int32_t tkz_encoder_small_path_phases(const tkz_encoder* e, int64_t* clocks16);
 tkz_status tkz_encoder_piece_stats(tkz_encoder* e, int64_t* out8, int32_t reset);
+tkz_status tkz_encoder_mid_ahead_stats(tkz_encoder* e, int64_t* out2);
 tkz_status tkz_encoder_adapt_stats(tkz_encoder* e, int64_t* out8);
 int64_t tkz_encoder_memo_slots(const tkz_encoder* e);
 int32_t tkz_encoder_memo_ways(const tkz_encoder* e);
diff --git a/tokenizer_amd/_native.py b/tokenizer_amd/_native.py
--- a/tokenizer_amd/_native.py
+++ b/tokenizer_amd/_native.py
@@ -116,6 +116,7 @@
         L.tkz_encoder_set_option.argtypes = [vp, i32, i64]
         L.tkz_encoder_piece_stats.argtypes = [vp, vp, i32]
         L.tkz_encoder_adapt_stats.argtypes = [vp, vp]
+        L.tkz_encoder_mid_ahead_stats.argtypes = [vp, vp]
         L.tkz_encoder_reserve.argtypes = [vp, i64, i64]
         L.tkz_encoder_set_profiling.argtypes = [vp, i32]
         L.tkz_encoder_kernel_ms.argtypes = [vp, vp, vp, i32]
@@ -255,6 +256,11 @@
                 "memo_lookups": look, "memo_hits": hit, "memo_hit_rate": round(hit / look, 5) if look else None,
                 "merged_short": look - hit if look else sm, "promoted_pieces_in_tables": int(out[7])}
 
+    def mid_ahead_stats(self):
+        out = np.zeros(2, np.int64)
+        self.lib.check(self.lib.L.tkz_encoder_mid_ahead_stats(self._h, out.ctypes.data))
+        return int(out[0]), int(out[1])
+
     def reserve(self, max_bytes, max_docs):
         self.lib.check(self.lib.L.tkz_encoder_reserve(self._h, int(max_bytes), int(max_docs)))
 
diff --git a/tokenizer_amd/csrc/tkz_api.cpp b/tokenizer_amd/csrc/tkz_api.cpp
--- a/tokenizer_amd/csrc/tkz_api.cpp
+++ b/tokenizer_amd/csrc/tkz_api.cpp
@@ -111,6 +111,9 @@
     DevBuf w_zero; size_t zero_bytes = 0;
     DevView w_counters, w_docbits, w_heavyq;
     DevBuf w_mlist, w_mquad, w_mcount, w_pextra, w_coopq, w_lqcnt, w_lqbase, w_lq;
+    DevBuf w_midahead;
+    bool mid_ahead_on = false;
+    const void* ahead_mid = nullptr; const void* ahead_promo = nullptr; uint32_t ahead_promo_n = 0;
     bool learn_window_start = false;
     DevBuf w_candbits, w_segbits, w_specbits, w_endbits, w_segoffs;
     int64_t n_seg = 0;
@@ -163,7 +166,7 @@
     double ms[tkz::K_COUNT] = {};
     int64_t launches[tkz::K_COUNT] = {};
     void release_all() {
-        DevBuf* bufs[] = {&w_candbits, &w_segbits, &w_specbits, &w_endbits, &w_segoffs, &w_counts3, &w_mlist, &w_mquad, &w_mcount, &w_pextra, &w_coopq, &w_lqcnt, &w_lqbase, &w_lq, &w_gq, &w_gcnt, &w_xq, &w_zero, &w_startbits, &w_tmp, &w_dense, &w_tcount, &w_prank, &w_pcount, &w_pbase, &w_tbase, &w_bsum,
+        DevBuf* bufs[] = {&w_candbits, &w_segbits, &w_specbits, &w_endbits, &w_segoffs, &w_counts3, &w_mlist, &w_mquad, &w_mcount, &w_pextra, &w_midahead, &w_coopq, &w_lqcnt, &w_lqbase, &w_lq, &w_gq, &w_gcnt, &w_xq, &w_zero, &w_startbits, &w_tmp, &w_dense, &w_tcount, &w_prank, &w_pcount, &w_pbase, &w_tbase, &w_bsum,
                           &w_doctok, &w_dcount, &w_dbase, &w_pool, &s_bytes[0], &s_bytes[1], &s_offs[0], &s_offs[1], &s_out[0], &s_out[1], &s_out[2],
                           &s_outoffs[0], &s_outoffs[1], &s_outoffs[2], &u_bytes[0], &u_bytes[1],
                           &d_grp, &d_tsum, &d_tbase, &d_bsum, &d_counters, &d_ids, &d_idoffs, &d_out, &d_outoffs, &p_boffs, &p_toffs, &p_docp};
@@ -484,7 +487,12 @@
     return TKZ_OK;
 }
 
-tkz_status prepare_workspace(Workspace* ws, int64_t total, int64_t n_docs, bool bitmap_only, bool pieces) {
+bool mid_ahead_wanted(const tkz_encoder* e) {
+    const char* v = getenv("TKZ_NO_MID_AHEAD");
+    return !(v && *v && *v != '0') && !e->pretok_seq && (e->pattern == TKZ_PATTERN_P1 || e->pattern == TKZ_PATTERN_CL100K);
+}
+
+tkz_status prepare_workspace(Workspace* ws, int64_t total, int64_t n_docs, bool bitmap_only, bool pieces, bool ahead) {
     using namespace tkz;
     const int64_t nwords = total / 64 + 1;
     const int64_t ntiles = (total + kSub - 1) / kSub;
@@ -510,6 +518,7 @@
         HIP_TRY(ws->w_mquad.ensure((size_t)ntiles * (size_t)ws->mcap * 16, acc));
         HIP_TRY(ws->w_mcount.ensure((size_t)ntiles * 4, acc));
         HIP_TRY(ws->w_pextra.ensure((size_t)ntiles * 4, acc));
+        if (ahead) HIP_TRY(ws->w_midahead.ensure((size_t)(ntiles + 1) * kAheadPerSub * 4, acc));
         HIP_TRY(ws->w_coopq.ensure((size_t)(total / kLanePiece + 64) * 8, acc));
         {
             const int64_t nchunks = (ntiles + 63) / 64;
@@ -674,6 +683,7 @@
     uint64_t* docbits = ws->w_docbits.as<uint64_t>();
     uint64_t* startbits = ws->w_startbits.as<uint64_t>();
     const SpecialCall* const special = d_bitmap_only || po || !pretok ? nullptr : g_special;
+    if (!marks_reused) ws->mid_ahead_on = false;
     if (marks_reused) {
         HIP_TRY(hipMemsetAsync(ws->w_zero.p, 0, 256, stream));
         if (!d_bitmap_only) HIP_TRY(hipMemsetAsync(ws->w_heavyq.p, 0, (size_t)(ws->w_zero.as<char>() + ws->zero_bytes - ws->w_heavyq.as<char>()), stream));
@@ -710,8 +720,12 @@
             launch_pretok_seq(L, e->pattern, d_bytes, iso_offs, n_iso, total, startbits, T.bmp_class, counters);
         } else {
             HIP_TRY(ws->w_xq.ensure((size_t)(nwords / kRowsPerWave + 4) * 16, &ws->bytes_allocated));
+            ws->mid_ahead_on = !d_bitmap_only && !special && !e->case_equiv && (e->pattern == TKZ_PATTERN_P1 || e->pattern == TKZ_PATTERN_CL100K) &&
+                               T.mid_slots && T.mid_ns && ws->w_midahead.cap >= (size_t)(ntiles + 1) * kAheadPerSub * 4 && mid_ahead_wanted(e);
+            ws->ahead_mid = T.mid_slots; ws->ahead_promo = T.promo; ws->ahead_promo_n = T.promo_n;
             launch_pretok_rows(L, e->pattern, d_bytes, iso_offs, n_iso, total, isobits, startbits, nwords, T.bmp_class, counters,
-                               ws->w_xq.as<int64_t>(), reinterpret_cast<unsigned long long*>(cb + offsetof(CounterBlock, xcount)));
+                               ws->w_xq.as<int64_t>(), reinterpret_cast<unsigned long long*>(cb + offsetof(CounterBlock, xcount)),
+                               ws->mid_ahead_on ? &T : nullptr, ws->w_midahead.as<uint32_t>());
         }
         if (pretok && e->case_equiv && e->pattern == TKZ_PATTERN_CL100K) launch_case_equiv_fix(L, d_bytes, total, isobits, startbits);
         if (special) launch_lit_fix(L, startbits, isobits, ws->w_specbits.as<uint64_t>(), ws->w_endbits.as<uint64_t>(), nwords);
@@ -740,6 +754,8 @@
             P.long_log_count = reinterpret_cast<unsigned long long*>(e->t_long_log.as<char>() + (size_t)kLongLogCap * kLongLogDwords * 4);
         }
         if (special) { P.specbits = ws->w_specbits.as<uint64_t>(); P.lit_meta = e->LIT.meta; P.lit_blob = e->LIT.blob; P.n_lit = e->LIT.n; }
+        P.mid_ahead = ws->mid_ahead_on && ws->ahead_mid == (const void*)T.mid_slots && ws->ahead_promo == (const void*)T.promo && ws->ahead_promo_n == T.promo_n
+                      ? ws->w_midahead.as<uint32_t>() : nullptr;
         TKZ_TRY(devprof_arm(&P, stream));
         int64_t* ndocstarts = reinterpret_cast<int64_t*>(cb + offsetof(CounterBlock, ndocstarts));
         int64_t* npieces = reinterpret_cast<int64_t*>(cb + offsetof(CounterBlock, npieces));
@@ -904,7 +920,7 @@
     }
     const int64_t ntiles = (total + kSub - 1) / kSub;
     SlowCallLog slow_log(total);
-    TKZ_TRY(prepare_workspace(ws, total, n_docs, d_bitmap_only != nullptr, po != nullptr));
+    TKZ_TRY(prepare_workspace(ws, total, n_docs, d_bitmap_only != nullptr, po != nullptr, mid_ahead_wanted(e)));
     if (!ws->h_counters) HIP_TRY(hipHostMalloc((void**)&ws->h_counters, sizeof(CounterBlock), 0));
 
     struct LearnGuard {
@@ -961,7 +977,7 @@
                         int32_t* out_ids, int64_t out_cap, int64_t* out_offsets, int64_t* needed, bool* handled) {
     using namespace tkz;
     *handled = false;
-    { const tkz_status ps = prepare_workspace(ws, total, n_docs, false, false); if (ps != TKZ_OK) return ps; }
+    { const tkz_status ps = prepare_workspace(ws, total, n_docs, false, false, false); if (ps != TKZ_OK) return ps; }
     int64_t* acc = &ws->bytes_allocated;
     HIP_TRY(ws->s_bytes[0].ensure((size_t)kSmallMaxBytes + 64, acc));
     HIP_TRY(ws->s_offs[0].ensure((size_t)(kSmallMaxDocs + 1) * 8, acc));
@@ -1990,6 +2006,19 @@
     if (reset) { HIP_TRY(hipMemset(e->t_stats.p, 0, 64)); e->stat_batches = e->stat_giants = 0; }
     return TKZ_OK;
 }
+tkz_status tkz_encoder_mid_ahead_stats(tkz_encoder* e, int64_t* out2) {
+    if (!e || !out2) return fail(TKZ_E_ARG, "null argument");
+    out2[0] = out2[1] = 0;
+    if (!e->t_stats.p) return TKZ_OK;
+    DeviceScope scope;
+    tkz_status st = check_encoder(e, scope);
+    if (st != TKZ_OK) return st;
+    unsigned long long h[8] = {};
+    HIP_TRY(hipDeviceSynchronize());
+    HIP_TRY(hipMemcpy(h, e->t_stats.p, sizeof h, hipMemcpyDeviceToHost));
+    out2[0] = (int64_t)h[5]; out2[1] = (int64_t)h[6];
+    return TKZ_OK;
+}
 int64_t tkz_encoder_memo_slots(const tkz_encoder* e) { return e ? (int64_t)e->memo_slots : 0; }
 void tkz_encoder_small_path_calls(const tkz_encoder* e, int64_t* calls, int64_t* handed_back) {
     int64_t c = 0, f = 0;
@@ -2021,7 +2050,7 @@
     Lease lease(e);
     Workspace* ws = lease.ws;
     int64_t* acc = &ws->bytes_allocated;
-    st = prepare_workspace(ws, max_bytes, max_docs, false, false);
+    st = prepare_workspace(ws, max_bytes, max_docs, false, false, mid_ahead_wanted(e));
     if (st != TKZ_OK) return st;
     const int64_t nwords = max_bytes / 64 + 1;
     HIP_TRY(ws->w_xq.ensure((size_t)(nwords / kRowsPerWave + 4) * 16, acc));
diff --git a/tokenizer_amd/csrc/tkz_kernels.h b/tokenizer_amd/csrc/tkz_kernels.h
--- a/tokenizer_amd/csrc/tkz_kernels.h
+++ b/tokenizer_amd/csrc/tkz_kernels.h
@@ -30,6 +30,9 @@
 constexpr int kRowsPerWave = 62;
 constexpr int kScanBlock = 1024;
 constexpr int kRecordLine = 16;
+constexpr int kAheadPerRow = 5, kAheadPerSub = (kSub / 64) * kAheadPerRow;
+constexpr uint32_t kAheadValid = 0x80000000u;
+TKZ_HD int tkz_ahead_slot(int pos) { return (pos >> 6) * kAheadPerRow + (pos & 63) / 13; }
 constexpr int kMissCapMin = 64, kMissCapMax = 1024;
 
 enum { K_DOCMARK = 0, K_PRETOK = 1, K_ENCODE = 2, K_SCAN = 3, K_GATHER = 4, K_DOCOFFS = 5, K_HEAVY = 6, K_MERGE_SHORT = 7, K_COUNT = 8 };
@@ -74,6 +77,7 @@
     int32_t tc_atomic;
     int32_t place128;
     const uint64_t* specbits; const uint32_t* lit_meta; const uint8_t* lit_blob; int32_t n_lit;
+    const uint32_t* mid_ahead;
 };
 
 constexpr int kLitMax = 256, kLitMaxLen = 128, kLitMetaHead = 8;
@@ -98,7 +102,7 @@
 void launch_docmark(const Launch& L, const int64_t* d_offs, int64_t n_items, int64_t total, uint64_t* bits, int32_t* counters);
 void launch_pretok_rows(const Launch& L, int pattern, const uint8_t* d_bytes, const int64_t* d_offs, int64_t n_docs, int64_t total,
                         const uint64_t* docbits, uint64_t* startbits, int64_t nrows, const uint8_t* bmp, int32_t* counters,
-                        int64_t* xq, unsigned long long* xcount);
+                        int64_t* xq, unsigned long long* xcount, const TkzTables* T = nullptr, uint32_t* mid_ahead = nullptr);
 void launch_pretok_seq(const Launch& L, int pattern, const uint8_t* d_bytes, const int64_t* d_offs, int64_t n_docs, int64_t total,
                        uint64_t* startbits, const uint8_t* bmp, int32_t* counters);
 void launch_ingest(const Launch& L, const uint8_t* h_bytes, int64_t total, uint8_t* d_bytes, const int64_t* h_offs, int64_t n_offs, int64_t* d_offs, void* zero, int64_t zero_bytes);
diff --git a/tokenizer_amd/csrc/tkz_kernels.hip b/tokenizer_amd/csrc/tkz_kernels.hip
--- a/tokenizer_amd/csrc/tkz_kernels.hip
+++ b/tokenizer_amd/csrc/tkz_kernels.hip
@@ -100,9 +100,69 @@
     if (simt::ballot(bad != 0) && lane == 0) simt::atomic_or((unsigned*)&counters[0], (unsigned)kErrUtf8);
 }
 
+struct alignas(4) TkzDwords4 { uint32_t x, y, z, w; };
+template <int BITS> TKZ_DEV int tkz_wave_scan(int v, int* total);
+
+TKZ_DEV void tkz_mid_ahead_block(const TkzTables& T, const uint8_t* bytes, int64_t first, uint64_t out, uint32_t* mid_ahead,
+                                 uint32_t* s_res, uint16_t* s_cand, uint64_t* s_word) {
+    const int lane = simt::lane();
+    constexpr int kSlots = kRowsPerWave * kAheadPerRow;
+    const bool own = lane >= 1 && lane <= kRowsPerWave;
+    const uint64_t w = own ? out : 0ull;
+    uint32_t nx = simt::shflu((uint32_t)out, (lane + 1) & 63);
+    if (lane >= kRowsPerWave) nx = 0;
+    struct W96 { uint64_t lo; uint32_t hi; };
+    auto shr = [](W96 a, int k) -> W96 { W96 r; r.lo = (a.lo >> k) | ((uint64_t)a.hi << (64 - k)); r.hi = a.hi >> k; return r; };
+    auto orr = [](W96 a, W96 b) -> W96 { W96 r; r.lo = a.lo | b.lo; r.hi = a.hi | b.hi; return r; };
+    W96 x; x.lo = w; x.hi = nx;
+    const W96 a1 = shr(x, 1), a2 = orr(a1, shr(a1, 1)), a4 = orr(a2, shr(a2, 2)), a8 = orr(a4, shr(a4, 4));
+    const W96 a12 = orr(a8, shr(a4, 8)), a16 = orr(a8, shr(a8, 8)), a28 = orr(a16, shr(a12, 16));
+    const uint64_t mid = w & ~a12.lo & a28.lo;
+    s_word[lane] = out;
+    for (int i = lane; i < kSlots; i += 64) s_res[i] = 0;
+    int ncand;
+    {
+        int off = tkz_wave_scan<3>(tkz_popc64(mid), &ncand);
+        for (uint64_t b = mid; b; b &= b - 1) s_cand[off++] = (uint16_t)((lane << 6) | tkz_ctz64(b));
+    }
+    (void)simt::ballot(true);
+    const char* mb = reinterpret_cast<const char*>(T.mid_slots);
+#pragma unroll 1
+    for (int m0 = 0; m0 < ncand; m0 += 64) {
+        const bool valid = m0 + lane < ncand;
+        uint32_t kk[7] = {0, 0, 0, 0, 0, 0, 0}, oa = 0, ob = 0;
+        int len = TKZ_SHORT_KEY_MAX + 1, slot = 0;
+        if (valid) {
+            const int e = s_cand[m0 + lane], r = e >> 6, p = e & 63;
+            const uint64_t wn = r < kRowsPerWave ? (uint64_t)(uint32_t)s_word[r + 1] : 0ull;
+            len = 1 + tkz_ctz64z(((s_word[r] >> p) >> 1) | (wn << (63 - p)));
+            slot = (r - 1) * kAheadPerRow + p / 13;
+            const uint8_t* a0 = bytes + (((first + r) << 6) + (p & ~3));
+            const TkzDwords4 lo = *reinterpret_cast<const TkzDwords4*>(a0), hi = *reinterpret_cast<const TkzDwords4*>(a0 + 16);
+            const uint32_t d[8] = {lo.x, lo.y, lo.z, lo.w, hi.x, hi.y, hi.z, hi.w};
+            const uint32_t sh = (uint32_t)(p & 3) * 8u;
+#pragma unroll
+            for (int i = 0; i < 7; ++i) {
+                const uint32_t v = simt::alignbit(d[i + 1], d[i], sh);
+                const int nb = len - 4 * i;
+                kk[i] = nb >= 4 ? v : (nb <= 0 ? 0u : (v & ((1u << (8 * nb)) - 1u)));
+            }
+            uint32_t s1, s2;
+            tkz_mid_slots(T, kk, (uint32_t)len, &s1, &s2);
+            oa = 32u * s1; ob = 32u * s2;
+        }
+        const uint4 q0 = tkz_load16(mb + oa), q1 = tkz_load16(mb + oa + 16u), q2 = tkz_load16(mb + ob), q3 = tkz_load16(mb + ob + 16u);
+        if (valid) s_res[slot] = kAheadValid | (uint32_t)tkz_match_mid(kk, (uint32_t)len, q0, q1, q2, q3);
+    }
+    (void)simt::ballot(true);
+    uint32_t* const dst = mid_ahead + (first + 1) * kAheadPerRow;
+    for (int i = lane; i < kSlots; i += 64) dst[i] = s_res[i];
+}
+
 template <int PATTERN>
 TKZ_KERNEL(64) void k_pretok_rows(const uint8_t* bytes, int64_t total, const uint64_t* docbits, uint64_t* startbits,
-                                  int64_t nrows, const uint8_t* bmp, int32_t* counters, int64_t* xq, unsigned long long* xcount) {
+                                  int64_t nrows, const uint8_t* bmp, int32_t* counters, int64_t* xq, unsigned long long* xcount,
+                                  TkzTables T, uint32_t* mid_ahead) {
     TKZ_SHARED uint16_t s_aflags[128];
     TKZ_SHARED uint4 s_blk[(65 * kBlockRowStride) / 16];
     for (int i = simt::tid(); i < 128; i += simt::nthreads()) s_aflags[i] = (uint16_t)tkz_ascii_flags((uint32_t)i, PATTERN == TKZ_PAT_CL100K);
@@ -138,6 +198,15 @@
         if (done) {
             if (lane >= 1 && lane <= kRowsPerWave && row < nrows) startbits[row] = out;
             if (PATTERN == TKZ_PAT_O200K && lane == 0) reinterpret_cast<uint8_t*>(xq)[simt::bid()] = 0;
+            if constexpr (PATTERN != TKZ_PAT_O200K) {
+                if (mid_ahead) {
+                    constexpr int kSlots = kRowsPerWave * kAheadPerRow;
+                    static_assert(64 * 8 + kSlots * 4 + kSlots * 2 <= (int)sizeof(s_blk), "the look-ahead's lists fit the staged block");
+                    uint8_t* const sb = reinterpret_cast<uint8_t*>(s_blk);
+                    tkz_mid_ahead_block(T, bytes, first, out, mid_ahead, reinterpret_cast<uint32_t*>(sb + 64 * 8), reinterpret_cast<uint16_t*>(sb + 64 * 8 + kSlots * 4),
+                                        reinterpret_cast<uint64_t*>(sb));
+                }
+            }
             return;
         }
     }
@@ -146,6 +215,7 @@
         for (int64_t r = r0 + lane; r < r1; r += 64) startbits[r] = docbits[r];
         if (lane == 0) reinterpret_cast<uint8_t*>(xq)[simt::bid()] = 1;
     } else {
+        if (mid_ahead) for (int64_t i = r0 * kAheadPerRow + lane; i < r1 * kAheadPerRow; i += 64) mid_ahead[i] = 0;
         TkzSrc S;
         S.bytes = bytes; S.total = total; S.stage = nullptr; S.lo = 0; S.hi = 0;
         tkz_rows_sequential<PATTERN>(S, docbits, startbits, nrows, bmp, s_aflags, r0, r1, counters);
@@ -490,7 +560,10 @@
 
 constexpr int kProbeLdsBytes = (kSub + kHalo) + 2 * (kSub + 2) + 2 * kMidMax + 4 * kMidMax + 4 * (kSub / 32);
 constexpr int kProbeLdsQuads = (kProbeLdsBytes + 15) / 16;
-struct ProbeLds { uint32_t* bytes; uint16_t* pstart; uint16_t* mid; uint32_t* midres; uint32_t* mark; const uint4* kmask; uint32_t* spec ; };
+struct ProbeLds {
+    uint32_t* bytes; uint16_t* pstart; uint16_t* mid; uint32_t* midres; uint32_t* mark; const uint4* kmask; uint32_t* spec ;
+    uint32_t* ahead; uint16_t* ford;
+};
 TKZ_DEV ProbeLds tkz_probe_lds(uint4* wave_quads, const uint4* kmask) {
     ProbeLds L;
     uint8_t* b = reinterpret_cast<uint8_t*>(wave_quads);
@@ -501,6 +574,7 @@
     L.mid = reinterpret_cast<uint16_t*>(b);
     L.kmask = kmask;
     L.spec = nullptr;
+    L.ahead = nullptr; L.ford = nullptr;
     return L;
 }
 TKZ_DEV void tkz_probe_kmask_init(uint4* s_kmask) {
@@ -548,7 +622,7 @@
     }
     return TKZ_RANK_NONE;
 }
-template <bool REPORT, bool SPECIAL = false>
+template <bool REPORT, bool SPECIAL = false, bool AHEAD = false>
 TKZ_DEV void tkz_probe_subtile(const TkzTables& T, const EncodeParams& P, int64_t sub, const ProbeLds& LD, ProbeText& tx, int64_t next) {
     const int lane = simt::lane();
     uint32_t* s_bytes = LD.bytes;
@@ -573,7 +647,14 @@
     const int64_t from = base + nb, w0 = from >> 6;
     uint64_t ahead = (w0 + lane < P.nwords) ? P.startbits[w0 + lane] : 0ull;
     const int64_t pb = P.pbase[sub];
+    uint32_t ah0 = 0, ah1 = 0;
+    if (AHEAD) {
+        const uint32_t* ap = P.mid_ahead + sub * kAheadPerSub;
+        ah0 = tkz_load_nt(ap + lane);
+        if (lane < kAheadPerSub - 64) ah1 = tkz_load_nt(ap + 64 + lane);
+    }
     { uint4* s4 = reinterpret_cast<uint4*>(s_bytes); s4[lane] = v0; if (lane + 64 < (kSub + kHalo) / 16) s4[lane + 64] = v1; }
+    if (AHEAD) { LD.ahead[lane] = ah0; if (lane < kAheadPerSub - 64) LD.ahead[64 + lane] = ah1; }
     if (next >= 0) tkz_probe_request_text(P, next, &tx);
     if (lane < kSub / 64) {
         const int lim = nb - lane * 64;
@@ -611,14 +692,28 @@
     const char* tb0 = reinterpret_cast<const char*>(T.short_slots);
     const uint32_t mid_off = (uint32_t)(reinterpret_cast<const char*>(T.mid_slots) - tb0);
     int nmid = 0;
+    int nord = 0, n28 = 0, nslot = 0;
 #pragma unroll 1
     for (int k0 = 0; k0 < np; k0 += 64) {
         const int k = k0 + lane;
         int len = 0;
         if (k < np) len = (int)s_pstart[k + 1] - (int)s_pstart[k];
-        const uint64_t midm = simt::ballot(len > TKZ_SHORT_KEY_MAX && len <= kArenaPiece);
-        if ((midm >> lane) & 1ull) s_mid[nmid + tkz_popc64(midm & tkz_lowmask(lane))] = (uint16_t)k;
-        nmid += tkz_popc64(midm);
+        const bool is13 = len > TKZ_SHORT_KEY_MAX && len <= kArenaPiece;
+        const uint64_t midm = simt::ballot(is13);
+        if (!AHEAD) {
+            if ((midm >> lane) & 1ull) s_mid[nmid + tkz_popc64(midm & tkz_lowmask(lane))] = (uint16_t)k;
+            nmid += tkz_popc64(midm);
+        } else if (midm) {
+            const int ord = nord + tkz_popc64(midm & tkz_lowmask(lane));
+            uint32_t slot = 0;
+            if (is13 && len <= TKZ_MID_KEY_MAX) slot = LD.ahead[tkz_ahead_slot((int)s_pstart[k])];
+            const bool hit = (slot & kAheadValid) != 0;
+            if (hit) s_midres[ord] = slot & ~kAheadValid;
+            const uint64_t fm = simt::ballot(is13 && !hit);
+            if (is13 && !hit) { const int j = nmid + tkz_popc64(fm & tkz_lowmask(lane)); s_mid[j] = (uint16_t)k; LD.ford[j] = (uint16_t)ord; }
+            nmid += tkz_popc64(fm); nord += tkz_popc64(midm);
+            if (P.stats) { n28 += tkz_popc64(simt::ballot(is13 && len <= TKZ_MID_KEY_MAX)); nslot += tkz_popc64(simt::ballot(hit)); }
+        }
     }
     (void)simt::ballot(true);
 #pragma unroll 1
@@ -648,7 +743,7 @@
             if (s + len <= kSub + kHalo) rank = tkz_lookup_long(T, [&](int i) -> uint32_t { return sb[s + i]; }, (uint32_t)len);
             else rank = tkz_lookup_long(T, [&](int i) -> uint32_t { return gbase[s + i]; }, (uint32_t)len);
         }
-        if (valid) s_midres[m0 + lane] = (uint32_t)rank;
+        if (valid) s_midres[AHEAD ? (int)LD.ford[m0 + lane] : m0 + lane] = (uint32_t)rank;
     }
     (void)simt::ballot(true);
     if (prof) t_2 = simt::clock();
@@ -784,6 +879,7 @@
         if (!REPORT && P.tc_atomic) P.tile_count[sub] = 0;
         if (REPORT && ns + nl > P.mcap) { simt::atomic_or((unsigned*)&P.counters[0], (unsigned)kErrMissCap); simt::atomic_max((unsigned*)&P.counters[1], (unsigned)(ns + nl)); }
         if (pb + np > P.prank_cap) simt::atomic_or((unsigned*)&P.counters[0], (unsigned)kErrCapacity);
+        if (AHEAD && P.stats && n28) { simt::atomic_add64(&P.stats[5], (unsigned long long)n28); simt::atomic_add64(&P.stats[6], (unsigned long long)nslot); }
     }
 }
 TKZ_KERNEL_OCC(256, TKZ_PROBE_OCC) void k_probe(TkzTables T, EncodeParams P) {
@@ -800,6 +896,27 @@
     for (int it = 0; it < kProbePer && sub0 + it < P.nsub; ++it) {
         const int64_t nxt = (it + 1 < kProbePer && sub0 + it + 1 < P.nsub) ? sub0 + it + 1 : -1;
         tkz_probe_subtile<false>(T, P, sub0 + it, LD, tx, nxt);
+        (void)simt::ballot(true);
+    }
+}
+
+TKZ_KERNEL_OCC(256, TKZ_PROBE_OCC) void k_probe_ahead(TkzTables T, EncodeParams P) {
+    TKZ_SHARED uint4 s_wave[kThreads / 64][kProbeLdsQuads];
+    TKZ_SHARED uint4 s_kmask[TKZ_SHORT_KEY_MAX + 1];
+    TKZ_SHARED uint32_t s_ahead[kThreads / 64][kAheadPerSub];
+    TKZ_SHARED uint16_t s_ford[kThreads / 64][kMidMax];
+    tkz_probe_kmask_init(s_kmask);
+    simt::sync();
+    const int64_t sub0 = (tkz_xcd_block(simt::bid(), simt::nblocks()) * (kThreads / 64) + simt::wave()) * kProbePer;
+    if (sub0 >= P.nsub) return;
+    ProbeLds LD = tkz_probe_lds(s_wave[simt::wave()], s_kmask);
+    LD.ahead = s_ahead[simt::wave()]; LD.ford = s_ford[simt::wave()];
+    ProbeText tx;
+    tkz_probe_request_text(P, sub0, &tx);
+#pragma unroll 1
+    for (int it = 0; it < kProbePer && sub0 + it < P.nsub; ++it) {
+        const int64_t nxt = (it + 1 < kProbePer && sub0 + it + 1 < P.nsub) ? sub0 + it + 1 : -1;
+        tkz_probe_subtile<false, false, true>(T, P, sub0 + it, LD, tx, nxt);
         (void)simt::ballot(true);
     }
 }
@@ -824,7 +941,6 @@
     }
 }
 
-struct alignas(4) TkzDwords4 { uint32_t x, y, z, w; };
 TKZ_DEV void tkz_load_piece16(const uint8_t* bytes, int64_t total, int64_t abs, uint32_t* pw) {
     const int64_t a0 = abs & ~(int64_t)3;
     const uint32_t sh = (uint32_t)(abs & 3) * 8u;
@@ -2770,15 +2886,16 @@
 }
 void launch_pretok_rows(const Launch& L, int pattern, const uint8_t* d_bytes, const int64_t* d_offs, int64_t n_docs, int64_t total,
                         const uint64_t* docbits, uint64_t* startbits, int64_t nrows, const uint8_t* bmp, int32_t* counters,
-                        int64_t* xq, unsigned long long* xcount) {
+                        int64_t* xq, unsigned long long* xcount, const TkzTables* Tp, uint32_t* mid_ahead) {
     const int64_t grid = cdiv(nrows, kRowsPerWave);
+    const TkzTables T0 = Tp ? *Tp : TkzTables{};
     hook(L, K_PRETOK, 0);
     if (pattern == TKZ_PAT_P1)
-        TKZ_LAUNCH(k_pretok_rows<TKZ_PAT_P1>, grid, 64, L.stream, d_bytes, total, docbits, startbits, nrows, bmp, counters, xq, xcount);
+        TKZ_LAUNCH(k_pretok_rows<TKZ_PAT_P1>, grid, 64, L.stream, d_bytes, total, docbits, startbits, nrows, bmp, counters, xq, xcount, T0, Tp ? mid_ahead : nullptr);
     else if (pattern == TKZ_PAT_CL100K)
-        TKZ_LAUNCH(k_pretok_rows<TKZ_PAT_CL100K>, grid, 64, L.stream, d_bytes, total, docbits, startbits, nrows, bmp, counters, xq, xcount);
+        TKZ_LAUNCH(k_pretok_rows<TKZ_PAT_CL100K>, grid, 64, L.stream, d_bytes, total, docbits, startbits, nrows, bmp, counters, xq, xcount, T0, Tp ? mid_ahead : nullptr);
     else {
-        TKZ_LAUNCH(k_pretok_rows<TKZ_PAT_O200K>, grid, 64, L.stream, d_bytes, total, docbits, startbits, nrows, bmp, counters, xq, xcount);
+        TKZ_LAUNCH(k_pretok_rows<TKZ_PAT_O200K>, grid, 64, L.stream, d_bytes, total, docbits, startbits, nrows, bmp, counters, xq, xcount, T0, (uint32_t*)nullptr);
         int64_t* xq2 = xq + grid + 1;
         unsigned long long* xcount2 = xcount + 1;
         TKZ_LAUNCH(k_pretok_mb_blocks, grid < 8192 ? grid : 8192, 64, L.stream, d_bytes, total, docbits, startbits, nrows, bmp, (const uint8_t*)xq, grid,
@@ -2818,10 +2935,15 @@
     TKZ_LAUNCH(k_merge_coop, grid < cap ? grid : cap, 64, st, T, P);
 }
 constexpr int64_t kSideLongGrid = 2048, kSideCoopGrid = 1024;
+static void launch_probe(const Launch& L, const TkzTables& T, const EncodeParams& P, int64_t n) {
+    const int64_t grid = xcd_grid(cdiv(n, (kThreads / 64) * kProbePer));
+    if (P.specbits) TKZ_LAUNCH(k_probe_special, grid, kThreads, L.stream, T, P);
+    else if (P.mid_ahead) TKZ_LAUNCH(k_probe_ahead, grid, kThreads, L.stream, T, P);
+    else TKZ_LAUNCH(k_probe, grid, kThreads, L.stream, T, P);
+}
 void launch_encode(const Launch& L, const TkzTables& T, const EncodeParams& P, int64_t nsub) {
     hook(L, K_ENCODE, 0);
-    if (P.specbits) TKZ_LAUNCH(k_probe_special, xcd_grid(cdiv(nsub, (kThreads / 64) * kProbePer)), kThreads, L.stream, T, P);
-    else TKZ_LAUNCH(k_probe, xcd_grid(cdiv(nsub, (kThreads / 64) * kProbePer)), kThreads, L.stream, T, P);
+    launch_probe(L, T, P, nsub);
     hook(L, K_ENCODE, 1);
     { const int64_t g = grid_for(nsub); TKZ_LAUNCH(k_list_stats, g < 1024 ? g : 1024, kThreads, L.stream, (const uint32_t*)P.mcount, nsub, P.mcap, P.counters,
                                                      (const uint8_t*)P.heavy_flag, P.startbits, P.nwords, P.total, P.giant_q, P.giant_count, P.giant_cap,
@@ -2865,8 +2987,7 @@
 void launch_probe_sample(const Launch& L, const TkzTables& T, const EncodeParams& P, int64_t nsample) {
     if (nsample > P.nsub) nsample = P.nsub;
     hook(L, K_ENCODE, 0);
-    if (P.specbits) TKZ_LAUNCH(k_probe_special, xcd_grid(cdiv(nsample, (kThreads / 64) * kProbePer)), kThreads, L.stream, T, P);
-    else TKZ_LAUNCH(k_probe, xcd_grid(cdiv(nsample, (kThreads / 64) * kProbePer)), kThreads, L.stream, T, P);
+    launch_probe(L, T, P, nsample);
     hook(L, K_ENCODE, 1);
     { const int64_t g = grid_for(nsample); TKZ_LAUNCH(k_list_stats, g < 1024 ? g : 1024, kThreads, L.stream, (const uint32_t*)P.mcount, nsample, P.mcap, P.counters,
                                                      (const uint8_t*)P.heavy_flag, P.startbits, P.nwords, P.total, P.giant_q, P.giant_count, P.giant_cap,
```

Result: slower. 250,900 (-1.5%).
